# sailab-code/GNN_tf_2.x

Measured on AMD Instinct MI355X. Metric: node-state-updates/sec (nodes x iters / s), 1M-node synthetic graph, higher is better.
Workload: dtype f32; 1 GPU; synthetic randomGraph-recipe graph, N=1000000 nodes, E=9999690 arcs, state_dim=64, net_state 135->128->128->64 selu+BN, net_output 67->2 softmax+BN, max_iter=30, threshold=0 (all iterations run); the loop-invariant label aggregates (GNN.py:259, :263; 0.2 ms) are kept between Loops until the labels change, see cold_aggregates_ms_per_step; parallelism=single GPU, tile_form=one wave per 32-node tile (k_fused)

## Files before the change

gnn_tf_2.x_amd/GNN/_engine.py:

```python
from __future__ import annotations

import ctypes as C
import os

import numpy as np

_HERE = os.path.dirname(os.path.abspath(__file__))
LIB_PATH = os.environ.get('GNN_HIP_LIBRARY') or os.path.join(_HERE, 'libgnn_hip.so')

ACT_CODES = {'linear': 0, None: 0, 'relu': 1, 'selu': 2, 'elu': 3, 'tanh': 4, 'sigmoid': 5, 'softmax': 6}

EXPORTS = ['gnn_last_error', 'gnn_version', 'gnn_device_count', 'gnn_device_synchronize', 'gnn_graph_create', 'gnn_graph_create_from_arcs',
           'gnn_graph_derive', 'gnn_graph_derive_edge', 'gnn_graph_set_arc_order', 'gnn_graph_update_labels', 'gnn_graph_get_nodes', 'gnn_graph_dims', 'gnn_graph_destroy',
           'gnn_mlp_create', 'gnn_mlp_set_weights', 'gnn_mlp_get_weights', 'gnn_mlp_reset_optimizer', 'gnn_mlp_forward', 'gnn_mlp_destroy', 'gnn_loop_create',
           'gnn_loop_set_state0', 'gnn_loop_run', 'gnn_loop_get_state', 'gnn_loop_get_output', 'gnn_loop_readout', 'gnn_loop_set_edge_readout', 'gnn_loop_train_step',
           'gnn_loop_train_forward', 'gnn_loop_train_backward', 'gnn_loop_arm_optimizer', 'gnn_loop_optimizer_step', 'gnn_loop_update_moving_statistics', 'gnn_loss_grad',
           'gnn_loss_grad_ex', 'gnn_loop_set_loss_params',
           'gnn_mlp_set_regularizers', 'gnn_loop_set_clipping', 'gnn_loop_grad_sqnorm', 'gnn_loop_optimizer_step_scaled',
           'gnn_counters_get', 'gnn_lgnn_run', 'gnn_loop_run_many', 'gnn_loop_set_impl', 'gnn_loop_gate_info', 'gnn_loop_set_pieces', 'gnn_loop_range_info', 'gnn_split_f16_exponent', 'gnn_split_f16', 'gnn_loop_set_persistent', 'gnn_loop_set_tile_form', 'gnn_loop_drop_cached_aggregates', 'gnn_loop_set_profiling', 'gnn_loop_get_timing', 'gnn_loop_get_exchange_timing', 'gnn_loop_destroy', 'gnn_shard_range',
           'gnn_comm_unique_id', 'gnn_comm_create', 'gnn_comm_allreduce_max', 'gnn_comm_destroy', 'gnn_halo_plan', 'gnn_graph_create_halo',
           'gnn_comm_create_loopback', 'gnn_graph_set_full_adjacency', 'gnn_loop_set_slice_exchange', 'gnn_loop_run_group', 'gnn_loop_readout_group', 'gnn_graph_update_labels_group']

_lib = None


class EngineError(RuntimeError):
    pass


def lib():
    global _lib
    if _lib is None:
        if not os.path.exists(LIB_PATH):
            raise EngineError(f'{LIB_PATH} is missing: build it with `python -c "import __graft_entry__ as g; g.build()"` '
                              f'or `make -C gnn_tf_2.x_amd/csrc`')
        _lib = C.CDLL(LIB_PATH)
        _lib.gnn_last_error.restype = C.c_char_p
        for name in EXPORTS:
            if name != 'gnn_last_error':
                getattr(_lib, name).restype = C.c_int
    return _lib


def loss_grad(loss_kind: int, targets, out, sample_weights, label_smoothing: float = 0.0, huber_delta: float = 1.0):
    t, o, w = _f32(targets), _f32(out), _f32(sample_weights)
    if t.shape != o.shape or w.shape != (o.shape[0],): raise ValueError(f'targets {t.shape}, outputs {o.shape}, weights {w.shape} do not match')
    d = np.zeros_like(o)
    loss = C.c_double()
    _check(lib().gnn_loss_grad_ex(C.c_int(loss_kind), C.c_int64(o.shape[0]), C.c_int(o.shape[1]), _fp(t), _fp(o), _fp(w), C.c_double(label_smoothing),
                                  C.c_double(huber_delta), C.byref(loss), _fp(d)))
    return float(loss.value), d


def split_f16(values, exponent=None):
    v = np.ascontiguousarray(values, np.float32).ravel()
    if exponent is None:
        exponent = int(lib().gnn_split_f16_exponent(C.c_float(float(np.max(np.abs(v))) if v.size else 0.0)))
    p0, p1 = np.empty(v.size, np.uint16), np.empty(v.size, np.uint16)
    lib().gnn_split_f16(v.ctypes.data_as(C.c_void_p), C.c_int(v.size), C.c_int(int(exponent)), p0.ctypes.data_as(C.c_void_p), p1.ctypes.data_as(C.c_void_p))
    return p0.view(np.float16), p1.view(np.float16), int(exponent)


def _check(rc: int):
    if rc == 0:
        return
    msg = lib().gnn_last_error().decode(errors='replace')
    if rc == -1:
        raise ValueError(msg)
    if rc == -5:
        raise NotImplementedError(msg)
    raise EngineError(f'[gnn_status {rc}] {msg}')


def _f32(a, shape=None):
    a = np.ascontiguousarray(a, dtype=np.float32)
    if shape is not None and a.shape != tuple(shape):
        raise ValueError(f'expected shape {tuple(shape)}, got {a.shape}')
    return a


def _fp(a):
    return a.ctypes.data_as(C.POINTER(C.c_float)) if a is not None else None


def _ip(a):
    return a.ctypes.data_as(C.POINTER(C.c_int32)) if a is not None else None


def device_count() -> int:
    n = C.c_int(0)
    _check(lib().gnn_device_count(C.byref(n)))
    return n.value


def require_device(device: int = 0) -> None:
    n = device_count()
    if n <= device:
        raise EngineError(f'no HIP device {device} visible ({n} found): this engine only runs on MI355X (gfx950)')


def shard_range(n_nodes: int, rank: int, world: int) -> tuple[int, int]:
    b, n = C.c_int64(0), C.c_int64(0)
    _check(lib().gnn_shard_range(C.c_int64(n_nodes), C.c_int(rank), C.c_int(world), C.byref(b), C.byref(n)))
    return b.value, n.value


def halo_plan(n_nodes: int, world: int, indptr, adj_src):
    indptr = np.ascontiguousarray(indptr, dtype=np.int32)
    adj_src = np.ascontiguousarray(adj_src, dtype=np.int32)
    slot = np.empty(n_nodes, np.int32)
    counts = np.zeros(world, np.int64)
    block = C.c_int64(0)
    _check(lib().gnn_halo_plan(C.c_int64(n_nodes), C.c_int(world), _ip(indptr), _ip(adj_src), _ip(slot),
                               counts.ctypes.data_as(C.POINTER(C.c_int64)), C.byref(block)))
    return slot, counts, int(block.value)


def shard_halo(n_nodes: int, rank: int, world: int, indptr, adj_src, nodes, plan=None):
    slot, counts, block = plan if plan is not None else halo_plan(n_nodes, world, indptr, adj_src)
    rb, nr = shard_range(n_nodes, rank, world)
    shard = ((n_nodes + world - 1) // world + 31) // 32 * 32
    indptr = np.asarray(indptr)
    e0, e1 = int(indptr[rb]), int(indptr[rb + nr])
    src = np.asarray(adj_src)[e0:e1].astype(np.int64)
    owner = src // shard
    mine = owner == rank
    if np.any(~mine & (slot[src] < 0)):
        raise ValueError('halo plan does not cover a remote source')
    remapped = np.where(mine, src - rb, shard + owner * block + slot[src]).astype(np.int32)
    nodes = np.asarray(nodes, np.float32)
    rep = np.zeros((shard + world * block, nodes.shape[1]), np.float32)
    rep[:nr] = nodes[rb:rb + nr]
    for q in range(world):
        qb, qn = shard_range(n_nodes, q, world)
        ids = qb + np.nonzero(slot[qb:qb + qn] >= 0)[0]
        rep[shard + q * block: shard + q * block + len(ids)] = nodes[ids]
    send = np.nonzero(slot[rb:rb + nr] >= 0)[0].astype(np.int32)
    return dict(block=block, send_rows=send, adj_src=remapped, nodes=rep, row_begin=rb, n_rows=nr, e0=e0, e1=e1)


def shard_csr(n_nodes: int, rank: int, world: int, indptr, *per_entry_arrays):
    rb, nr = shard_range(n_nodes, rank, world)
    indptr = np.asarray(indptr)
    e0, e1 = int(indptr[rb]), int(indptr[rb + nr])
    return (rb, nr, (indptr[rb:rb + nr + 1] - e0).astype(np.int32)) + tuple(np.asarray(a)[e0:e1] for a in per_entry_arrays)


class Graph:

    def __init__(self, n_nodes, indptr, adj_src, adj_w, arc_w, arc_labels, nodes, mask, row_begin=0, device=0, _handle=None):
        self._h = C.c_void_p()
        if _handle is not None:
            self._h = _handle
            return
        require_device(device)
        indptr = np.ascontiguousarray(indptr, dtype=np.int32)
        adj_src = np.ascontiguousarray(adj_src, dtype=np.int32)
        adj_w, arc_w = _f32(adj_w), _f32(arc_w)
        arc_labels, nodes = _f32(arc_labels), _f32(nodes)
        mask = np.ascontiguousarray(mask, dtype=np.uint8)
        n_rows, n_arcs = len(indptr) - 1, len(adj_src)
        if arc_labels.ndim != 2 or arc_labels.shape[0] != n_arcs or nodes.ndim != 2 or nodes.shape[0] != n_nodes:
            raise ValueError('arc_labels must be [n_arcs, AL] and nodes [n_nodes, NL]')
        if len(adj_w) != n_arcs or len(arc_w) != n_arcs or len(mask) != n_rows:
            raise ValueError('inconsistent array lengths')
        _check(lib().gnn_graph_create(C.c_int64(n_nodes), C.c_int64(row_begin), C.c_int64(n_rows), C.c_int64(n_arcs),
                                      _ip(indptr), _ip(adj_src), _fp(adj_w), _fp(arc_w), _fp(arc_labels),
                                      C.c_int(arc_labels.shape[1]), _fp(nodes), C.c_int(nodes.shape[1]),
                                      mask.ctypes.data_as(C.POINTER(C.c_uint8)), C.c_int(device), C.byref(self._h)))

    @classmethod
    def halo(cls, n_nodes_global, rank, world, block, send_rows, indptr, adj_src_replica, adj_w, arc_w, arc_labels, nodes_replica, mask, device=0):
        require_device(device)
        indptr = np.ascontiguousarray(indptr, dtype=np.int32)
        adj = np.ascontiguousarray(adj_src_replica, dtype=np.int32)
        send = np.ascontiguousarray(send_rows, dtype=np.int32)
        adj_w, arc_w, arc_labels, nodes_replica = _f32(adj_w), _f32(arc_w), _f32(arc_labels), _f32(nodes_replica)
        mask = np.ascontiguousarray(mask, dtype=np.uint8)
        if len(adj_w) != len(adj) or len(arc_w) != len(adj) or arc_labels.shape[0] != len(adj) or len(mask) != len(indptr) - 1:
            raise ValueError('inconsistent array lengths')
        h = C.c_void_p()
        _check(lib().gnn_graph_create_halo(C.c_int64(n_nodes_global), C.c_int(rank), C.c_int(world), C.c_int64(block), C.c_int64(len(send)), _ip(send),
                                           C.c_int64(len(adj)), _ip(indptr), _ip(adj), _fp(adj_w), _fp(arc_w), _fp(arc_labels), C.c_int(arc_labels.shape[1]),
                                           _fp(nodes_replica), C.c_int(nodes_replica.shape[1]), mask.ctypes.data_as(C.POINTER(C.c_uint8)), C.c_int(device), C.byref(h)))
        return cls(None, None, None, None, None, None, None, None, _handle=h)

    @classmethod
    def from_arcs(cls, n_nodes, arc_src, arc_dst, arc_labels, aggregation_mode, nodes, mask, device=0):
        require_device(device)
        modes = {'sum': 0, 'normalized': 1, 'average': 2}
        if aggregation_mode not in modes: raise ValueError('ERROR: Unknown aggregation mode')
        arc_src = np.ascontiguousarray(arc_src, dtype=np.int32)
        arc_dst = np.ascontiguousarray(arc_dst, dtype=np.int32)
        arc_labels, nodes = _f32(arc_labels), _f32(nodes)
        mask = np.ascontiguousarray(mask, dtype=np.uint8)
        e = len(arc_src)
        if len(arc_dst) != e or arc_labels.shape[0] != e or nodes.shape[0] != n_nodes or len(mask) != n_nodes:
            raise ValueError('inconsistent array lengths')
        indptr, adj_src, arc_id = np.zeros(n_nodes + 1, np.int32), np.zeros(e, np.int32), np.zeros(e, np.int32)
        adj_w, arc_w = np.zeros(e, np.float32), np.zeros(e, np.float32)
        h = C.c_void_p()
        _check(lib().gnn_graph_create_from_arcs(C.c_int64(n_nodes), C.c_int64(e), _ip(arc_src), _ip(arc_dst), _fp(arc_labels),
                                                C.c_int(arc_labels.shape[1]), C.c_int(modes[aggregation_mode]), _fp(nodes), C.c_int(nodes.shape[1]),
                                                mask.ctypes.data_as(C.POINTER(C.c_uint8)), C.c_int(device), C.byref(h), _ip(indptr), _ip(adj_src),
                                                _fp(adj_w), _ip(arc_id), _fp(arc_w)))
        return cls(None, None, None, None, None, None, None, None, _handle=h), indptr, adj_src, adj_w, arc_id, arc_w

    def dims(self):
        n, r, e, m = C.c_int64(), C.c_int64(), C.c_int64(), C.c_int64()
        nl, al = C.c_int(), C.c_int()
        _check(lib().gnn_graph_dims(self._h, C.byref(n), C.byref(r), C.byref(e), C.byref(nl), C.byref(al), C.byref(m)))
        return dict(n_nodes=n.value, n_rows=r.value, n_arcs=e.value, NL=nl.value, AL=al.value, n_masked=m.value)

    def derive(self, extra: int) -> 'Graph':
        h = C.c_void_p()
        _check(lib().gnn_graph_derive(self._h, C.c_int(extra), C.byref(h)))
        d = Graph(None, None, None, None, None, None, None, None, _handle=h)
        d._base = self
        return d

    def derive_edge(self, extra_nodes: int, extra_arcs: int) -> 'Graph':
        h = C.c_void_p()
        _check(lib().gnn_graph_derive_edge(self._h, C.c_int(extra_nodes), C.c_int(extra_arcs), C.byref(h)))
        d = Graph(None, None, None, None, None, None, None, None, _handle=h)
        d._base = self
        return d

    def set_arc_order(self, arc_id, arc_labels_orig) -> None:
        arc_id = np.ascontiguousarray(arc_id, dtype=np.int32)
        _check(lib().gnn_graph_set_arc_order(self._h, _ip(arc_id), _fp(_f32(arc_labels_orig))))

    def update_labels(self, base: 'Graph', loop: 'Loop', get_state: bool, get_output: bool) -> None:
        _check(lib().gnn_graph_update_labels(self._h, base._h, loop._h, C.c_int(bool(get_state)), C.c_int(bool(get_output))))

    def set_full_adjacency(self, n_global: int, indptr, adj_src, adj_w):
        ip, src, w = np.ascontiguousarray(indptr, np.int32), np.ascontiguousarray(adj_src, np.int32), _f32(adj_w)
        _check(lib().gnn_graph_set_full_adjacency(self._h, C.c_int64(n_global), _ip(ip), _ip(src), _fp(w)))

    @staticmethod
    def update_labels_group(dsts, bases, loops, get_state: bool, get_output: bool) -> None:
        n = len(loops)
        arr = lambda xs: (C.c_void_p * n)(*[x._h for x in xs])
        _check(lib().gnn_graph_update_labels_group(arr(dsts), arr(bases), arr(loops), C.c_int(n), C.c_int(bool(get_state)), C.c_int(bool(get_output))))

    def nodes(self) -> np.ndarray:
        d = self.dims()
        out = np.empty((d['n_nodes'], d['NL']), dtype=np.float32)
        _check(lib().gnn_graph_get_nodes(self._h, _fp(out)))
        return out

    def close(self):
        if self._h:
            lib().gnn_graph_destroy(self._h)
            self._h = C.c_void_p()

    def __del__(self):
        try:
            self.close()
        except Exception:
            pass


class Mlp:

    def __init__(self, weights, activations, batch_normalization, bn_eps=1e-3, device=0):
        require_device(device)
        self._h = C.c_void_p()
        self.n = len(activations)
        self.activations = list(activations)
        self.batch_normalization = bool(batch_normalization)
        for a in activations:
            if a not in ACT_CODES:
                raise ValueError(f'unsupported activation {a!r}')
        w, b, bn = self._pack(weights)
        self.dims = np.array([w[0].shape[0]] + [x.shape[1] for x in w], dtype=np.int32)
        acts = np.array([ACT_CODES[a] for a in activations], dtype=np.int32)
        wp = (C.POINTER(C.c_float) * self.n)(*[_fp(x) for x in w])
        bp = (C.POINTER(C.c_float) * self.n)(*[_fp(x) for x in b])
        _check(lib().gnn_mlp_create(C.c_int(self.n), _ip(self.dims), _ip(acts), wp, bp, _fp(bn), C.c_float(bn_eps),
                                    C.c_int(device), C.byref(self._h)))

    def _pack(self, weights):
        n = self.n
        if len(weights) != 2 * n + (4 if self.batch_normalization else 0):
            raise ValueError(f'expected {2 * n + (4 if self.batch_normalization else 0)} weight arrays, got {len(weights)}')
        w = [_f32(weights[2 * l]) for l in range(n)]
        b = [_f32(weights[2 * l + 1]) for l in range(n)]
        for l in range(n):
            if w[l].ndim != 2 or b[l].shape != (w[l].shape[1],) or (l and w[l].shape[0] != w[l - 1].shape[1]):
                raise ValueError(f'layer {l}: inconsistent weight shapes')
        bn = None
        if self.batch_normalization:
            bn = np.ascontiguousarray(np.concatenate([_f32(a).ravel() for a in weights[2 * n:]]))
            if bn.size != 4 * w[-1].shape[1]:
                raise ValueError('BatchNormalization arrays must each have the output width')
        return w, b, bn

    def set_weights(self, weights):
        w, b, bn = self._pack(weights)
        if [x.shape for x in w] != [(int(self.dims[l]), int(self.dims[l + 1])) for l in range(self.n)]:
            raise ValueError('weight shapes differ from the ones this MLP was created with')
        wp = (C.POINTER(C.c_float) * self.n)(*[_fp(x) for x in w])
        bp = (C.POINTER(C.c_float) * self.n)(*[_fp(x) for x in b])
        _check(lib().gnn_mlp_set_weights(self._h, wp, bp, _fp(bn)))

    def get_weights(self):
        w = [np.empty((int(self.dims[l]), int(self.dims[l + 1])), np.float32) for l in range(self.n)]
        b = [np.empty((int(self.dims[l + 1]),), np.float32) for l in range(self.n)]
        f = int(self.dims[-1])
        bn = np.empty(4 * f, np.float32) if self.batch_normalization else None
        wp = (C.POINTER(C.c_float) * self.n)(*[_fp(x) for x in w])
        bp = (C.POINTER(C.c_float) * self.n)(*[_fp(x) for x in b])
        _check(lib().gnn_mlp_get_weights(self._h, wp, bp, _fp(bn)))
        out = []
        for l in range(self.n):
            out += [w[l], b[l]]
        if bn is not None:
            out += [bn[i * f:(i + 1) * f].copy() for i in range(4)]
        return out

    def reset_optimizer(self):
        _check(lib().gnn_mlp_reset_optimizer(self._h))

    def set_regularizers(self, coefficients):
        key = None if coefficients is None else (tuple(coefficients[0]), tuple(coefficients[1]))
        if key is not None and not any(key[0]) and not any(key[1]): key = None
        if key == getattr(self, '_reg_set', None):
            return
        if key is None:
            _check(lib().gnn_mlp_set_regularizers(self._h, None, None))
        else:
            if len(key[0]) != 2 * self.n or len(key[1]) != 2 * self.n: raise ValueError(f'expected {2 * self.n} coefficients per list')
            _check(lib().gnn_mlp_set_regularizers(self._h, (C.c_double * (2 * self.n))(*key[0]), (C.c_double * (2 * self.n))(*key[1])))
        self._reg_set = key

    def forward(self, x):
        x = _f32(x)
        if x.ndim != 2 or x.shape[1] != self.dims[0]:
            raise ValueError(f'expected [n, {self.dims[0]}] input')
        y = np.empty((x.shape[0], int(self.dims[-1])), dtype=np.float32)
        _check(lib().gnn_mlp_forward(self._h, C.c_int64(x.shape[0]), _fp(x), _fp(y)))
        return y

    def close(self):
        if self._h:
            lib().gnn_mlp_destroy(self._h)
            self._h = C.c_void_p()

    def __del__(self):
        try:
            self.close()
        except Exception:
            pass


class Comm:

    def __init__(self, unique_id: bytes, rank: int, world: int, device: int, _handle=None):
        self._h = C.c_void_p()
        self.rank, self.world = rank, world
        if _handle is not None:
            self._h = _handle
            return
        buf = (C.c_uint8 * 128).from_buffer_copy(unique_id)
        _check(lib().gnn_comm_create(buf, C.c_int(rank), C.c_int(world), C.c_int(device), C.byref(self._h)))

    @classmethod
    def loopback(cls, world: int, device: int = 0) -> list:
        require_device(device)
        hs = (C.c_void_p * world)()
        _check(lib().gnn_comm_create_loopback(C.c_int(world), C.c_int(device), hs))
        return [cls(None, r, world, device, _handle=C.c_void_p(hs[r])) for r in range(world)]

    @staticmethod
    def unique_id() -> bytes:
        buf = (C.c_uint8 * 128)()
        _check(lib().gnn_comm_unique_id(buf))
        return bytes(buf)

# ... 67 lines not shown
        u8 = lambda a: a.ctypes.data_as(C.POINTER(C.c_uint8)) if a is not None else None
        if ng_csr is not None:
            ngi, ngn, ngw = np.ascontiguousarray(ng_csr[0], np.int32), np.ascontiguousarray(ng_csr[1], np.int32), _f32(ng_csr[2])
            n_graphs = len(ngi) - 1
        else:
            ngi = ngn = ngw = None
            n_graphs = 0
        bs = _f32(bn_state) if bn_state is not None else None
        bo = _f32(bn_output) if bn_output is not None else None
        loss, k = C.c_float(), C.c_float()
        _check(lib().gnn_loop_train_step(self._h, _ip(sip), _ip(sdst), _fp(sw), _fp(targets), _fp(sample_weights),
                                         C.c_int64(targets.shape[0]), C.c_int(loss_kind), C.c_int(n_graphs), _ip(ngi), _ip(ngn), _fp(ngw),
                                         _fp(ds_), _fp(do_), u8(ms), u8(mo), C.c_uint64(seed), _fp(bs), _fp(bo), C.byref(loss), C.byref(k),
                                         _fp(gs), _fp(go), _fp(bns), _fp(bno)))

        def split(flat, shp):
            out, off = [], 0
            for x in shp:
                cnt = int(np.prod(x))
                out.append(flat[off:off + cnt].reshape(x).copy())
                off += cnt
            return out

        kk = int(k.value)
        return dict(loss=float(loss.value), k=float(k.value), grads_state=split(gs, shp_s), grads_output=split(go, shp_o),
                    bn_batch_state=bns[:kk], bn_batch_output=bno)

    def set_slice_exchange(self, on=True, form=None):
        if form not in (None, 'oneshot', 'pipelined'):
            raise ValueError("form must be 'oneshot' or 'pipelined'")
        code = 0 if not on else (1 if form == 'pipelined' else 2)
        _check(lib().gnn_loop_set_slice_exchange(self._h, C.c_int(code)))

    def update_moving_statistics(self, bn_momentum_state: float = 0.99, bn_momentum_output: float = 0.99):
        _check(lib().gnn_loop_update_moving_statistics(self._h, C.c_float(bn_momentum_state), C.c_float(bn_momentum_output)))

    def arm_optimizer(self, kind: int, hyper, mean: bool, bn_momentum_state: float = 0.99, bn_momentum_output: float = 0.99):
        h = _f32(np.asarray(list(hyper) + [0.0] * (4 - len(hyper)), np.float32))
        _check(lib().gnn_loop_arm_optimizer(self._h, C.c_int(kind), _fp(h), C.c_int(1 if mean else 0), C.c_float(bn_momentum_state),
                                            C.c_float(bn_momentum_output)))

    def optimizer_step(self, kind: int, hyper, state_grad_scale: float = 1.0, bn_momentum_state: float = 0.99, bn_momentum_output: float = 0.99):
        h = _f32(np.asarray(list(hyper) + [0.0] * (4 - len(hyper)), np.float32))
        _check(lib().gnn_loop_optimizer_step(self._h, C.c_int(kind), _fp(h), C.c_float(state_grad_scale), C.c_float(bn_momentum_state),
                                             C.c_float(bn_momentum_output)))

    def set_clipping(self, clipvalue: float = 0.0, clipnorm: float = 0.0, global_clipnorm: float = 0.0):
        key = (float(clipvalue), float(clipnorm), float(global_clipnorm))
        if key != getattr(self, '_clip_set', (0.0, 0.0, 0.0)):
            _check(lib().gnn_loop_set_clipping(self._h, C.c_double(key[0]), C.c_double(key[1]), C.c_double(key[2])))
            self._clip_set = key

    def set_loss_params(self, label_smoothing: float = 0.0, huber_delta: float = 1.0):
        key = (float(label_smoothing), float(huber_delta))
        if key != getattr(self, '_loss_params_set', (0.0, 1.0)):
            _check(lib().gnn_loop_set_loss_params(self._h, C.c_double(key[0]), C.c_double(key[1])))
            self._loss_params_set = key

    def grad_sqnorm(self, state_grad_scale: float = 1.0):
        sq, pen = C.c_double(), C.c_double()
        _check(lib().gnn_loop_grad_sqnorm(self._h, C.c_float(state_grad_scale), C.byref(sq), C.byref(pen)))
        return sq.value, pen.value

    def optimizer_step_scaled(self, kind: int, hyper, state_grad_scale: float, grad_scale: float, bn_momentum_state: float = 0.99,
                              bn_momentum_output: float = 0.99):
        h = _f32(np.asarray(list(hyper) + [0.0] * (4 - len(hyper)), np.float32))
        _check(lib().gnn_loop_optimizer_step_scaled(self._h, C.c_int(kind), _fp(h), C.c_float(state_grad_scale), C.c_double(grad_scale),
                                                    C.c_float(bn_momentum_state), C.c_float(bn_momentum_output)))

    @staticmethod
    def _grad_shapes(net: 'Mlp'):
        out = []
        for l in range(net.n):
            out += [(int(net.dims[l]), int(net.dims[l + 1])), (int(net.dims[l + 1]),)]
        if net.batch_normalization:
            out += [(int(net.dims[-1]),), (int(net.dims[-1]),)]
        return out

    def train_forward(self, net_state: 'Mlp', net_output: 'Mlp', src_csr, dropout_state=None, dropout_output=None,
                      masks_state=None, masks_output=None, seed: int = 0, bn_state=None, bn_output=None):
        sip, sdst, sw = (np.ascontiguousarray(src_csr[0], np.int32), np.ascontiguousarray(src_csr[1], np.int32), _f32(src_csr[2])) if src_csr is not None else (None, None, None)
        ds_ = _f32(dropout_state if dropout_state is not None else np.zeros(net_state.n + 1))
        do_ = _f32(dropout_output if dropout_output is not None else np.zeros(net_output.n + 1))
        ms = np.ascontiguousarray(masks_state, np.uint8) if masks_state is not None else None
        mo = np.ascontiguousarray(masks_output, np.uint8) if masks_output is not None else None
        u8 = lambda a: a.ctypes.data_as(C.POINTER(C.c_uint8)) if a is not None else None
        bs = _f32(bn_state) if bn_state is not None else None
        bo = _f32(bn_output) if bn_output is not None else None
        k = C.c_float()
        out = np.zeros((self.n_masked, self.T), np.float32)
        _check(lib().gnn_loop_train_forward(self._h, _ip(sip), _ip(sdst), _fp(sw), _fp(ds_), _fp(do_), u8(ms), u8(mo), C.c_uint64(seed),
                                            _fp(bs), _fp(bo), C.byref(k), _fp(out)))
        self._train_nets = (net_state, net_output, int(k.value))
        return float(k.value), out

    def train_backward(self, d_out_nodes, d_state_extra=None, want_d_nodes: bool = False, want_d_arcs: bool = False):
        net_state, net_output, kk = self._train_nets
        shp_s, shp_o = self._grad_shapes(net_state), self._grad_shapes(net_output)
        gs = np.zeros(sum(int(np.prod(x)) for x in shp_s), np.float32)
        go = np.zeros(sum(int(np.prod(x)) for x in shp_o), np.float32)
        bns = np.zeros((max(1, kk), 2, int(net_state.dims[-1])), np.float32)
        bno = np.zeros((2, int(net_output.dims[-1])), np.float32)
        d_out = _f32(d_out_nodes)
        if d_out.shape != (self.n_masked, self.T): raise ValueError(f'd_out_nodes shape {d_out.shape} != {(self.n_masked, self.T)}')
        dse = None
        if d_state_extra is not None:
            dse = _f32(d_state_extra)
            if dse.shape != (self.n_rows, self.Ds): raise ValueError(f'd_state_extra shape {dse.shape} != {(self.n_rows, self.Ds)}')
        dims = self.graph.dims()
        dn = np.zeros((self.n_rows, dims['NL']), np.float32) if want_d_nodes else None
        da = np.zeros((dims['n_arcs'], dims['AL']), np.float32) if want_d_arcs else None
        _check(lib().gnn_loop_train_backward(self._h, _fp(d_out), _fp(dse), _fp(gs), _fp(go), _fp(bns), _fp(bno), _fp(dn), _fp(da)))

        def split(flat, shp):
            out, off = [], 0
            for x in shp:
                cnt = int(np.prod(x))
                out.append(flat[off:off + cnt].reshape(x).copy())
                off += cnt
            return out

        return dict(grads_state=split(gs, shp_s), grads_output=split(go, shp_o), bn_batch_state=bns[:kk], bn_batch_output=bno, d_nodes=dn, d_arcs=da)

    def set_impl(self, impl: int) -> int:
        used = C.c_int(0)
        _check(lib().gnn_loop_set_impl(self._h, C.c_int(impl), C.byref(used)))
        return used.value

    def gate_info(self) -> tuple:
        a, b = C.c_int(0), C.c_int(0)
        _check(lib().gnn_loop_gate_info(self._h, C.byref(a), C.byref(b)))
        return bool(a.value), int(b.value)

    def set_pieces(self, pieces: int) -> int:
        used = C.c_int(0)
        _check(lib().gnn_loop_set_pieces(self._h, C.c_int(int(pieces)), C.byref(used)))
        return used.value

    def range_info(self) -> tuple:
        a, b = C.c_int(0), C.c_int(0)
        _check(lib().gnn_loop_range_info(self._h, C.byref(a), C.byref(b)))
        return bool(a.value), int(b.value)

    def set_persistent(self, enable: bool) -> bool:
        used = C.c_int(0)
        _check(lib().gnn_loop_set_persistent(self._h, C.c_int(bool(enable)), C.byref(used)))
        return bool(used.value)

    def set_tile_form(self, form: int) -> int:
        used = C.c_int(0)
        _check(lib().gnn_loop_set_tile_form(self._h, C.c_int(int(form)), C.byref(used)))
        return used.value

    def counters(self) -> dict:
        b, f, it, tot, avg = C.c_double(), C.c_double(), C.c_int(), C.c_float(), C.c_float()
        _check(lib().gnn_counters_get(self._h, C.byref(b), C.byref(f), C.byref(it), C.byref(tot), C.byref(avg)))
        return dict(bytes_per_iteration=b.value, flops_per_iteration=f.value, iterations=it.value, total_ms=tot.value, avg_iteration_ms=avg.value)

    @staticmethod
    def lgnn_run(loops, graphs, get_state: bool, get_output: bool) -> list:
        n = len(loops)
        ks = (C.c_float * n)()
        _check(lib().gnn_lgnn_run((C.c_void_p * n)(*[x._h for x in loops]), (C.c_void_p * n)(*[x._h for x in graphs]), C.c_int(n),
                                  C.c_int(bool(get_state)), C.c_int(bool(get_output)), ks))
        return [float(k) for k in ks]

    def drop_cached_aggregates(self):
        _check(lib().gnn_loop_drop_cached_aggregates(self._h))

    def set_profiling(self, on: bool):
        _check(lib().gnn_loop_set_profiling(self._h, C.c_int(bool(on))))

    def run(self, training: bool = False) -> float:
        k = C.c_float(0)
        _check(lib().gnn_loop_run(self._h, C.c_int(bool(training)), C.byref(k)))
        return float(k.value)

    @staticmethod
    def run_many(loops) -> list:
        n = len(loops)
        hs = (C.c_void_p * n)(*[l._h for l in loops])
        ks = (C.c_float * n)()
        _check(lib().gnn_loop_run_many(hs, C.c_int(n), ks))
        return [float(x) for x in ks]

    @staticmethod
    def run_group(loops) -> float:
        n = len(loops)
        hs = (C.c_void_p * n)(*[l._h for l in loops])
        k = C.c_float(0)
        _check(lib().gnn_loop_run_group(hs, C.c_int(n), C.byref(k)))
        return float(k.value)

    @staticmethod
    def readout_group(loops, ng_indptr, ng_node, ng_w) -> np.ndarray:
        n = len(loops)
        hs = (C.c_void_p * n)(*[l._h for l in loops])
        ng_indptr = np.ascontiguousarray(ng_indptr, dtype=np.int32)
        ng_node = np.ascontiguousarray(ng_node, dtype=np.int32)
        ng_w = _f32(ng_w)
        g = len(ng_indptr) - 1
        out = np.empty((g, loops[0].T), dtype=np.float32)
        _check(lib().gnn_loop_readout_group(hs, C.c_int(n), C.c_int(g), _ip(ng_indptr), _ip(ng_node), _fp(ng_w), _fp(out)))
        return out

    def timing(self):
        tot, avg, n = C.c_float(), C.c_float(), C.c_int()
        _check(lib().gnn_loop_get_timing(self._h, C.byref(tot), C.byref(avg), C.byref(n)))
        gap = C.c_float()
        _check(lib().gnn_loop_get_exchange_timing(self._h, C.byref(gap)))
        return dict(total_ms=tot.value, avg_iter_ms=avg.value, n_iter_timed=n.value, avg_between_bodies_ms=gap.value)

    def state(self) -> np.ndarray:
        out = np.empty((self.n_rows, self.Ds), dtype=np.float32)
        _check(lib().gnn_loop_get_state(self._h, _fp(out)))
        return out

    def output(self) -> np.ndarray:
        out = np.empty((self.n_masked, self.T), dtype=np.float32)
        m = C.c_int64(0)
        _check(lib().gnn_loop_get_output(self._h, _fp(out), C.byref(m)))
        return out

    def readout(self, ng_indptr, ng_node, ng_w) -> np.ndarray:
        ng_indptr = np.ascontiguousarray(ng_indptr, dtype=np.int32)
        ng_node = np.ascontiguousarray(ng_node, dtype=np.int32)
        ng_w = _f32(ng_w)
        g = len(ng_indptr) - 1
        out = np.empty((g, self.T), dtype=np.float32)
        _check(lib().gnn_loop_readout(self._h, C.c_int(g), _ip(ng_indptr), _ip(ng_node), _fp(ng_w), _fp(out)))
        return out

    def close(self):
        if self._h:
            lib().gnn_loop_destroy(self._h)
            self._h = C.c_void_p()

    def __del__(self):
        try:
            self.close()
        except Exception:
            pass
```

gnn_tf_2.x_amd/csrc/gnn_build.hip:

```cpp
#include <hipcub/hipcub.hpp>
#include <string.h>

#include <algorithm>
#include <vector>

#include "gnn_common.h"

namespace {

inline unsigned cdiv(int64_t a, int64_t b) { return (unsigned)((a + b - 1) / b); }

__global__ void k_keys(int64_t e, const int32_t *src, const int32_t *dst, unsigned long long *key, int32_t *id, int32_t *indeg)
{
    const int64_t a = (int64_t)blockIdx.x * blockDim.x + threadIdx.x;
    if (a >= e) return;
    key[a] = ((unsigned long long)(uint32_t)dst[a] << 32) | (uint32_t)src[a];
    id[a] = (int32_t)a;
    atomicAdd(indeg + dst[a], 1);
}

__global__ void k_values(int64_t e, const int32_t *dst, const int32_t *indeg, int mode, float *w)
{
    const int64_t a = (int64_t)blockIdx.x * blockDim.x + threadIdx.x;
    if (a >= e) return;
    float v = 1.0f;
    if (mode == 1) v = (float)(1.0 / (double)e);
    else if (mode == 2) v = (float)(1.0 / (double)indeg[dst[a]]);
    w[a] = v;
}

__global__ void k_permute_adj(int64_t e, const int32_t *perm, const int32_t *src, const float *w, int32_t *adj_src, float *adj_w)
{
    const int64_t q = (int64_t)blockIdx.x * blockDim.x + threadIdx.x;
    if (q >= e) return;
    const int32_t a = perm[q];
    adj_src[q] = src[a];
    adj_w[q] = w[a];
}

__global__ void k_permute_arc(int64_t e, int AL, const int32_t *perm, const float *w, const float *labels, float *arc_w, float *arc_labels)
{
    const int64_t t = (int64_t)blockIdx.x * blockDim.x + threadIdx.x;
    const int width = AL > 0 ? AL : 1;
    if (t >= e * width) return;
    const int64_t q = t / width;
    const int c = (int)(t - q * width);
    const int32_t a = perm[q];
    if (c == 0) arc_w[q] = w[a];
    if (AL > 0) arc_labels[q * AL + c] = labels[(int64_t)a * AL + c];
}

struct Scratch {
    std::vector<void *> p;
    template <typename T>
    int get(T **out, size_t count)
    {
        *out = nullptr;
        if (gnn_dev_malloc((void **)out, std::max<size_t>(1, count) * sizeof(T)) != hipSuccess) return gnn_fail(GNN_ERR_HIP, "hipMalloc of %zu bytes failed", count * sizeof(T));
        p.push_back(*out);
        return GNN_OK;
    }
    ~Scratch() { for (void *q : p) (void)hipFree(q); }
};

template <typename T>
int keep(T **dst, size_t count)
{
    *dst = nullptr;
    if (gnn_dev_malloc((void **)dst, std::max<size_t>(1, count) * sizeof(T)) != hipSuccess) return gnn_fail(GNN_ERR_HIP, "hipMalloc of %zu bytes failed", count * sizeof(T));
    return GNN_OK;
}

}

extern "C" int gnn_graph_create_from_arcs(int64_t n_nodes, int64_t n_arcs, const int32_t *arc_src, const int32_t *arc_dst,
                                          const float *arc_labels, int dim_arc_label, int aggregation_mode, const float *nodes,
                                          int dim_node_label, const uint8_t *mask, int device, gnn_graph **out,
                                          int32_t *indptr_out, int32_t *adj_src_out, float *adj_w_out, int32_t *arc_id_out,
                                          float *arc_w_out)
{
    ARGCHK(out, "out is NULL");
    *out = nullptr;
    ARGCHK(n_nodes > 0 && n_nodes < (int64_t)1 << 31, "n_nodes=%lld out of range", (long long)n_nodes);
    ARGCHK(n_arcs >= 0 && n_arcs < (int64_t)1 << 31, "n_arcs=%lld out of range", (long long)n_arcs);
    ARGCHK(dim_node_label > 0 && dim_arc_label >= 0, "label dims must be NL>0, AL>=0");
    ARGCHK(aggregation_mode >= 0 && aggregation_mode <= 2, "aggregation_mode: 0 sum, 1 normalized, 2 average");
    ARGCHK(nodes && mask, "nodes/mask are required");
    ARGCHK(n_arcs == 0 || (arc_src && arc_dst && (arc_labels || dim_arc_label == 0)), "arc arrays are required");
    for (int64_t a = 0; a < n_arcs; ++a)
        ARGCHK(arc_src[a] >= 0 && arc_src[a] < n_nodes && arc_dst[a] >= 0 && arc_dst[a] < n_nodes, "arc %lld = (%d, %d) outside [0,%lld)",
               (long long)a, arc_src[a], arc_dst[a], (long long)n_nodes);
    HIPCHK(hipSetDevice(device));
    const int64_t N = n_nodes, E = n_arcs;
    const int AL = dim_arc_label;
    Scratch tmp;
    int32_t *d_src = nullptr, *d_dst = nullptr, *d_id = nullptr, *d_perm1 = nullptr, *d_perm2 = nullptr, *d_indeg = nullptr, *d_dst_sorted = nullptr;
    unsigned long long *d_key = nullptr, *d_key_sorted = nullptr;
    float *d_lab = nullptr, *d_w = nullptr;
    int rc;
    if ((rc = tmp.get(&d_src, E)) || (rc = tmp.get(&d_dst, E)) || (rc = tmp.get(&d_id, E)) || (rc = tmp.get(&d_perm1, E)) ||
        (rc = tmp.get(&d_perm2, E)) || (rc = tmp.get(&d_indeg, N + 1)) || (rc = tmp.get(&d_dst_sorted, E)) || (rc = tmp.get(&d_key, E)) ||
        (rc = tmp.get(&d_key_sorted, E)) || (rc = tmp.get(&d_lab, (size_t)E * AL)) || (rc = tmp.get(&d_w, E)))
        return rc;
    if (E) {
        HIPCHK(hipMemcpy(d_src, arc_src, sizeof(int32_t) * E, hipMemcpyHostToDevice));
        HIPCHK(hipMemcpy(d_dst, arc_dst, sizeof(int32_t) * E, hipMemcpyHostToDevice));
        if (AL) HIPCHK(hipMemcpy(d_lab, arc_labels, sizeof(float) * E * AL, hipMemcpyHostToDevice));
    }
    HIPCHK(hipMemset(d_indeg, 0, sizeof(int32_t) * (N + 1)));

    gnn_graph *g = new gnn_graph();
    g->device = device; g->N = N; g->N_global = N; g->nodes_rows = N; g->row_begin = 0; g->own_off = 0; g->n_rows = N; g->E = E;
    g->NL = dim_node_label; g->AL = AL; g->base_NL = dim_node_label; g->base_AL = AL;
    g->sh = new gnn_graph_shared();
    gnn_graph_shared *sh = g->sh;
    auto fail = [&](int code) { gnn_graph_destroy(g); return code; };
#define HIPCHK_G(expr)                                                                                         \
    do {                                                                                                       \
        hipError_t e_ = (expr);                                                                                \
        if (e_ != hipSuccess) return fail(gnn_fail(GNN_ERR_HIP, "%s -> %s", #expr, hipGetErrorString(e_)));    \
    } while (0)
    if ((rc = keep(&sh->indptr, N + 1)) || (rc = keep(&sh->adj_src, E)) || (rc = keep(&sh->adj_w, E)) || (rc = keep(&sh->arc_w, E)) ||
        (rc = keep(&sh->arc_labels, (size_t)E * AL)))
        return fail(rc);

    if (E) {
        hipLaunchKernelGGL(k_keys, cdiv(E, 256), 256, 0, 0, E, d_src, d_dst, d_key, d_id, d_indeg);
        hipLaunchKernelGGL(k_values, cdiv(E, 256), 256, 0, 0, E, d_dst, d_indeg, aggregation_mode, d_w);
    }
    {
        size_t bytes = 0;
        if (hipcub::DeviceScan::ExclusiveSum(nullptr, bytes, d_indeg, sh->indptr, (int)(N + 1)) != hipSuccess) return fail(gnn_fail(GNN_ERR_HIP, "hipcub scan sizing failed"));
        void *ws = nullptr;
        if ((rc = tmp.get((char **)&ws, bytes))) return fail(rc);
        if (hipcub::DeviceScan::ExclusiveSum(ws, bytes, d_indeg, sh->indptr, (int)(N + 1)) != hipSuccess) return fail(gnn_fail(GNN_ERR_HIP, "hipcub scan failed"));
    }
    if (E) {
        int node_bits = 1;
        while (((int64_t)1 << node_bits) < N) ++node_bits;
        size_t b1 = 0, b2 = 0;
        if (hipcub::DeviceRadixSort::SortPairs(nullptr, b1, d_key, d_key_sorted, d_id, d_perm1, (int)E, 0, 32 + node_bits) != hipSuccess ||
            hipcub::DeviceRadixSort::SortPairs(nullptr, b2, d_dst, d_dst_sorted, d_id, d_perm2, (int)E, 0, node_bits) != hipSuccess)
            return fail(gnn_fail(GNN_ERR_HIP, "hipcub sort sizing failed"));
        void *ws = nullptr;
        if ((rc = tmp.get((char **)&ws, std::max(b1, b2)))) return fail(rc);
        if (hipcub::DeviceRadixSort::SortPairs(ws, b1, d_key, d_key_sorted, d_id, d_perm1, (int)E, 0, 32 + node_bits) != hipSuccess ||
            hipcub::DeviceRadixSort::SortPairs(ws, b2, d_dst, d_dst_sorted, d_id, d_perm2, (int)E, 0, node_bits) != hipSuccess)
            return fail(gnn_fail(GNN_ERR_HIP, "hipcub sort failed"));
        hipLaunchKernelGGL(k_permute_adj, cdiv(E, 256), 256, 0, 0, E, d_perm1, d_src, d_w, sh->adj_src, sh->adj_w);
        hipLaunchKernelGGL(k_permute_arc, cdiv(E * (AL > 0 ? AL : 1), 256), 256, 0, 0, E, AL, d_perm2, d_w, d_lab, sh->arc_w, sh->arc_labels);
        HIPCHK_G(hipGetLastError());
    }
    HIPCHK_G(hipStreamSynchronize(nullptr));

    std::vector<int32_t> indptr((size_t)N + 1);
    HIPCHK_G(hipMemcpy(indptr.data(), sh->indptr, sizeof(int32_t) * (N + 1), hipMemcpyDeviceToHost));
    if (indptr[N] != E) return fail(gnn_fail(GNN_ERR_HIP, "device build: indptr[N]=%d but %lld arcs", indptr[N], (long long)E));
    int maxdeg = 0;
    for (int64_t r = 0; r < N; ++r) maxdeg = std::max(maxdeg, indptr[r + 1] - indptr[r]);
    sh->max_degree = maxdeg;
    std::vector<int32_t> rows, pos((size_t)N);
    for (int64_t r = 0; r < N; ++r) { pos[r] = (int32_t)rows.size(); if (mask[r]) rows.push_back((int32_t)r); }
    g->n_masked = (int64_t)rows.size();
    std::vector<int32_t> both(rows);
    both.insert(both.end(), pos.begin(), pos.end());
    if ((rc = keep(&sh->mask, N)) || (rc = keep(&sh->masked_rows, both.size())) || (rc = keep(&g->nodes, (size_t)N * dim_node_label))) return fail(rc);
    HIPCHK_G(hipMemcpy(sh->mask, mask, (size_t)N, hipMemcpyHostToDevice));
    HIPCHK_G(hipMemcpy(sh->masked_rows, both.data(), sizeof(int32_t) * both.size(), hipMemcpyHostToDevice));
    HIPCHK_G(hipMemcpy(g->nodes, nodes, sizeof(float) * (size_t)N * dim_node_label, hipMemcpyHostToDevice));

    if (indptr_out) memcpy(indptr_out, indptr.data(), sizeof(int32_t) * (N + 1));
    if (E) {
        if (adj_src_out) HIPCHK_G(hipMemcpy(adj_src_out, sh->adj_src, sizeof(int32_t) * E, hipMemcpyDeviceToHost));
        if (adj_w_out) HIPCHK_G(hipMemcpy(adj_w_out, sh->adj_w, sizeof(float) * E, hipMemcpyDeviceToHost));
        if (arc_id_out) HIPCHK_G(hipMemcpy(arc_id_out, d_perm2, sizeof(int32_t) * E, hipMemcpyDeviceToHost));
        if (arc_w_out) HIPCHK_G(hipMemcpy(arc_w_out, sh->arc_w, sizeof(float) * E, hipMemcpyDeviceToHost));
    }
    *out = g;
    return GNN_OK;
#undef HIPCHK_G
}
```

gnn_tf_2.x_amd/csrc/gnn_common.h:

```cpp
#pragma once
#include <hip/hip_runtime.h>
#include <stdint.h>
#include <string>
#include <vector>

#include "gnn_hip.h"

int gnn_fail(int code, const char *fmt, ...);

hipError_t gnn_dev_malloc(void **p, size_t bytes);
bool gnn_poison_enabled();

#define HIPCHK(expr)                                                                             \
    do {                                                                                         \
        hipError_t e_ = (expr);                                                                  \
        if (e_ != hipSuccess) return gnn_fail(GNN_ERR_HIP, "%s -> %s", #expr, hipGetErrorString(e_)); \
    } while (0)

#define ARGCHK(cond, ...)                                     \
    do {                                                      \
        if (!(cond)) return gnn_fail(GNN_ERR_ARG, __VA_ARGS__); \
    } while (0)

__device__ __forceinline__ float gnn_expf(float x)
{
    const float xc = __builtin_fminf(__builtin_fmaxf(x, -87.33654022216797f), 88.72283935546875f);
    const float u = xc * 1.44269504088896341f;
    const float n = __builtin_rintf(u);
    const float f = u - n;
    float p = 0.0013218672247603536f;
    p = __builtin_fmaf(p, f, 0.009671698324382305f);
    p = __builtin_fmaf(p, f, 0.05550893023610115f);
    p = __builtin_fmaf(p, f, 0.24022237956523895f);
    p = __builtin_fmaf(p, f, 0.6931468844413757f);
    p = __builtin_fmaf(p, f, 1.0f);
    float e = __builtin_ldexpf(p, (int)n);
    e = x > 88.72283935546875f ? __builtin_inff() : e;
    e = x < -87.33654022216797f ? 0.0f : e;
    return x != x ? x : e;
}

__device__ __forceinline__ float gnn_act(float v, int act)
{
    switch (act) {
    case GNN_ACT_RELU: return v > 0.0f ? v : 0.0f;
    case GNN_ACT_SELU: {
        float neg = 1.6732632423543772f * (gnn_expf(v) - 1.0f);
        return 1.0507009873554805f * (v > 0.0f ? v : neg);
    }
    case GNN_ACT_ELU: return v > 0.0f ? v : (gnn_expf(v) - 1.0f);
    case GNN_ACT_TANH: {
        float a = __builtin_fabsf(v);
        float t = gnn_expf(-2.0f * a);
        float q = __fdiv_rn(1.0f - t, 1.0f + t);
        return v < 0.0f ? -q : q;
    }
    case GNN_ACT_SIGMOID: return __fdiv_rn(1.0f, 1.0f + gnn_expf(-v));
    default: return v;
    }
}

#define GNN_FLAG_SLOTS 16
#define GNN_FLAG_STRIDE 32
#define GNN_FLAG_WORDS (GNN_FLAG_SLOTS * GNN_FLAG_STRIDE)
#define GNN_BODY_CHUNK 16

__device__ __forceinline__ bool gnn_gate_open(const int *gate, int world)
{
    if (!gate) return true;
    int any = 0;
    for (int p = 0; p < world * GNN_FLAG_SLOTS; ++p) any |= gate[p * GNN_FLAG_STRIDE];
    return any != 0;
}

__device__ __forceinline__ bool gnn_gate_open_block(const int *gate, int world)
{
    if (!gate) return true;
    __shared__ int gate_any;
    if (threadIdx.x == 0) gate_any = 0;
    __syncthreads();
    int any = 0;
    for (int p = threadIdx.x; p < world * GNN_FLAG_SLOTS; p += blockDim.x) any |= gate[p * GNN_FLAG_STRIDE];
    if (any) gate_any = 1;
    __syncthreads();
    return gate_any != 0;
}

__device__ __forceinline__ void gnn_flag_raise(int *flag_rank_base)
{
    int *w = flag_rank_base + (blockIdx.x & (GNN_FLAG_SLOTS - 1)) * GNN_FLAG_STRIDE;
    if (__hip_atomic_load(w, __ATOMIC_RELAXED, __HIP_MEMORY_SCOPE_AGENT) == 0) atomicOr(w, 1);
}

#define GNN_BAND_ABS 1e-5f
#define GNN_BAND_REL 1e-3f
__device__ __forceinline__ bool gnn_gate_borderline(float root, float rhs, float band) { return band > 0.0f && __builtin_fabsf(root - rhs) <= band; }
struct GnnFlagPeek { int c0, c1, c2; };
__device__ __forceinline__ GnnFlagPeek gnn_flag_peek(int *flag_rank_base)
{
    int *w = flag_rank_base + (blockIdx.x & (GNN_FLAG_SLOTS - 1)) * GNN_FLAG_STRIDE;
    GnnFlagPeek p;
    p.c0 = __hip_atomic_load(w, __ATOMIC_RELAXED, __HIP_MEMORY_SCOPE_AGENT);
    p.c1 = __hip_atomic_load(w + 1, __ATOMIC_RELAXED, __HIP_MEMORY_SCOPE_AGENT);
    p.c2 = __hip_atomic_load(w + 2, __ATOMIC_RELAXED, __HIP_MEMORY_SCOPE_AGENT);
    return p;
}
__device__ __forceinline__ void gnn_flag_raise_peeked(int *flag_rank_base, const GnnFlagPeek &p, bool moved, bool robust, bool border)
{
    int *w = flag_rank_base + (blockIdx.x & (GNN_FLAG_SLOTS - 1)) * GNN_FLAG_STRIDE;
    if (moved && p.c0 == 0) atomicOr(w, 1);
    if (robust && p.c1 == 0) atomicOr(w + 1, 1);
    if (border && p.c2 == 0) atomicOr(w + 2, 1);
}

__device__ __forceinline__ void gnn_flag_raise_certified(int *flag_rank_base, bool moved, bool robust, bool border)
{
    int *w = flag_rank_base + (blockIdx.x & (GNN_FLAG_SLOTS - 1)) * GNN_FLAG_STRIDE;
    if (!(moved || border)) return;
    const int c0 = __hip_atomic_load(w, __ATOMIC_RELAXED, __HIP_MEMORY_SCOPE_AGENT);
    const int c1 = __hip_atomic_load(w + 1, __ATOMIC_RELAXED, __HIP_MEMORY_SCOPE_AGENT);
    const int c2 = __hip_atomic_load(w + 2, __ATOMIC_RELAXED, __HIP_MEMORY_SCOPE_AGENT);
    if (moved && c0 == 0) atomicOr(w, 1);
    if (robust && c1 == 0) atomicOr(w + 1, 1);
    if (border && c2 == 0) atomicOr(w + 2, 1);
}

struct gnn_graph_shared {
    int refs = 1;
    int32_t *indptr = nullptr, *adj_src = nullptr, *masked_rows = nullptr;
    float *adj_w = nullptr, *arc_w = nullptr, *arc_labels = nullptr;
    uint8_t *mask = nullptr;
    int max_degree = 0;
    int32_t *src_indptr = nullptr, *src_dst = nullptr;
    float *src_w = nullptr;
    int32_t *arc_id = nullptr;
    float *arc_labels_orig = nullptr;
    int32_t *full_indptr = nullptr, *full_src = nullptr;
    float *full_w = nullptr;
    int64_t full_rows = 0;
};

struct gnn_graph {
    int device = 0;
    int64_t N = 0, N_global = 0, row_begin = 0, own_off = 0, n_rows = 0, E = 0, n_masked = 0;
    int NL = 0, AL = 0;
    int halo_world = 0, halo_rank = 0;
    int64_t halo_block = 0, halo_count = 0;
    int32_t *halo_send = nullptr;
    bool halo_send_owned = true;
    int64_t nodes_rows = 0;
    gnn_graph_shared *sh = nullptr;
    float *nodes = nullptr;
    int base_NL = 0;
    float *arc_labels_own = nullptr, *arc_labels_orig_own = nullptr;
    int base_AL = 0;
    uint64_t label_version = 1;
    hipEvent_t ready = nullptr;
};

inline const float *gnn_graph_arc_labels(const gnn_graph *g) { return g->arc_labels_own ? g->arc_labels_own : g->sh->arc_labels; }

struct gnn_mlp {
    int device = 0;
    int n_layers = 0;
    std::vector<int> dims, acts;
    std::vector<float *> W, b;
    float *slab = nullptr;
    size_t slab_floats = 0;
    float *bn_scale = nullptr, *bn_shift = nullptr;
    float *bn_raw = nullptr;
    float *opt_a = nullptr, *opt_b = nullptr;
    float *opt_c = nullptr;
    int opt_kind = -1;
    std::vector<double> reg_l1, reg_l2;
    bool has_bn = false;
    float eps = 1e-3f;
    float *packed = nullptr;
    size_t packed_floats = 0;
    int *packed_split = nullptr;
    size_t packed_split_dwords = 0;
    int split_exp[3] = {0, 0, 0};
    int pack_nlc = -1;
    bool pack_dirty = true;
    uint64_t version = 0;
};

struct gnn_loop;
struct gnn_comm_group {
    int world = 1, refs = 0;
    hipStream_t stream = nullptr;
    std::vector<gnn_loop *> member;
};

struct gnn_comm {
    int rank = 0, world = 1, device = 0;
    void *nccl = nullptr;
    gnn_comm_group *grp = nullptr;
    hipStream_t stream = nullptr;
    hipStream_t xstream = nullptr;
    double *scratch = nullptr;
    int loops = 0;
    bool closed = false;
};

struct gnn_train_settings {
    struct { bool armed = false; int kind = 0; float h[4] = {0, 0, 0, 0}; bool mean = false; float mom_s = 0.99f, mom_o = 0.99f; } opt;
    struct { float value = 0.0f; double norm = 0.0, global = 0.0; } clip;
    struct { double smoothing = 0.0, delta = 1.0; } loss;
    int k_hint = 0;
};
#define GNN_INTERNAL __attribute__((visibility("hidden")))
struct GNN_INTERNAL gnn_train_ctx;
struct GNN_INTERNAL gnn_train_arena;

struct gnn_loop {
    gnn_graph *g = nullptr;
    gnn_mlp *st = nullptr, *ou = nullptr;
    gnn_comm *comm = nullptr;
    int device = 0, rank = 0, world = 1;
    int D = 0, Ds = 0, NLc = 0, in_s = 0, wf = 0, T = 0, max_iter = 0;
    float thr = 0.f;
    int64_t shard_rows = 0, N_pad = 0, own_off = 0;
    hipStream_t stream = nullptr;
    float *state[2] = {nullptr, nullptr};
    float *state_init = nullptr;
    float *inp = nullptr;
    float *inv = nullptr;
    uint64_t inv_version = 0;
    float *tmp[2] = {nullptr, nullptr};
    float *feats = nullptr, *out = nullptr, *otmp[2] = {nullptr, nullptr};
    int *flags = nullptr;
    int *tile_ctr = nullptr;
    int *kfinal_dev = nullptr, *kfinal_host = nullptr;
    int certified_reruns = 0;
    bool last_run_rerun = false;
    int pieces = 2;
    int range_reruns = 0;
    bool last_run_range_rerun = false;
    bool small_words_clean = false;
    unsigned small_runs = 0;
    float *small_xs = nullptr;
    size_t small_xs_floats = 0;
    bool small_disabled = false;
    int kfinal = -1;
    bool have_state0 = false, ran = false;
    bool graph_ready_seen = false;
    int impl_req = 1, impl_used = 0;
    int tile_form = 0;
    int32_t *ng_ip = nullptr, *ng_node = nullptr;
    float *ng_w = nullptr, *ng_out = nullptr, *ng_part = nullptr;
    std::vector<int32_t> ng_key;
    std::vector<float> ng_w_host;
    float *ng_host = nullptr;
    int ng_G = 0, ng_host_floats = 0;
    bool ng_inlaunch = false;
    uint64_t out_runs = 0, ng_inlaunch_run = 0;
    bool edge_mode = false, edge_expected = false;
    int32_t *edge_dst = nullptr, *edge_rows = nullptr;
    float *edge_labels = nullptr;
    int64_t n_edge_masked = 0;
    int32_t *edge_inc_ptr = nullptr, *edge_inc = nullptr;
    int *gate_host = nullptr;
    bool profiling = false;
    std::vector<hipEvent_t> ev;
    hipEvent_t ev_total[2] = {nullptr, nullptr};
    float total_ms = 0.f, avg_iter_ms = 0.f;
    float avg_gap_ms = 0.f;
    int n_iter_timed = 0;
    bool slice_mode = false;
    int Cs = 0;
    float *sl_send = nullptr;
    float *sl_state = nullptr;
    float *sl_agg = nullptr;
    float *sl_recv = nullptr;
    bool sl_pipeline = true;
    std::vector<hipEvent_t> sl_ev;
    hipEvent_t sl_done = nullptr;
    float *agg_own = nullptr;
    gnn_train_ctx *train_ctx = nullptr;
    gnn_train_arena *train_arena = nullptr;
    gnn_train_settings train;
};

inline bool gnn_loop_ng_folded(const gnn_loop *l) { return l->ng_inlaunch && l->ng_inlaunch_run == l->out_runs; }

int gnn_graph_wait_ready(const gnn_graph *g, hipStream_t st);
int gnn_launch_spmm(hipStream_t st, int64_t n_rows, const int32_t *indptr, const int32_t *idx, const float *w, const float *X,
                    int width, int64_t ldx, float *out, int64_t ldo, const int *gate, int world);

int gnn_launch_dense(hipStream_t st, int64_t n, int n_in, int n_out, const float *X, int64_t ldx, const float *W, const float *b,
                     int act, float *Y, int64_t ldy);
int gnn_launch_check(hipStream_t st, int64_t n_rows, int d, const float *s, const float *so, float thr, int *flag_rank_base);
int gnn_comm_allgather32(gnn_comm *c, const void *send, void *recv, size_t count, hipStream_t st);
int gnn_launch_feats_edge(hipStream_t st, const gnn_loop *l, const float *state, float *feats);

int gnn_launch_copy_cols(hipStream_t st, int64_t n_rows, int w, const float *src, int64_t lds_, float *dst, int64_t ldd, const int *gate, int world);

int gnn_mlp_refresh_bn(gnn_mlp *m, hipStream_t st);
void gnn_train_ctx_free(gnn_loop *l);
void gnn_train_arena_free(gnn_loop *l);

bool gnn_fused_supported(const gnn_loop *l);
bool gnn_fused_pair_selected(const gnn_loop *l);
int gnn_fused_prepare(gnn_loop *l);
int gnn_fused_pack(gnn_mlp *m, int nlc);
int gnn_fused_iteration(gnn_loop *l, int k);
bool gnn_small_supported(const gnn_loop *l);
int gnn_small_run(gnn_loop *l, bool *output_done);
void gnn_fused_release(gnn_mlp *m);
```

gnn_tf_2.x_amd/csrc/gnn_engine.hip:

```cpp
#include <dlfcn.h>
#include <math.h>
#include <stdarg.h>
#include <stdio.h>
#include <stdlib.h>
#include <string.h>

#include <algorithm>

#include "gnn_common.h"

static thread_local char g_err[1024] = "";

int gnn_fail(int code, const char *fmt, ...)
{
    va_list ap;
    va_start(ap, fmt);
    vsnprintf(g_err, sizeof(g_err), fmt, ap);
    va_end(ap);
    return code;
}

extern "C" const char *gnn_last_error(void) { return g_err; }
extern "C" int gnn_version(void) { return 1; }

// ... 491 lines not shown
}

__global__ void k_arc_base(int64_t E, int ALb, const float *__restrict__ base, int ALd, float *__restrict__ dst)
{
    const int64_t t = (int64_t)blockIdx.x * blockDim.x + threadIdx.x;
    if (t >= E * ALd) return;
    const int64_t p = t / ALd;
    const int c = (int)(t - p * ALd);
    dst[t] = c < ALb ? base[p * ALb + c] : 0.0f;
}

__global__ void k_arc_scatter(int64_t M, int T, const int32_t *__restrict__ rows, const float *__restrict__ out, int ALb, int ALd, float *__restrict__ dst)
{
    const int64_t t = (int64_t)blockIdx.x * blockDim.x + threadIdx.x;
    if (t >= M * T) return;
    const int64_t m = t / T;
    const int c = (int)(t - m * T);
    dst[(int64_t)rows[m] * ALd + ALb + c] = out[t];
}

__global__ void k_arc_permute(int64_t E, int AL, const int32_t *__restrict__ arc_id, const float *__restrict__ orig, float *__restrict__ csr)
{
    const int64_t t = (int64_t)blockIdx.x * blockDim.x + threadIdx.x;
    if (t >= E * AL) return;
    const int64_t q = t / AL;
    const int c = (int)(t - q * AL);
    csr[t] = orig[(int64_t)arc_id[q] * AL + c];
}

__global__ void k_randn(int64_t count, int64_t offset, uint64_t seed, float stddev, float *out)
{
    const int64_t t = (int64_t)blockIdx.x * blockDim.x + threadIdx.x;
    if (t >= count) return;
    const uint64_t h = splitmix64(seed ^ splitmix64((uint64_t)(t + offset)));
    const float u1 = ((float)(uint32_t)(h >> 40) + 1.0f) * (1.0f / 16777217.0f);
    const float u2 = (float)(uint32_t)((h >> 8) & 0xFFFFFF) * (1.0f / 16777216.0f);
    out[t] = stddev * sqrtf(-2.0f * logf(u1)) * cosf(6.28318530717958647692f * u2);
}

__global__ void k_fill(int64_t count, float v, float *out)
{
    const int64_t t = (int64_t)blockIdx.x * blockDim.x + threadIdx.x;
    if (t < count) out[t] = v;
}

static inline unsigned cdiv(int64_t a, int64_t b) { return (unsigned)((a + b - 1) / b); }

int gnn_launch_spmm(hipStream_t st, int64_t n_rows, const int32_t *indptr, const int32_t *idx, const float *w,
                       const float *X, int width, int64_t ldx, float *out, int64_t ldo, const int *gate, int world)
{
    if (n_rows == 0 || width == 0) return GNN_OK;
    const bool vec4 = (width % 4 == 0) && (ldx % 4 == 0) && (((uintptr_t)X & 15) == 0);
    const int vec = vec4 ? 4 : 1;
    int lpr = 1;
    while (lpr * vec < width && lpr < 64) lpr <<= 1;
    const int64_t threads = n_rows * lpr;
    const unsigned grid = (unsigned)std::min<int64_t>(cdiv(threads, 256), 256 * 32);
    const bool indexed = idx != nullptr;
    if (vec4 && indexed && width <= 16) hipLaunchKernelGGL((k_spmm<4, true, 8>), grid, 256, 0, st, n_rows, indptr, idx, w, X, width, ldx, out, ldo, lpr, gate, world);
    else if (vec4 && indexed) hipLaunchKernelGGL((k_spmm<4, true>), grid, 256, 0, st, n_rows, indptr, idx, w, X, width, ldx, out, ldo, lpr, gate, world);
    else if (vec4) hipLaunchKernelGGL((k_spmm<4, false>), grid, 256, 0, st, n_rows, indptr, idx, w, X, width, ldx, out, ldo, lpr, gate, world);
    else if (indexed) hipLaunchKernelGGL((k_spmm<1, true>), grid, 256, 0, st, n_rows, indptr, idx, w, X, width, ldx, out, ldo, lpr, gate, world);
    else hipLaunchKernelGGL((k_spmm<1, false>), grid, 256, 0, st, n_rows, indptr, idx, w, X, width, ldx, out, ldo, lpr, gate, world);
    HIPCHK(hipGetLastError());
    return GNN_OK;
}

int gnn_launch_dense(hipStream_t st, int64_t n, int n_in, int n_out, const float *X, int64_t ldx, const float *W, const float *b,
                     int act, float *Y, int64_t ldy)
{
    if (n == 0) return GNN_OK;
    constexpr int R = 8;
    const int n_in_pad = (n_in + 3) & ~3;
    const size_t lds = sizeof(float) * R * n_in_pad;
    if (lds > 64 * 1024) return gnn_fail(GNN_ERR_UNSUPPORTED, "layer input width %d too large", n_in);
    if (act == GNN_ACT_SOFTMAX) return gnn_fail(GNN_ERR_ARG, "gnn_launch_dense: softmax is applied by the caller");
    const int threads = std::min(256, ((n_out + 63) / 64) * 64);
    hipLaunchKernelGGL((k_dense<R>), cdiv(n, R), threads, lds, st, n, n_in, n_in_pad, n_out, X, ldx, W, b, act, (const float *)nullptr,
                       (const float *)nullptr, Y, ldy, (const int *)nullptr, 1);
    HIPCHK(hipGetLastError());
    return GNN_OK;
}

static int launch_check(hipStream_t st, int64_t n_rows, int d, const float *s, const float *so, float thr, int *flag_out,
                        const int *gate, int world)
{
    if (n_rows == 0) return GNN_OK;
    static bool big_lds[64] = {false};
    int dev = 0;
    HIPCHK(hipGetDevice(&dev));
    if (dev < 0 || dev >= 64 || !big_lds[dev]) {
        HIPCHK(hipFuncSetAttribute(reinterpret_cast<const void *>(k_check), hipFuncAttributeMaxDynamicSharedMemorySize, 2 * 256 * 33 * 4));
        if (dev >= 0 && dev < 64) big_lds[dev] = true;
    }
    hipLaunchKernelGGL(k_check, cdiv(n_rows, 256), 256, sizeof(float) * 256 * 33 * (so ? 2 : 1), st, n_rows, d, s, so, thr, flag_out, gate, world);
    HIPCHK(hipGetLastError());
    return GNN_OK;
}

int gnn_launch_feats_edge(hipStream_t st, const gnn_loop *l, const float *state, float *feats)
{
    if (!l->n_edge_masked) return GNN_OK;
    const gnn_graph *g = l->g;
    const int64_t tot = l->n_edge_masked * l->ou->dims[0];
    hipLaunchKernelGGL(k_feats_edge, cdiv(tot, 256), 256, 0, st, l->n_edge_masked, l->edge_rows, l->edge_dst, g->sh->adj_src, state, state,
                       l->kfinal_dev, l->Ds, g->nodes, g->NL, l->NLc, g->arc_labels_orig_own ? g->arc_labels_orig_own : l->edge_labels, g->AL, feats, l->own_off);
    HIPCHK(hipGetLastError());
    return GNN_OK;
}

int gnn_launch_check(hipStream_t st, int64_t n_rows, int d, const float *s, const float *so, float thr, int *flag_rank_base)
{
    return launch_check(st, n_rows, d, s, so, thr, flag_rank_base, nullptr, 1);
}

static int launch_mlp(hipStream_t st, const gnn_mlp *m, int64_t n, const float *X, int64_t ldx, float *Y, int64_t ldy,
                      float *t0, float *t1, const int *gate, int world)
{
    if (n == 0) return GNN_OK;
    const float *in = X;
    int64_t ldin = ldx;
    constexpr int R = 8;
    for (int l = 0; l < m->n_layers; ++l) {
        const bool last = l == m->n_layers - 1;
        float *out = last ? Y : ((l & 1) ? t1 : t0);
        const int64_t ldo = last ? ldy : m->dims[l + 1];
        const int n_in = m->dims[l], n_out = m->dims[l + 1], act = m->acts[l];
        const int n_in_pad = (n_in + 3) & ~3;
        const size_t lds = sizeof(float) * R * n_in_pad;
        if (lds > 64 * 1024) return gnn_fail(GNN_ERR_UNSUPPORTED, "layer input width %d too large", n_in);
        const int threads = std::min(256, ((n_out + 63) / 64) * 64);
        const float *sc = (last && m->has_bn) ? m->bn_scale : nullptr, *sh = (last && m->has_bn) ? m->bn_shift : nullptr;
        hipLaunchKernelGGL((k_dense<R>), cdiv(n, R), threads, lds, st, n, n_in, n_in_pad, n_out, in, ldin, m->W[l], m->b[l],
                           act, sc, sh, out, ldo, gate, world);
        HIPCHK(hipGetLastError());
        if (act == GNN_ACT_SOFTMAX) {
            hipLaunchKernelGGL(k_softmax_bn, cdiv(n, 256), 256, 0, st, n, n_out, out, ldo, sc, sh, gate, world);
            HIPCHK(hipGetLastError());
        }
        in = out;
        ldin = ldo;
    }
    return GNN_OK;
}

static void graph_release_shared(gnn_graph_shared *sh)
{
    if (!sh || --sh->refs > 0) return;
    (void)hipFree(sh->indptr); (void)hipFree(sh->adj_src); (void)hipFree(sh->masked_rows);
    (void)hipFree(sh->adj_w); (void)hipFree(sh->arc_w); (void)hipFree(sh->arc_labels); (void)hipFree(sh->mask);
    (void)hipFree(sh->src_indptr); (void)hipFree(sh->src_dst); (void)hipFree(sh->src_w);
    (void)hipFree(sh->arc_id); (void)hipFree(sh->arc_labels_orig);
    (void)hipFree(sh->full_indptr); (void)hipFree(sh->full_src); (void)hipFree(sh->full_w);
    delete sh;
}

static int graph_create_impl(int64_t n_index, int64_t n_global, int64_t row_begin, int64_t own_off, int64_t n_rows, int64_t n_arcs,
                             const int32_t *indptr, const int32_t *adj_src, const float *adj_w, const float *arc_w,
                             const float *arc_labels, int dim_arc_label, const float *nodes, int dim_node_label,
                             const uint8_t *mask, int device, gnn_graph **out)
{
    ARGCHK(out, "out is NULL");
    *out = nullptr;
    ARGCHK(n_index > 0 && n_index < (int64_t)1 << 31 && n_global > 0 && n_global < (int64_t)1 << 31, "n_nodes=%lld out of range", (long long)n_global);
    ARGCHK(row_begin >= 0 && n_rows >= 0 && row_begin + n_rows <= n_global && own_off >= 0 && own_off + n_rows <= n_index,
           "owned rows [%lld,+%lld) outside [0,%lld)", (long long)row_begin, (long long)n_rows, (long long)n_global);
    ARGCHK(n_arcs >= 0 && n_arcs < (int64_t)1 << 31, "n_arcs=%lld out of range", (long long)n_arcs);
    ARGCHK(dim_node_label > 0 && dim_arc_label >= 0, "label dims must be NL>0, AL>=0");
    ARGCHK(indptr && nodes && mask, "indptr/nodes/mask are required");
    ARGCHK(n_arcs == 0 || (adj_src && adj_w && arc_w && (arc_labels || dim_arc_label == 0)), "arc arrays are required");
    ARGCHK(indptr[0] == 0 && indptr[n_rows] == n_arcs, "indptr[0]=%d, indptr[n_rows]=%d, n_arcs=%lld", indptr[0],
           indptr[n_rows], (long long)n_arcs);
    int maxdeg = 0;
    for (int64_t r = 0; r < n_rows; ++r) {
        const int d = indptr[r + 1] - indptr[r];
        ARGCHK(d >= 0, "indptr not monotone at row %lld", (long long)r);
        maxdeg = std::max(maxdeg, d);
    }
    for (int64_t e = 0; e < n_arcs; ++e)
        ARGCHK(adj_src[e] >= 0 && adj_src[e] < n_index, "adj_src[%lld]=%d outside [0,%lld)", (long long)e, adj_src[e], (long long)n_index);

    HIPCHK(hipSetDevice(device));
    gnn_graph *g = new gnn_graph();
    g->device = device; g->N = n_index; g->N_global = n_global; g->row_begin = row_begin; g->own_off = own_off; g->n_rows = n_rows; g->E = n_arcs;
    g->NL = dim_node_label; g->AL = dim_arc_label; g->base_NL = dim_node_label; g->base_AL = dim_arc_label;
    g->nodes_rows = n_index;
    g->sh = new gnn_graph_shared();
    g->sh->max_degree = maxdeg;
    std::vector<int32_t> rows, pos((size_t)n_rows);
    for (int64_t r = 0; r < n_rows; ++r) { pos[r] = (int32_t)rows.size(); if (mask[r]) rows.push_back((int32_t)r); }
    g->n_masked = (int64_t)rows.size();
    std::vector<int32_t> both(rows);
    both.insert(both.end(), pos.begin(), pos.end());
    int rc = 0;
    if ((rc = dev_upload(&g->sh->indptr, indptr, (size_t)n_rows + 1)) || (rc = dev_upload(&g->sh->adj_src, adj_src, (size_t)n_arcs)) ||
        (rc = dev_upload(&g->sh->adj_w, adj_w, (size_t)n_arcs)) || (rc = dev_upload(&g->sh->arc_w, arc_w, (size_t)n_arcs)) ||
        (rc = dev_upload(&g->sh->arc_labels, arc_labels, (size_t)n_arcs * dim_arc_label)) ||
        (rc = dev_upload(&g->sh->mask, mask, (size_t)n_rows)) || (rc = dev_upload(&g->sh->masked_rows, both.data(), both.size())) ||
        (rc = dev_upload(&g->nodes, nodes, (size_t)n_index * dim_node_label))) {
        gnn_graph_destroy(g);
        return rc;
    }
    *out = g;
    return GNN_OK;
}

extern "C" int gnn_graph_create(int64_t n_nodes, int64_t row_begin, int64_t n_rows, int64_t n_arcs,
                                const int32_t *indptr, const int32_t *adj_src, const float *adj_w, const float *arc_w,
                                const float *arc_labels, int dim_arc_label, const float *nodes, int dim_node_label,
                                const uint8_t *mask, int device, gnn_graph **out)
{
    return graph_create_impl(n_nodes, n_nodes, row_begin, row_begin, n_rows, n_arcs, indptr, adj_src, adj_w, arc_w, arc_labels, dim_arc_label,
                             nodes, dim_node_label, mask, device, out);
}

extern "C" int gnn_graph_create_halo(int64_t n_nodes_global, int rank, int world, int64_t halo_block, int64_t n_send, const int32_t *send_rows,
                                     int64_t n_arcs, const int32_t *indptr, const int32_t *adj_src_replica, const float *adj_w,
                                     const float *arc_w, const float *arc_labels, int dim_arc_label, const float *nodes_replica,
                                     int dim_node_label, const uint8_t *mask, int device, gnn_graph **out)
{
    ARGCHK(out, "out is NULL");
    *out = nullptr;
    ARGCHK(world >= 2 && rank >= 0 && rank < world && halo_block >= 0 && n_send >= 0 && n_send <= halo_block && (n_send == 0 || send_rows), "bad halo description");
    int64_t rb = 0, nr = 0;
    int rc = gnn_shard_range(n_nodes_global, rank, world, &rb, &nr);
    if (rc) return rc;
    const int64_t shard = ((n_nodes_global + world - 1) / world + 31) / 32 * 32;
    for (int64_t j = 0; j < n_send; ++j)
        ARGCHK(send_rows[j] >= 0 && send_rows[j] < nr && (j == 0 || send_rows[j] > send_rows[j - 1]), "send_rows must be ascending owned-row indices");
    const int64_t n_index = shard + (int64_t)world * halo_block;
    rc = graph_create_impl(n_index, n_nodes_global, rb, 0, nr, n_arcs, indptr, adj_src_replica, adj_w, arc_w, arc_labels, dim_arc_label, nodes_replica,
                           dim_node_label, mask, device, out);
    if (rc) return rc;
    gnn_graph *g = *out;
    g->halo_world = world; g->halo_rank = rank; g->halo_block = halo_block; g->halo_count = n_send;
    rc = dev_upload(&g->halo_send, send_rows, (size_t)n_send);
    if (rc) { gnn_graph_destroy(g); *out = nullptr; return rc; }
    return GNN_OK;
}

extern "C" int gnn_halo_plan(int64_t n_nodes, int world, const int32_t *indptr, const int32_t *adj_src, int32_t *slot, int64_t *counts, int64_t *block)
{
    ARGCHK(n_nodes > 0 && world >= 1 && indptr && slot && counts && block, "bad arguments");
    const int64_t shard = ((n_nodes + world - 1) / world + 31) / 32 * 32;
    std::vector<uint8_t> bnd((size_t)n_nodes, 0);
    for (int64_t d = 0; d < n_nodes; ++d) {
        const int64_t od = d / shard;
        for (int32_t e = indptr[d]; e < indptr[d + 1]; ++e) {
            const int32_t v = adj_src[e];
            ARGCHK(v >= 0 && v < n_nodes, "adj_src[%d]=%d outside [0,%lld)", e, v, (long long)n_nodes);
            if (v / shard != od) bnd[v] = 1;
        }
    }
    int64_t mx = 0;
    for (int q = 0; q < world; ++q) {
        int64_t c = 0;
        const int64_t b = std::min<int64_t>(n_nodes, shard * q), e = std::min<int64_t>(n_nodes, shard * (q + 1));
        for (int64_t v = b; v < e; ++v) slot[v] = bnd[v] ? (int32_t)c++ : -1;
        counts[q] = c;
        mx = std::max(mx, c);
    }
    *block = mx;
    return GNN_OK;
}

static inline const int32_t *graph_mask_pos(const gnn_graph *g) { return g->sh->masked_rows + g->n_masked; }

static inline int64_t derived_node_rows(int64_t n) { return n + 33 * 64; }

extern "C" int gnn_graph_derive(const gnn_graph *base, int extra, gnn_graph **out)
{
    ARGCHK(base && out && extra >= 0, "bad arguments");
    *out = nullptr;
    HIPCHK(hipSetDevice(base->device));
    gnn_graph *g = new gnn_graph(*base);
    g->sh->refs++;
    g->NL = base->base_NL + extra;
    g->nodes = nullptr;
    g->arc_labels_own = g->arc_labels_orig_own = nullptr;
    g->halo_send_owned = false;
    g->AL = base->base_AL;
    g->nodes_rows = derived_node_rows(g->N);
    g->ready = nullptr;
    int rc = dev_alloc(&g->nodes, (size_t)g->nodes_rows * g->NL);
    if (!rc) rc = graph_zero_fill(g, g->nodes, (size_t)g->nodes_rows * g->NL * sizeof(float));
    if (rc) { gnn_graph_destroy(g); return rc; }
    *out = g;
    return GNN_OK;
}

extern "C" int gnn_graph_set_arc_order(gnn_graph *g, const int32_t *arc_id, const float *arc_labels_orig)
{
    ARGCHK(g && (g->E == 0 || (arc_id && (arc_labels_orig || g->AL == 0))), "bad arguments");
    ARGCHK(g->NL == g->base_NL && !g->arc_labels_own, "set the arc order on the original (underived) graph");
    HIPCHK(hipSetDevice(g->device));
    std::vector<uint8_t> seen((size_t)g->E, 0);
    for (int64_t q = 0; q < g->E; ++q) {
        ARGCHK(arc_id[q] >= 0 && arc_id[q] < g->E && !seen[arc_id[q]], "arc_id is not a permutation of the arcs at entry %lld", (long long)q);
        seen[arc_id[q]] = 1;
    }
    (void)hipFree(g->sh->arc_id); (void)hipFree(g->sh->arc_labels_orig);
    g->sh->arc_id = nullptr; g->sh->arc_labels_orig = nullptr;
    int rc = dev_upload(&g->sh->arc_id, arc_id, (size_t)g->E);
    if (!rc) rc = dev_upload(&g->sh->arc_labels_orig, arc_labels_orig, (size_t)g->E * g->AL);
    return rc;
}
// ... 366 lines not shown
        return GNN_OK;
    }
    if (c->nccl && g_rccl.CommDestroy) g_rccl.CommDestroy(c->nccl);
    if (c->stream) (void)hipStreamDestroy(c->stream);
    if (c->xstream) (void)hipStreamDestroy(c->xstream);
    (void)hipFree(c->scratch);
    delete c;
    return GNN_OK;
}

extern "C" int gnn_shard_range(int64_t n_nodes, int rank, int world, int64_t *row_begin, int64_t *n_rows)
{
    ARGCHK(n_nodes > 0 && world >= 1 && rank >= 0 && rank < world && row_begin && n_rows, "bad arguments");
    const int64_t shard = ((n_nodes + world - 1) / world + 31) / 32 * 32;
    const int64_t b = std::min<int64_t>(n_nodes, shard * rank), e = std::min<int64_t>(n_nodes, shard * (rank + 1));
    *row_begin = b;
    *n_rows = e - b;
    return GNN_OK;
}

extern "C" int gnn_loop_create(gnn_graph *g, gnn_mlp *net_state, gnn_mlp *net_output, int state_dim, int max_iter,
                               float threshold, gnn_comm *comm, gnn_loop **out)
{
    ARGCHK(out, "out is NULL");
    *out = nullptr;
    ARGCHK(g && net_state && net_output, "graph and both MLPs are required");
    ARGCHK(state_dim >= 0, "param <state_vect_dim> must be int>=0");
    ARGCHK(max_iter >= 0 && max_iter <= 100000, "max_iteration=%d out of range", max_iter);
    ARGCHK(g->device == net_state->device && g->device == net_output->device, "handles live on different devices");
    const int Ds = state_dim ? state_dim : g->NL;
    const int NLc = state_dim ? g->NL : 0;
    const int in_s = Ds + NLc + Ds + NLc + g->AL;
    ARGCHK(net_state->dims[0] == in_s, "net_state input width %d != AL + 2*(NL + D) = %d", net_state->dims[0], in_s);
    ARGCHK(net_state->dims.back() == Ds, "net_state output width %d != state width %d", net_state->dims.back(), Ds);
    const bool edge_width = net_output->dims[0] == 2 * (Ds + NLc) + g->AL && net_output->dims[0] != Ds + NLc;
    ARGCHK(net_output->dims[0] == Ds + NLc || edge_width, "net_output input width %d is neither NL + D = %d (node/graph based) nor 2 (NL + D) + AL = %d (edge based)",
           net_output->dims[0], Ds + NLc, 2 * (Ds + NLc) + g->AL);
    const int world = comm ? comm->world : 1, rank = comm ? comm->rank : 0;
    ARGCHK(!g->halo_world || (g->halo_world == world && g->halo_rank == rank), "boundary-exchange shard of rank %d/%d used with rank %d/%d",
           g->halo_rank, g->halo_world, rank, world);
    ARGCHK(!comm || !comm->grp || !comm->grp->member[rank], "loopback rank %d already has a loop (one loop per rank and group)", rank);
    int64_t rb = 0, nr = 0;
    gnn_shard_range(g->N_global, rank, world, &rb, &nr);
    ARGCHK(rb == g->row_begin && nr == g->n_rows, "graph owns rows [%lld,+%lld) but rank %d/%d must own [%lld,+%lld)",
           (long long)g->row_begin, (long long)g->n_rows, rank, world, (long long)rb, (long long)nr);
    ARGCHK(!comm || comm->device == g->device, "communicator and graph live on different devices");

    HIPCHK(hipSetDevice(g->device));
    gnn_loop *l = new gnn_loop();
    if (comm) comm->loops++;
    l->g = g; l->st = net_state; l->ou = net_output; l->comm = comm; l->device = g->device; l->rank = rank; l->world = world;
    l->D = state_dim; l->Ds = Ds; l->NLc = NLc; l->in_s = in_s; l->wf = Ds + NLc; l->T = net_output->dims.back();
    l->max_iter = max_iter; l->thr = threshold;
    l->edge_expected = edge_width;
    l->shard_rows = ((g->N_global + world - 1) / world + 31) / 32 * 32;
    l->N_pad = g->halo_world ? g->N : l->shard_rows * world;
    l->own_off = g->halo_world ? 0 : l->shard_rows * rank;
    int rc = 0;
    if (comm) l->stream = comm->stream;
    else {
        hipError_t e = hipStreamCreateWithFlags(&l->stream, hipStreamNonBlocking);
        if (e != hipSuccess) { gnn_loop_destroy(l); return gnn_fail(GNN_ERR_HIP, "hipStreamCreate: %s", hipGetErrorString(e)); }
    }
    int maxw_s = 1, maxw_o = 1;
    for (int i = 1; i <= net_state->n_layers; ++i) maxw_s = std::max(maxw_s, net_state->dims[i]);
    for (int i = 1; i <= net_output->n_layers; ++i) maxw_o = std::max(maxw_o, net_output->dims[i]);
    for (int b = 0; b < 2 && !rc; ++b) {
        rc = dev_alloc(&l->state[b], (size_t)l->N_pad * Ds);
        if (!rc) rc = zero_on_stream(l->state[b], sizeof(float) * (size_t)l->N_pad * Ds, l->stream);
    }
    if (!rc) rc = dev_alloc(&l->flags, (size_t)(max_iter + 2) * world * GNN_FLAG_WORDS + 4);
    if (!rc) rc = dev_alloc(&l->kfinal_dev, 4);
    if (!rc) rc = dev_alloc(&l->tile_ctr, (2 * ((size_t)max_iter + 1) + 3) & ~(size_t)3);
    if (!rc && hipHostMalloc((void **)&l->kfinal_host, 4 * sizeof(int)) != hipSuccess) rc = gnn_fail(GNN_ERR_HIP, "hipHostMalloc");
    if (!rc) l->kfinal_host[1] = l->kfinal_host[2] = l->kfinal_host[3] = 0;
    if (!rc && hipHostMalloc((void **)&l->gate_host, sizeof(int) * (size_t)world * GNN_FLAG_WORDS) != hipSuccess) rc = gnn_fail(GNN_ERR_HIP, "hipHostMalloc");
    if (!edge_width) {
        if (!rc) rc = dev_alloc(&l->feats, (size_t)g->n_masked * l->wf);
        if (!rc) rc = dev_alloc(&l->out, (size_t)g->n_masked * l->T);
        for (int b = 0; b < 2 && !rc; ++b) rc = dev_alloc(&l->otmp[b], (size_t)g->n_masked * maxw_o);
    }
    if (!rc && hipEventCreate(&l->ev_total[0]) != hipSuccess) rc = gnn_fail(GNN_ERR_HIP, "hipEventCreate");
    if (!rc && hipEventCreate(&l->ev_total[1]) != hipSuccess) rc = gnn_fail(GNN_ERR_HIP, "hipEventCreate");
    if (rc) { gnn_loop_destroy(l); return rc; }
    l->impl_req = 2;
    (void)maxw_s;
    if (comm && comm->grp) comm->grp->member[rank] = l;
    *out = l;
    return GNN_OK;
}

static int loop_ensure_unfused(gnn_loop *l)
{
    if (l->inp) return GNN_OK;
    int maxw = 1;
    for (int i = 1; i <= l->st->n_layers; ++i) maxw = std::max(maxw, l->st->dims[i]);
    int rc = dev_alloc(&l->inp, (size_t)l->g->n_rows * l->in_s);
    for (int b = 0; b < 2 && !rc; ++b) rc = dev_alloc(&l->tmp[b], (size_t)l->g->n_rows * maxw);
    return rc;
}

extern "C" int gnn_loop_set_impl(gnn_loop *l, int impl, int *used)
{
    ARGCHK(l && impl >= 0 && impl <= 2, "impl must be 0 (unfused), 1 (fused, exact f32 MFMA) or 2 (fused, split bf16 MFMA)");
    l->impl_req = impl;
    if (used) *used = (impl >= 1 && gnn_fused_supported(l)) ? impl : 0;
    return GNN_OK;
}

extern "C" int gnn_loop_set_pieces(gnn_loop *l, int pieces, int *used)
{
    ARGCHK(l && (pieces == 2 || pieces == 3), "pieces must be 2 (fp16 x 2) or 3 (bf16 x 3)");
    l->pieces = pieces;
    if (used) *used = pieces;
    return GNN_OK;
}

extern "C" int gnn_loop_range_info(const gnn_loop *l, int *last_run_repeated, int *repeats_total)
{
    ARGCHK(l, "loop is NULL");
    if (last_run_repeated) *last_run_repeated = l->last_run_range_rerun ? 1 : 0;
    if (repeats_total) *repeats_total = l->range_reruns;
    return GNN_OK;
}

extern "C" int gnn_loop_gate_info(const gnn_loop *l, int *last_run_repeated, int *repeats_total)
{
    ARGCHK(l, "loop is NULL");
    if (last_run_repeated) *last_run_repeated = l->last_run_rerun ? 1 : 0;
    if (repeats_total) *repeats_total = l->certified_reruns;
    return GNN_OK;
}

extern "C" int gnn_loop_drop_cached_aggregates(gnn_loop *l)
{
    ARGCHK(l, "loop is NULL");
    l->inv_version = 0;
    return GNN_OK;
}

extern "C" int gnn_loop_set_persistent(gnn_loop *l, int enable, int *used)
{
    ARGCHK(l, "loop is NULL");
    l->small_disabled = enable == 0;
    if (used) *used = gnn_small_supported(l) ? 1 : 0;
    return GNN_OK;
}

extern "C" int gnn_loop_set_tile_form(gnn_loop *l, int form, int *used)
{
    ARGCHK(l && form >= 0 && form <= 2, "form must be 0 (library's choice), 1 (one wave per tile) or 2 (wave pair per tile)");
    l->tile_form = form;
    if (used) *used = (l->impl_req >= 1 && gnn_fused_supported(l)) ? (gnn_fused_pair_selected(l) ? 2 : 1) : 0;
    return GNN_OK;
}

extern "C" int gnn_loop_set_profiling(gnn_loop *l, int enable)
{
    ARGCHK(l, "loop is NULL");
    l->profiling = enable != 0;
    return GNN_OK;
}

extern "C" int gnn_loop_get_timing(const gnn_loop *l, float *total_ms, float *avg_iter_ms, int *n_iter_timed)
{
    ARGCHK(l, "loop is NULL");
    if (!l->ran) return gnn_fail(GNN_ERR_STATE, "gnn_loop_run has not been called");
    if (total_ms) *total_ms = l->total_ms;
    if (avg_iter_ms) *avg_iter_ms = l->avg_iter_ms;
    if (n_iter_timed) *n_iter_timed = l->n_iter_timed;
    return GNN_OK;
}

extern "C" int gnn_loop_get_exchange_timing(const gnn_loop *l, float *avg_between_bodies_ms)
{
    ARGCHK(l && avg_between_bodies_ms, "bad arguments");
    if (!l->ran) return gnn_fail(GNN_ERR_STATE, "gnn_loop_run has not been called");
    *avg_between_bodies_ms = l->avg_gap_ms;
    return GNN_OK;
}

extern "C" int gnn_counters_get(const gnn_loop *l, double *bytes_per_iteration, double *flops_per_iteration, int *iterations, float *total_ms,
                                float *avg_iteration_ms)
{
    ARGCHK(l, "loop is NULL");
    const gnn_graph *g = l->g;
    const double n = (double)g->n_rows, e = (double)g->E, ds = (double)l->Ds;
    if (bytes_per_iteration) *bytes_per_iteration = e * (4.0 * ds + 8.0) + 4.0 * (n + 1.0) + n * (8.0 * ds + 4.0 * (2.0 * l->NLc + g->AL));
    if (flops_per_iteration) {
        double f = 0.0;
        for (int i = 0; i < l->st->n_layers; ++i) f += 2.0 * (double)l->st->dims[i] * (double)l->st->dims[i + 1];
        *flops_per_iteration = n * f + 2.0 * e * ds;
    }
    if (iterations) *iterations = l->ran ? l->kfinal : 0;
    if (total_ms) *total_ms = l->ran ? l->total_ms : 0.f;
    if (avg_iteration_ms) *avg_iteration_ms = l->ran ? l->avg_iter_ms : 0.f;
    return GNN_OK;
}

extern "C" int gnn_loop_set_state0(gnn_loop *l, const float *state0, uint64_t seed)
{
    ARGCHK(l, "loop is NULL");
    HIPCHK(hipSetDevice(l->device));
    const gnn_graph *g = l->g;
    const size_t cnt = (size_t)g->n_rows * l->Ds;
    if (!l->state_init && l->D) { int rc = dev_alloc(&l->state_init, cnt); if (rc) return rc; }
    float *own = l->state_init;
    if (l->D == 0) {
        l->have_state0 = true;
        return GNN_OK;
    }
    if (state0) {
        HIPCHK(hipMemcpyAsync(own, state0, cnt * sizeof(float), hipMemcpyHostToDevice, l->stream));
        HIPCHK(hipStreamSynchronize(l->stream));
    } else if (cnt) {
        hipLaunchKernelGGL(k_randn, cdiv((int64_t)cnt, 256), 256, 0, l->stream, (int64_t)cnt, (int64_t)g->row_begin * l->Ds, seed, 0.1f, own);
        HIPCHK(hipGetLastError());
        HIPCHK(hipStreamSynchronize(l->stream));
    }
    l->have_state0 = true;
    return GNN_OK;
}

static const size_t NO_FLAGS = ~(size_t)0;

__global__ void k_pack_rows(int64_t count, int Ds, const int32_t *__restrict__ rows, const float *__restrict__ own, float *__restrict__ dst)
{
    const int64_t t = (int64_t)blockIdx.x * blockDim.x + threadIdx.x;
    if (t >= count * Ds) return;
    const int64_t r = t / Ds;
    const int c = (int)(t - r * Ds);
    dst[t] = own[(int64_t)rows[r] * Ds + c];
}

static inline void loop_segment(const gnn_loop *l, int rank, size_t *off_rows, size_t *rows)
{
    const gnn_graph *g = l->g;
    if (g->halo_world) { *off_rows = (size_t)l->shard_rows + (size_t)rank * g->halo_block; *rows = (size_t)g->halo_block; }
    else { *off_rows = (size_t)l->shard_rows * rank; *rows = (size_t)l->shard_rows; }
}

static int loop_exchange(gnn_loop *l, int b, size_t flag_off)
{
    if (l->world == 1) return GNN_OK;
    const gnn_graph *g = l->g;
    size_t off = 0, rows = 0;
    loop_segment(l, l->rank, &off, &rows);
    if (b >= 0 && g->halo_world && g->halo_count) {
        const int64_t tot = g->halo_count * l->Ds;
        hipLaunchKernelGGL(k_pack_rows, cdiv(tot, 256), 256, 0, l->stream, g->halo_count, l->Ds, g->halo_send, l->state[b] + (size_t)l->own_off * l->Ds,
                           l->state[b] + off * l->Ds);
        HIPCHK(hipGetLastError());
    }
    if (l->comm->grp) {
        gnn_comm_group *grp = l->comm->grp;
        for (int p = 0; p < l->world; ++p) {
            gnn_loop *peer = grp->member[p];
            if (p == l->rank) continue;
            if (!peer) return gnn_fail(GNN_ERR_STATE, "loopback rank %d has no loop: create one loop per rank and run them with gnn_loop_run_group", p);
            if (b >= 0 && rows)
                HIPCHK(hipMemcpyAsync(peer->state[b] + off * l->Ds, l->state[b] + off * l->Ds, sizeof(float) * rows * l->Ds, hipMemcpyDeviceToDevice, l->stream));
            if (flag_off != NO_FLAGS)
                HIPCHK(hipMemcpyAsync(peer->flags + flag_off + (size_t)l->rank * GNN_FLAG_WORDS, l->flags + flag_off + (size_t)l->rank * GNN_FLAG_WORDS,
                                      sizeof(int) * GNN_FLAG_WORDS, hipMemcpyDeviceToDevice, l->stream));
        }
        return GNN_OK;
    }
    size_t base = 0, unused = 0;
    loop_segment(l, 0, &base, &unused);
    NCCLCHK(g_rccl.GroupStart());
    if (b >= 0 && rows)
        NCCLCHK(g_rccl.AllGather(l->state[b] + off * l->Ds, l->state[b] + base * l->Ds, rows * l->Ds, NCCL_FLOAT32, l->comm->nccl, l->stream));
    if (flag_off != NO_FLAGS)
        NCCLCHK(g_rccl.AllGather(l->flags + flag_off + (size_t)l->rank * GNN_FLAG_WORDS, l->flags + flag_off, GNN_FLAG_WORDS, NCCL_INT32, l->comm->nccl, l->stream));
    NCCLCHK(g_rccl.GroupEnd());
    return GNN_OK;
}

__global__ void k_copy_cols(int64_t n_rows, int w, const float *__restrict__ src, int64_t lds_, float *__restrict__ dst, int64_t ldd,
                            const int *gate, int world)
{
    if (!gnn_gate_open_block(gate, world)) return;
    const int64_t t = (int64_t)blockIdx.x * blockDim.x + threadIdx.x;
    if (t >= n_rows * w) return;
    const int64_t r = t / w;
    const int c = (int)(t - r * w);
    dst[r * ldd + c] = src[r * lds_ + c];
}

int gnn_launch_copy_cols(hipStream_t st, int64_t n_rows, int w, const float *src, int64_t lds_, float *dst, int64_t ldd, const int *gate, int world)
{
    if (n_rows == 0 || w == 0) return GNN_OK;
    hipLaunchKernelGGL(k_copy_cols, cdiv(n_rows * w, 256), 256, 0, st, n_rows, w, src, lds_, dst, ldd, gate, world);
    HIPCHK(hipGetLastError());
    return GNN_OK;
}

template <int VEC>
__global__ void k_slice_pack(int64_t n_rows, int64_t shard_rows, int Ds, int Cs, const float *__restrict__ own, float *__restrict__ send,
                             const int *gate, int world)
{
    if (!gnn_gate_open_block(gate, world)) return;
    const int64_t t = (int64_t)blockIdx.x * blockDim.x + threadIdx.x;
    const int pr = Ds / VEC;
    if (t >= shard_rows * pr) return;
    const int64_t r = t / pr;
// ... 811 lines not shown
```

gnn_tf_2.x_amd/csrc/gnn_fused.h:

```cpp
#pragma once
#include <hip/hip_runtime.h>
#include <stdint.h>

constexpr int GNN_FUSED_MAXL = 3;
constexpr int GNN_FUSED_WAVES = 8;
constexpr int GNN_FUSED_THREADS = 64 * GNN_FUSED_WAVES;
#define GNN_F16_EX 4
#define GNN_F16_LIMIT 65504.0f

struct GnnFusedArgs {
    int64_t n_rows, row_begin;
    const int32_t *indptr, *adj_src;
    const float *adj_w;
    const float *inv;
    const float *state_cur;
    float *state_nxt;
    int64_t state_bytes;
    int Ds, NLc, AL, IW, in_s, c_aggs, KP, lpr, lpr_log2, vec, kk0;
    const float *Wp[GNN_FUSED_MAXL];
    const float *bias[GNN_FUSED_MAXL];
    const float *bn_scale, *bn_shift;
    float thr;
    const int *gate;
    int *flag_out;
    int world;
    int certify;
    int *tile_ctr;
    int wstride;
    int stagger;
    const int *Ws[GNN_FUSED_MAXL];
    int chunks0;
    int pieces;
    float bsc[GNN_FUSED_MAXL], usc[GNN_FUSED_MAXL];
    const int *Ws_base;
    int ws_bytes, ws_off[GNN_FUSED_MAXL];
    int tile_base;
    int full_tiles;
    int variant;
    const float *agg_in;
    int threads;
    int single_ticket;
    unsigned long long *stamps;
    int lds_floats;
};

struct GnnSmallCtl {
    float *state0, *state1;
    const float *init;
    int *kfinal;
    int *flags;
    int *host_result;
    float *xs;
    int DP;
    int rnd;
    const float *Wraw[GNN_FUSED_MAXL];
    int din[GNN_FUSED_MAXL], dout[GNN_FUSED_MAXL];
    int KP16;
    int *zero_words;
    int n_words;
    int max_iter;
    float *out;
    const uint8_t *mask;
    const int32_t *mask_pos;
    const float *nodes_own;
    const float *ow, *ob, *obn_scale, *obn_shift;
    int NL, NLc, T, oact;
    const int32_t *ng_ip, *ng_node;
    const float *ng_w;
    float *ng_host;
    int G, ro_word;
    int ecache;
};

constexpr int GNN_SMALL_ECACHE = 1024;
constexpr int GNN_SMALL16_HP = 36;
template <int ROWS>
struct GnnSmallLds {
    static_assert(ROWS == 16 || ROWS == 32, "16- or 32-node tiles");
    static constexpr int H = 0;
    static constexpr int IPT = ROWS == 16 ? 16 * GNN_SMALL16_HP : 32;
    static constexpr int EP = IPT + ROWS + 4;
    static constexpr int HB = EP + 96;
    static constexpr int HW = HB + 64;
    static constexpr int SCR = HW + 544;
    static constexpr int LABELS = 32 * ROWS;
    static constexpr int EC_SRC = SCR + 2 * LABELS;
    static constexpr int EC_W = EC_SRC + GNN_SMALL_ECACHE;
    static constexpr int END = EC_W + GNN_SMALL_ECACHE + 4;
    static constexpr size_t bytes(int KP) { return sizeof(float) * ((size_t)ROWS * KP + END); }
};

template <int... V> struct GnnSteps { static constexpr int values[] = {V...}; };
using GnnSmallKK0 = GnnSteps<8, 12, 16, 24, 32, 36, 40, 48>;
using GnnSmall16S0 = GnnSteps<4, 8, 12, 16, 20, 24>;

bool gnn_small_launch(int layers, int act, int kk0, const GnnFusedArgs &a, const GnnSmallCtl &c, unsigned grid, size_t lds_bytes,
                      hipStream_t st);
bool gnn_small16_launch(int layers, int act, int s0, const GnnFusedArgs &a, const GnnSmallCtl &c, unsigned grid, size_t lds_bytes, hipStream_t st);

bool gnn_fused_launch_l1(int act, int nt, int ntl, const GnnFusedArgs &a, unsigned grid, size_t lds_bytes, hipStream_t st);
bool gnn_fused_launch_s1(int act, int nt, int ntl, const GnnFusedArgs &a, unsigned grid, size_t lds_bytes, hipStream_t st);
bool gnn_fused_launch_s2(int act, int nt, int ntl, const GnnFusedArgs &a, unsigned grid, size_t lds_bytes, hipStream_t st);
bool gnn_fused_launch_s3(int act, int nt, int ntl, const GnnFusedArgs &a, unsigned grid, size_t lds_bytes, hipStream_t st);
bool gnn_fused_launch_p2(int act, const GnnFusedArgs &a, unsigned grid, size_t lds_bytes, hipStream_t st);
bool gnn_fused_launch_p3(int act, const GnnFusedArgs &a, unsigned grid, size_t lds_bytes, hipStream_t st);
bool gnn_fused_launch_l2(int act, int nt, int ntl, const GnnFusedArgs &a, unsigned grid, size_t lds_bytes, hipStream_t st);
bool gnn_fused_launch_l3(int act, int nt, int ntl, const GnnFusedArgs &a, unsigned grid, size_t lds_bytes, hipStream_t st);
```

gnn_tf_2.x_amd/csrc/gnn_fused.hip:

```cpp
#include <stdio.h>
#include <stdlib.h>
#include <string.h>

#include <algorithm>
#include <cmath>
#include <vector>

#include "gnn_common.h"
#include "gnn_fused.h"

namespace {

constexpr int MAXL = GNN_FUSED_MAXL;
constexpr int K_GROUP = 12;
constexpr int K_SLACK = 8;

struct FusedPlan {
    int layers = 0, NT = 0, NTL = 0, KP = 0, kk0 = 0, act = 0;
    int pad = 0, KPs = 0;
    int nt[MAXL] = {0, 0, 0};
    int kk[MAXL] = {0, 0, 0};
    size_t w_off[MAXL] = {0, 0, 0}, b_off[MAXL] = {0, 0, 0}, bn_off = 0, total = 0;
    int chunks[MAXL] = {0, 0, 0};
    size_t s_off[MAXL] = {0, 0, 0}, h_off[MAXL] = {0, 0, 0}, s_total = 0;
};

constexpr int GNN_FUSED_VARIANT_DEFAULT = 1;
constexpr int GNN_FUSED_SPREAD_DEFAULT = 8;
constexpr int GNN_FUSED_SPREAD_SMALL_DEFAULT = 6;
constexpr int S_SLACK = 2;

int round_tiles(int width) { return width <= 32 ? 1 : (width <= 64 ? 2 : 4); }

bool make_plan(const gnn_mlp *m, int nlc, FusedPlan &p)
{
    if (m->n_layers < 1 || m->n_layers > MAXL) return false;
    p.layers = m->n_layers;
    p.act = m->acts[0];
    int hid = 0;
    for (int l = 0; l < m->n_layers; ++l) {
        if (m->acts[l] != p.act || m->acts[l] == GNN_ACT_SOFTMAX) return false;
        if (m->dims[l + 1] > 128) return false;
        if (l < m->n_layers - 1) hid = std::max(hid, m->dims[l + 1]);
    }
    p.NTL = round_tiles(m->dims.back());
    if (p.layers == 1) {
        p.NT = p.NTL;
    } else {
        p.NT = std::max(round_tiles(hid), p.NTL);
        if (p.NT > 1 && p.NTL == 1) p.NTL = 2;
    }
    p.kk0 = ((m->dims[0] + 1) / 2 + K_GROUP - 1) / K_GROUP * K_GROUP;
    p.KP = std::max(2 * p.kk0, (m->dims[0] + 15) / 16 * 16) + 1;
    size_t off = 0;
    for (int l = 0; l < p.layers; ++l) {
        p.nt[l] = l == p.layers - 1 ? p.NTL : p.NT;
        p.kk[l] = l == 0 ? p.kk0 : 16 * p.NT;
        p.w_off[l] = off;
        off += (size_t)(p.kk[l] + (l == 0 ? K_SLACK : 0)) * 64 * p.nt[l];
    }
    for (int l = 0; l < p.layers; ++l) { p.b_off[l] = off; off += 32 * (size_t)p.nt[l]; }
    p.bn_off = off;
    off += 2 * 32 * (size_t)p.NTL;
    p.total = off;
    const int ds = m->dims.back();
    p.pad = ds == 64 ? (4 - (ds + nlc) % 4) % 4 : 0;
    p.KPs = p.KP;
    if (ds == 64) {
        p.KPs = (std::max(2 * p.kk0, (m->dims[0] + p.pad + 15) / 16 * 16) + 3) / 4 * 4;
        if ((p.KPs / 4) % 2 == 0) p.KPs += 4;
    }
    size_t soff = 0;
    for (int l = 0; l < p.layers; ++l) {
        p.chunks[l] = l == 0 ? (m->dims[0] + p.pad + 15) / 16 : 2 * p.NT;
        p.s_off[l] = soff;
        soff += (size_t)(p.chunks[l] + (l == 0 ? S_SLACK : 0)) * p.nt[l] * 3 * 256;
    }
    for (int l = 0; l < p.layers; ++l) {
        p.h_off[l] = soff;
        soff += (size_t)(p.chunks[l] + (l == 0 ? S_SLACK : 0)) * p.nt[l] * 2 * 256;
    }
    p.s_total = soff;
    return true;
}

size_t lds_bytes(const FusedPlan &p)
{
    return (size_t)GNN_FUSED_WAVES * 32 * std::max(p.KP, p.KPs) * sizeof(float) + 128 + GNN_FUSED_WAVES * 36 * sizeof(int) + (3 + 2) * 32 * 4 * sizeof(float) + 16;
}

constexpr int PAIR_CH0 = 9;
bool pair_covers(const FusedPlan &p, int ds) { return ds == 64 && p.NTL == 2 && p.NT == 4 && (p.layers == 2 || p.layers == 3) && p.chunks[0] == PAIR_CH0; }
int pair_xs(const FusedPlan &p)
{
    int xs = 16 * p.chunks[0] - 64 + 4;
    if ((xs / 4) % 2 == 0) xs += 4;
    return xs;
}
size_t pair_lds_bytes(const FusedPlan &p)
{
    return sizeof(float) * ((size_t)4 * (32 * pair_xs(p) + p.chunks[0] * 768) + 16 + GNN_FUSED_WAVES * 20 + 3 * 32 * 2 + 2 * 32 * 4) + 128;
}
int device_cus(int device)
{
    static int n_cu_dev[64] = {0};
    if (device < 0 || device >= 64) return 256;
    if (!n_cu_dev[device]) {
        hipDeviceProp_t prop;
        n_cu_dev[device] = hipGetDeviceProperties(&prop, device) == hipSuccess ? std::max(1, prop.multiProcessorCount) : 256;
    }
    return n_cu_dev[device];
}

}

bool gnn_fused_pair_selected(const gnn_loop *l)
{
    FusedPlan p;
    if (l->impl_req != 2 || l->slice_mode || !make_plan(l->st, l->NLc, p)) return false;
    if (!pair_covers(p, l->Ds) || pair_lds_bytes(p) > 160 * 1024) return false;
    if (l->tile_form) return l->tile_form == 2;
    return (l->g->n_rows + 31) / 32 <= (int64_t)4 * device_cus(l->device);
}

extern "C" int gnn_split_f16_exponent(float max_abs)
{
    if (!(max_abs > 0.0f) || !std::isfinite(max_abs)) return 0;
    int e2 = 0;
    (void)std::frexp(max_abs, &e2);
    return std::min(60, std::max(-60, 15 - e2));
}
extern "C" void gnn_split_f16(const float *v, int n, int e, uint16_t *p0, uint16_t *p1)
{
    for (int i = 0; i < n; ++i) {
        const float s = std::ldexp(v[i], e);
        const _Float16 h0 = (_Float16)s;
        const _Float16 h1 = (_Float16)(s - (float)h0);
        memcpy(p0 + i, &h0, 2);
        memcpy(p1 + i, &h1, 2);
    }
}

int gnn_fused_pack(gnn_mlp *m, int nlc)
{
    FusedPlan p;
    if (!make_plan(m, nlc, p)) { gnn_fused_release(m); return GNN_OK; }
    m->pack_nlc = nlc;
    const int lab = m->dims.back() + nlc;
    std::vector<float> img(p.total, 0.0f);
    std::vector<uint32_t> simg(p.s_total, 0u);
    std::vector<float> W, b;
    for (int l = 0; l < m->n_layers; ++l) {
        const int n_in = m->dims[l], n_out = m->dims[l + 1];
        W.resize((size_t)n_in * n_out);
        b.resize(n_out);
        HIPCHK(hipMemcpy(W.data(), m->W[l], W.size() * sizeof(float), hipMemcpyDeviceToHost));
        HIPCHK(hipMemcpy(b.data(), m->b[l], b.size() * sizeof(float), hipMemcpyDeviceToHost));
        float *wp = img.data() + p.w_off[l];
        const int nt = p.nt[l];
        for (int kk = 0; kk < p.kk[l]; ++kk)
            for (int lane = 0; lane < 64; ++lane)
                for (int jt = 0; jt < nt; ++jt) {
                    const int k = 2 * kk + (lane >> 5), j = 32 * jt + (lane & 31);
                    wp[((size_t)kk * 64 + lane) * nt + jt] = (k < n_in && j < n_out) ? W[(size_t)k * n_out + j] : 0.0f;
                }
        for (int j = 0; j < n_out; ++j) img[p.b_off[l] + j] = b[j];
        float fold = 1.0f;
        if (p.act == GNN_ACT_SELU && m->n_layers > 1) {
            const double LOG2E = 1.44269504088896341, SCALE = 1.0507009873554805;
            const bool in_folded = l > 0, out_folded = l < m->n_layers - 1;
            fold = (float)((in_folded ? SCALE / LOG2E : 1.0) * (out_folded ? LOG2E : 1.0));
        }
        uint32_t *sp = simg.data() + p.s_off[l];
        std::vector<float> wf((size_t)p.chunks[l] * nt * 64 * 8);
        for (int c = 0; c < p.chunks[l]; ++c)
            for (int jt = 0; jt < nt; ++jt)
                for (int lane = 0; lane < 64; ++lane)
                    for (int i = 0; i < 8; ++i) {
                        const int h = lane >> 5, r = 8 * (c & 1) + i;
                        int k = l == 0 ? 16 * c + 8 * h + i : 32 * (c >> 1) + (r & 3) + 8 * (r >> 2) + 4 * h;
                        if (l == 0 && p.pad) k = k < lab ? k : (k < lab + p.pad ? n_in : k - p.pad);
                        const int j = 32 * jt + (lane & 31);
                        float v = (k < n_in && j < n_out) ? W[(size_t)k * n_out + j] : 0.0f;
                        v *= fold;
                        wf[(((size_t)c * nt + jt) * 64 + lane) * 8 + i] = v;
                        for (int pc = 0; pc < 3; ++pc) {
                            uint32_t bits;
                            memcpy(&bits, &v, 4);
                            const uint32_t hi = bits & 0xffff0000u;
                            float piece;
                            memcpy(&piece, &hi, 4);
                            v = v - piece;
                            uint32_t &d = sp[((((size_t)c * nt + jt) * 3 + pc) * 64 + lane) * 4 + i / 2];
                            d |= (i & 1) ? hi : (hi >> 16);
                        }
                    }
        float mw = 0.0f;
        for (float v : wf) mw = std::max(mw, std::fabs(v));
        const int e = gnn_split_f16_exponent(mw);
        m->split_exp[l] = e;
        std::vector<uint16_t> h0(wf.size()), h1(wf.size());
        gnn_split_f16(wf.data(), (int)wf.size(), e, h0.data(), h1.data());
        uint16_t *hp = reinterpret_cast<uint16_t *>(simg.data() + p.h_off[l]);
        for (int c = 0; c < p.chunks[l]; ++c)
            for (int jt = 0; jt < nt; ++jt)
                for (int lane = 0; lane < 64; ++lane)
                    for (int i = 0; i < 8; ++i) {
                        const size_t src = (((size_t)c * nt + jt) * 64 + lane) * 8 + i;
                        hp[((((size_t)c * nt + jt) * 2 + 0) * 64 + lane) * 8 + i] = h0[src];
                        hp[((((size_t)c * nt + jt) * 2 + 1) * 64 + lane) * 8 + i] = h1[src];
                    }
    }
    if (m->has_bn) {
        const int f = m->dims.back();
        HIPCHK(hipMemcpy(img.data() + p.bn_off, m->bn_scale, f * sizeof(float), hipMemcpyDeviceToHost));
        HIPCHK(hipMemcpy(img.data() + p.bn_off + 32 * p.NTL, m->bn_shift, f * sizeof(float), hipMemcpyDeviceToHost));
    }
    if (m->packed_floats != p.total) {
        gnn_fused_release(m);
        HIPCHK(gnn_dev_malloc((void **)&m->packed, p.total * sizeof(float)));
        m->packed_floats = p.total;
    }
    HIPCHK(hipMemcpy(m->packed, img.data(), p.total * sizeof(float), hipMemcpyHostToDevice));
    if (m->packed_split_dwords != p.s_total) {
        if (m->packed_split) (void)hipFree(m->packed_split);
        m->packed_split = nullptr;
        HIPCHK(gnn_dev_malloc((void **)&m->packed_split, p.s_total * sizeof(uint32_t)));
        m->packed_split_dwords = p.s_total;
    }
    HIPCHK(hipMemcpy(m->packed_split, simg.data(), p.s_total * sizeof(uint32_t), hipMemcpyHostToDevice));
    return GNN_OK;
}

void gnn_fused_release(gnn_mlp *m)
{
    if (m->packed) (void)hipFree(m->packed);
    if (m->packed_split) (void)hipFree(m->packed_split);
    m->packed = nullptr;
    m->packed_split = nullptr;
    m->packed_floats = 0;
    m->packed_split_dwords = 0;
}

bool gnn_fused_supported(const gnn_loop *l)
{
    FusedPlan p;
    if (!make_plan(l->st, l->NLc, p)) return false;
    if (l->st->pack_dirty || l->st->pack_nlc != l->NLc) {
        if (gnn_fused_pack(l->st, l->NLc) != GNN_OK) return false;
        l->st->pack_dirty = false;
    }
    if (!l->st->packed) return false;
    if (lds_bytes(p) > 160 * 1024) return false;
    const int Ds = l->Ds;
    if (!((Ds % 4 == 0 && Ds <= 256) || Ds <= 64)) return false;
    if ((int64_t)l->N_pad * Ds * (int64_t)sizeof(float) >= ((int64_t)1 << 31)) return false;
    return l->g->n_rows > 0;
}

int gnn_fused_prepare(gnn_loop *l)
{
    const gnn_graph *g = l->g;
    const int IW = 2 * l->NLc + g->AL;
    if (!l->inv) {
        const size_t inv_floats = std::max<size_t>(1, (size_t)((g->n_rows + 31) / 32 * 32) * IW);
        HIPCHK(gnn_dev_malloc((void **)&l->inv, inv_floats * sizeof(float)));
        HIPCHK(hipMemsetAsync(l->inv, 0, inv_floats * sizeof(float), l->stream));
    }
    if (IW == 0) return GNN_OK;
    if (l->inv_version == g->label_version) return GNN_OK;
    l->inv_version = g->label_version;
    int rc = gnn_launch_spmm(l->stream, g->n_rows, g->sh->indptr, nullptr, g->sh->arc_w, gnn_graph_arc_labels(g), g->AL, g->AL,
                             l->inv + 2 * l->NLc, IW, nullptr, 1);
    if (rc) return rc;
    if (l->NLc) {
        rc = gnn_launch_spmm(l->stream, g->n_rows, g->sh->indptr, g->sh->adj_src, g->sh->adj_w, g->nodes, g->NL, g->NL,
                             l->inv + l->NLc, IW, nullptr, 1);
        if (rc) return rc;
        rc = gnn_launch_copy_cols(l->stream, g->n_rows, g->NL, g->nodes + (size_t)g->own_off * g->NL, g->NL, l->inv, IW, nullptr, 1);
        if (rc) return rc;
    }
    return GNN_OK;
}

static int fused_args(gnn_loop *l, int k, bool split, FusedPlan &p, GnnFusedArgs &a)
{
    const gnn_graph *g = l->g;
    const gnn_mlp *m = l->st;
    if (!make_plan(m, l->NLc, p)) return gnn_fail(GNN_ERR_UNSUPPORTED, "fused path does not cover this net_state");
    if (m->pack_nlc != l->NLc) return gnn_fail(GNN_ERR_STATE, "weight image laid out for another label width");
    const int cur = k & 1, nxt = cur ^ 1, P = l->world;
    a = GnnFusedArgs{};
    a.n_rows = g->n_rows; a.row_begin = l->own_off;
    a.indptr = g->sh->indptr; a.adj_src = g->sh->adj_src; a.adj_w = g->sh->adj_w;
    a.inv = l->inv;
    a.state_cur = l->state[cur];
    a.state_bytes = (int64_t)l->N_pad * l->Ds * (int64_t)sizeof(float);
    a.state_nxt = l->state[nxt] + (size_t)l->own_off * l->Ds;
    const int pad = split ? p.pad : 0;
    a.Ds = l->Ds; a.NLc = l->NLc; a.AL = g->AL; a.IW = 2 * l->NLc + g->AL; a.in_s = l->in_s + pad; a.c_aggs = l->Ds + l->NLc + pad;
    a.KP = split ? p.KPs : p.KP; a.kk0 = p.kk0;
    a.vec = (l->Ds % 4 == 0) ? 4 : 1;
    int lpr = 1, lg = 0;
    while ((lpr * a.vec < l->Ds || lpr < 2) && lpr < 64) { lpr <<= 1; ++lg; }
    a.lpr = lpr; a.lpr_log2 = lg;
    for (int i = 0; i < p.layers; ++i) {
        a.Wp[i] = m->packed + p.w_off[i];
        a.bias[i] = m->packed + p.b_off[i];
    }
    for (int i = 0; i < p.layers; ++i) a.Ws[i] = m->packed_split + p.s_off[i];
    a.chunks0 = p.chunks[0];
    a.Ws_base = m->packed_split;
    a.ws_bytes = (int)(p.s_total * sizeof(uint32_t));
    a.pieces = l->pieces == 2 ? 2 : 3;
    for (int i = 0; i < p.layers; ++i) {
        a.ws_off[i] = (int)((a.pieces == 2 ? p.h_off[i] : p.s_off[i]) * sizeof(uint32_t));
        const int e = a.pieces == 2 ? m->split_exp[i] + GNN_F16_EX : 0;
        a.bsc[i] = std::ldexp(1.0f, e);
        a.usc[i] = std::ldexp(1.0f, -e);
    }
    a.variant = GNN_FUSED_VARIANT_DEFAULT;
    a.bn_scale = m->has_bn ? m->packed + p.bn_off : nullptr;
    a.bn_shift = m->has_bn ? m->packed + p.bn_off + 32 * p.NTL : nullptr;
    a.thr = l->thr;
    a.gate = l->flags + (size_t)k * P * GNN_FLAG_WORDS;
    a.flag_out = l->flags + ((size_t)(k + 1) * P + l->rank) * GNN_FLAG_WORDS;
    a.world = P;
    a.certify = split ? 1 : 0;
    a.stamps = nullptr;
    a.agg_in = l->slice_mode ? l->agg_own : nullptr;
    a.threads = 0;
    a.wstride = 1;
    a.tile_base = 0;
    a.full_tiles = 0;
    return GNN_OK;
}

int gnn_fused_iteration(gnn_loop *l, int k)
{
    const gnn_graph *g = l->g;
    FusedPlan p;
    GnnFusedArgs a;
    const bool split = l->impl_req == 2;
    int rc = fused_args(l, k, split, p, a);
    if (rc) return rc;
    const size_t n_tiles = (size_t)((g->n_rows + 31) / 32);
#ifdef GNN_DIAG
    static const int variant_env = getenv("GNN_FUSED_VARIANT") ? atoi(getenv("GNN_FUSED_VARIANT")) : GNN_FUSED_VARIANT_DEFAULT;
    a.variant = variant_env;
#endif
#ifdef GNN_DIAG
    static const int debug = getenv("GNN_FUSED_DEBUG") ? atoi(getenv("GNN_FUSED_DEBUG")) : 0;
    a.wstride = (debug & 1) ? 0 : 1;
    static const char *stamp_file = getenv("GNN_FUSED_STAMPS");
    static unsigned long long *stamp_buf = nullptr;
    const size_t n_waves = n_tiles;
    if (stamp_file && k == 1) {
        if (!stamp_buf) HIPCHK(gnn_dev_malloc((void **)&stamp_buf, n_waves * 16 * sizeof(unsigned long long)));
        HIPCHK(hipMemsetAsync(stamp_buf, 0, n_waves * 16 * sizeof(unsigned long long), l->stream));
        a.stamps = stamp_buf;
    }
#endif
    if (l->device < 0 || l->device >= 64) return gnn_fail(GNN_ERR_ARG, "device %d out of range", l->device);
    const int n_cu = device_cus(l->device);
    const unsigned grid = (unsigned)std::min<size_t>((size_t)n_cu, n_tiles);
    a.tile_ctr = l->tile_ctr + k;
    int stagger_rounds = GNN_FUSED_SPREAD_DEFAULT;
#ifdef GNN_DIAG
    static const int stagger_env = getenv("GNN_FUSED_STAGGER") ? atoi(getenv("GNN_FUSED_STAGGER")) : GNN_FUSED_SPREAD_DEFAULT;
    stagger_rounds = stagger_env;
#endif
    a.stagger = n_tiles >= (size_t)4 * GNN_FUSED_WAVES * grid ? stagger_rounds : (n_tiles > (size_t)GNN_FUSED_WAVES * grid ? GNN_FUSED_SPREAD_SMALL_DEFAULT : 0);
#ifdef GNN_DIAG
    static const int stagger_small = getenv("GNN_FUSED_STAGGER_SMALL") ? atoi(getenv("GNN_FUSED_STAGGER_SMALL")) : 0;
    const bool small_grid = n_tiles > (size_t)GNN_FUSED_WAVES * grid && n_tiles < (size_t)4 * GNN_FUSED_WAVES * grid;
    if (small_grid && stagger_small > 0) { a.stagger = stagger_small; a.variant |= 4; }
    static const int spread_small = getenv("GNN_FUSED_SPREAD_SMALL") ? atoi(getenv("GNN_FUSED_SPREAD_SMALL")) : -1;
    if (small_grid && spread_small >= 0) a.stagger = spread_small;
#endif
    a.single_ticket = n_tiles <= (size_t)GNN_FUSED_WAVES * grid ? 1 : 0;
    const size_t lds = lds_bytes(p);
    a.lds_floats = gnn_poison_enabled() ? (int)(lds / sizeof(float)) : 0;
    auto go = [&](const GnnFusedArgs &aa, unsigned gr) -> bool {
        if (split) {
            if (p.layers == 1) return gnn_fused_launch_s1(p.act, p.NT, p.NTL, aa, gr, lds, l->stream);
            if (p.layers == 2) return gnn_fused_launch_s2(p.act, p.NT, p.NTL, aa, gr, lds, l->stream);
            return gnn_fused_launch_s3(p.act, p.NT, p.NTL, aa, gr, lds, l->stream);
        }
        if (p.layers == 1) return gnn_fused_launch_l1(p.act, p.NT, p.NTL, aa, gr, lds, l->stream);
        if (p.layers == 2) return gnn_fused_launch_l2(p.act, p.NT, p.NTL, aa, gr, lds, l->stream);
        return gnn_fused_launch_l3(p.act, p.NT, p.NTL, aa, gr, lds, l->stream);
    };
    bool ok = false;
    const int64_t n_tiles64 = (g->n_rows + 31) / 32;
    bool pair = false;
    if (split && gnn_fused_pair_selected(l)) {
        GnnFusedArgs ap = a;
        ap.KP = pair_xs(p);
        ap.full_tiles = 1; ap.tile_base = 0;
        const unsigned grid_p = (unsigned)std::min<int64_t>((int64_t)n_cu, (n_tiles64 + 3) / 4);
        ap.stagger = n_tiles64 >= (int64_t)4 * 4 * grid_p ? stagger_rounds : (n_tiles64 > (int64_t)4 * grid_p ? GNN_FUSED_SPREAD_SMALL_DEFAULT : 0);
        const size_t lds_p = pair_lds_bytes(p);
        ap.lds_floats = gnn_poison_enabled() ? (int)(lds_p / sizeof(float)) : 0;
        pair = p.layers == 2 ? gnn_fused_launch_p2(p.act, ap, grid_p, lds_p, l->stream) : gnn_fused_launch_p3(p.act, ap, grid_p, lds_p, l->stream);
    }
    if (pair) ok = true;
    else if (l->Ds == 64 && p.NTL == 2 && n_tiles64 >= 1) {
        GnnFusedArgs af = a;
        af.full_tiles = 1; af.tile_base = 0;
        ok = go(af, (unsigned)std::min<size_t>((size_t)n_cu, (size_t)n_tiles64));
    } else
        ok = go(a, grid);
    if (!ok) return gnn_fail(GNN_ERR_UNSUPPORTED, "no fused instantiation for %d layers, tiles (%d,%d), activation %d", p.layers, p.NT, p.NTL, p.act);
#ifdef GNN_DIAG
    if (a.stamps) {
        std::vector<unsigned long long> host(n_waves * (pair ? 16 : 8));
        HIPCHK(hipStreamSynchronize(l->stream));
        HIPCHK(hipMemcpy(host.data(), stamp_buf, host.size() * sizeof(unsigned long long), hipMemcpyDeviceToHost));
        if (FILE *f = fopen(stamp_file, "wb")) { fwrite(host.data(), sizeof(unsigned long long), host.size(), f); fclose(f); }
    }
#endif
    HIPCHK(hipGetLastError());
    return GNN_OK;
}

bool gnn_small_supported(const gnn_loop *l)
{
    if (l->world != 1 || l->impl_req < 1 || l->small_disabled || l->profiling) return false;
    if (!gnn_fused_supported(l)) return false;
    FusedPlan p;
    if (!make_plan(l->st, l->NLc, p)) return false;
    if (p.NT != 1 || p.NTL != 1) return false;
    const int64_t n_tiles = (l->g->n_rows + 31) / 32;
    if (p.kk0 > 48) return false;
    return n_tiles >= 1 && n_tiles <= 256;
}

int gnn_small_run(gnn_loop *l, bool *output_done)
{
    FusedPlan p;
    GnnFusedArgs a;
    int rc = fused_args(l, 0, false, p, a);
    if (rc) return rc;
    const gnn_graph *g = l->g;
    a.gate = nullptr; a.flag_out = nullptr; a.tile_ctr = nullptr; a.stagger = 0;
    GnnSmallCtl c{};
    c.state0 = l->state[0]; c.state1 = l->state[1];
    c.init = l->D ? l->state_init : g->nodes + (size_t)g->own_off * g->NL;
    c.kfinal = l->kfinal_dev;
    c.host_result = l->kfinal_host;
    int kk_small = p.kk0, s0 = 0;
    for (int cand : GnnSmallKK0::values)
        if (2 * cand >= a.in_s && cand <= p.kk0) { kk_small = cand; break; }
    for (int cand : GnnSmall16S0::values)
        if (4 * cand >= a.in_s) { s0 = cand; break; }
    bool tile16 = g->n_rows <= 16 * 256 && s0 > 0;
#ifdef GNN_DIAG
    static const int tile_env = getenv("GNN_SMALL_TILE") ? atoi(getenv("GNN_SMALL_TILE")) : 0;
    if (tile_env == 32) tile16 = false;
#endif
    const int rows_per_tile = tile16 ? 16 : 32;
    const unsigned grid = (unsigned)((g->n_rows + rows_per_tile - 1) / rows_per_tile);
    c.DP = l->Ds <= 16 ? 16 : 32;
    {
        const size_t need = (size_t)2 * grid * rows_per_tile * c.DP;
        if (l->small_xs_floats < need) {
            if (l->small_xs) (void)hipFree(l->small_xs);
            l->small_xs = nullptr; l->small_xs_floats = 0;
            HIPCHK(gnn_dev_malloc((void **)&l->small_xs, need * sizeof(float)));
            l->small_xs_floats = need;
        }
        c.xs = l->small_xs;
    }
    c.max_iter = l->max_iter;
    c.ecache = GNN_SMALL_ECACHE;
#ifdef GNN_DIAG
    static const int ecache_env = getenv("GNN_SMALL_ECACHE") ? atoi(getenv("GNN_SMALL_ECACHE")) : GNN_SMALL_ECACHE;
    c.ecache = std::min(GNN_SMALL_ECACHE, ecache_env);
#endif
    const size_t n_words = ((size_t)l->max_iter + 3 + 3) & ~(size_t)3;
    l->kfinal_host[1] = 0;
    if (!l->small_words_clean) {
        HIPCHK(hipMemsetAsync(l->flags, 0, sizeof(int) * 2 * n_words, l->stream));
        l->small_words_clean = true;
        l->small_runs = 0;
    }
    c.flags = l->flags + (l->small_runs & 1) * n_words;
    c.zero_words = l->flags + ((l->small_runs & 1) ^ 1) * n_words;
    c.n_words = (int)n_words;
    ++l->small_runs;
    *output_done = false;
    const gnn_mlp *ou = l->ou;
    if (!l->edge_mode && g->n_masked && ou->n_layers == 1 && l->T <= 8 && l->Ds + l->NLc <= 64 && l->Ds <= 32 && g->NL <= 32) {
        c.out = l->out; c.mask = g->sh->mask; c.mask_pos = g->sh->masked_rows + g->n_masked;
        c.nodes_own = g->nodes + (size_t)g->own_off * g->NL;
        c.ow = ou->W[0]; c.ob = ou->b[0];
        c.obn_scale = ou->has_bn ? ou->bn_scale : nullptr; c.obn_shift = ou->has_bn ? ou->bn_shift : nullptr;
        c.NL = g->NL; c.NLc = l->NLc; c.T = l->T; c.oact = ou->acts[0];
        *output_done = true;
        l->ng_inlaunch = false;
        if (l->ng_ip && l->ng_G > 0 && g->n_masked == g->n_rows) {
            if (l->ng_host_floats < l->ng_G * l->T) {
                if (l->ng_host) (void)hipHostFree(l->ng_host);
                l->ng_host = nullptr; l->ng_host_floats = 0;
                if (hipHostMalloc((void **)&l->ng_host, sizeof(float) * (size_t)l->ng_G * l->T) == hipSuccess) l->ng_host_floats = l->ng_G * l->T;
            }
            if (l->ng_host) {
                c.ng_ip = l->ng_ip; c.ng_node = l->ng_node; c.ng_w = l->ng_w; c.ng_host = l->ng_host; c.G = l->ng_G; c.ro_word = l->max_iter + 1;
                l->ng_inlaunch = true;
                l->ng_inlaunch_run = l->out_runs;
            }
        }
    }
    c.rnd = g->sh->max_degree > 8 ? 8 : 4;
#ifdef GNN_DIAG
    static const char *small_stamp_file = getenv("GNN_SMALL_STAMPS");
    static unsigned long long *small_stamp_buf = nullptr;
    if (small_stamp_file) {
        if (!small_stamp_buf) HIPCHK(gnn_dev_malloc((void **)&small_stamp_buf, 256 * sizeof(unsigned long long)));
        HIPCHK(hipMemsetAsync(small_stamp_buf, 0, 256 * sizeof(unsigned long long), l->stream));
        a.stamps = small_stamp_buf;
    }
#endif
    bool launched;
    if (tile16) {
        const gnn_mlp *m = l->st;
        for (int q = 0; q < p.layers; ++q) { c.Wraw[q] = m->W[q]; c.din[q] = m->dims[q]; c.dout[q] = m->dims[q + 1]; }
        c.KP16 = std::max((a.in_s + 3) / 4 * 4, 4 * s0);
        if (c.KP16 % 8 == 0) c.KP16 += 4;
        const size_t lds = GnnSmallLds<16>::bytes(c.KP16);
        a.lds_floats = gnn_poison_enabled() ? (int)(lds / sizeof(float)) : 0;
        launched = gnn_small16_launch(p.layers, p.act, s0, a, c, grid, lds, l->stream);
    } else {
        const size_t lds = GnnSmallLds<32>::bytes(p.KP);
        a.lds_floats = gnn_poison_enabled() ? (int)(lds / sizeof(float)) : 0;
        launched = gnn_small_launch(p.layers, p.act, kk_small, a, c, grid, lds, l->stream);
    }
    if (!launched)
        return gnn_fail(GNN_ERR_UNSUPPORTED, "no persistent-loop instantiation for %d layers, activation %d", p.layers, p.act);
    HIPCHK(hipGetLastError());
#ifdef GNN_DIAG
    if (small_stamp_file) {
        unsigned long long host[256];
        HIPCHK(hipStreamSynchronize(l->stream));
        HIPCHK(hipMemcpy(host, small_stamp_buf, sizeof(host), hipMemcpyDeviceToHost));
        if (FILE *f = fopen(small_stamp_file, "wb")) { fwrite(host, sizeof(unsigned long long), 256, f); fclose(f); }
    }
#endif
    return GNN_OK;
}
```

gnn_tf_2.x_amd/csrc/gnn_fused_kernel.h:

```cpp
#pragma once
#include <utility>

#include "gnn_common.h"
#include "gnn_fused.h"

typedef float f32x16 __attribute__((ext_vector_type(16)));

namespace gnn_fused_dev {

#define GNN_GLOBAL __attribute__((address_space(1)))
template <class T>
__device__ __forceinline__ const GNN_GLOBAL T *gptr(const T *p) { return (const GNN_GLOBAL T *)p; }
template <class T>
__device__ __forceinline__ GNN_GLOBAL T *gptr_w(T *p) { return (GNN_GLOBAL T *)p; }
typedef float v4f __attribute__((ext_vector_type(4)));
typedef float v2f __attribute__((ext_vector_type(2)));
typedef int v4i_ __attribute__((ext_vector_type(4)));
__device__ __forceinline__ v4f gload4(const float *p) { return *(const GNN_GLOBAL v4f *)p; }
#ifndef GNN_STORE_AUX
#define GNN_STORE_AUX 2
#endif
__device__ __forceinline__ void gstore_row4(float *base, int64_t off, v4f v)
{
#if GNN_STORE_AUX == 0
// ... 588 lines not shown
    {
        i = lane / width; c = lane - i * width;
        qi = 64 / width; qc = 64 - qi * width;
    }
    __device__ __forceinline__ void next()
    {
        i += qi; c += qc;
        if (c >= width) { c -= width; ++i; }
    }
};

__device__ __forceinline__ void zero_pad_columns(const GnnFusedArgs &a, float *X, int lane, int KP)
{
    const int padw = KP - a.in_s;
    RowCol rc(lane, padw);
    for (int t = lane; t < 32 * padw; t += 64, rc.next()) X[rc.i * KP + a.in_s + rc.c] = 0.0f;
    const int hole0 = a.Ds + a.NLc, holew = a.c_aggs - hole0;
    if (holew > 0 && lane < 32)
        for (int c = 0; c < holew; ++c) X[lane * KP + hole0 + c] = 0.0f;
}

template <bool COH = false, int RND = 4>
__device__ __forceinline__ void load_tile_generic(const GnnFusedArgs &a, float *X, const int *ipt, int64_t i0, int lane,
                                               int nvalid, int KP, int c_aggs, bool own_from_lds = false, const int *ecache_src = nullptr,
                                               const float *ecache_w = nullptr, int ecache_base = 0, bool skip_gather = false)
{
    const int Ds = a.Ds, NLc = a.NLc;
    if (!own_from_lds) {
        zero_pad_columns(a, X, lane, KP);
        if (nvalid < 32) {
            RowCol rc(lane, a.in_s);
            for (int t = lane; t < (32 - nvalid) * a.in_s; t += 64, rc.next()) X[(nvalid + rc.i) * KP + rc.c] = 0.0f;
        }
    }
    if (own_from_lds) {
        const int total = nvalid * Ds;
        RowCol rc(lane, Ds);
        for (int t = lane; t < total; t += 64, rc.next()) X[rc.i * KP + rc.c] = X[rc.i * KP + c_aggs + rc.c];
        __builtin_amdgcn_fence(__ATOMIC_ACQ_REL, "wavefront");
    } else {
        const float *src = a.state_cur + (a.row_begin + i0) * Ds;
        const int total = nvalid * Ds;
        RowCol rc(lane, Ds);
        for (int t = lane; t < total; t += 64, rc.next()) X[rc.i * KP + rc.c] = sload1<COH>(src + t);
    }
    if (a.IW > 0 && !own_from_lds) {
        const float *src = a.inv + i0 * a.IW;
        const int total = nvalid * a.IW;
        RowCol rc(lane, a.IW);
        for (int t = lane; t < total; t += 64, rc.next()) X[rc.i * KP + label_col(rc.c, Ds, NLc, c_aggs)] = gload1(src + t);
    }
    __builtin_amdgcn_fence(__ATOMIC_ACQ_REL, "wavefront");
    if (skip_gather) return;
    if (a.agg_in) {
        const float *src = a.agg_in + i0 * Ds;
        const int total = nvalid * Ds;
        RowCol rc(lane, Ds);
        for (int t = lane; t < total; t += 64, rc.next()) X[rc.i * KP + c_aggs + rc.c] = gload1(src + t);
        return;
    }
    if (Ds <= 32) {
        const int node = lane & 31, hf = lane >> 5;
        const int cbeg = hf ? (Ds + 1) / 2 : 0, cend = hf ? Ds : (Ds + 1) / 2;
        const int beg = ipt[node], end = ipt[node + 1];
        float acc[16];
#pragma unroll
        for (int c = 0; c < 16; ++c) acc[c] = 0.0f;
        for (int e = beg; e < end; e += RND) {
            float w[RND];
            const float *xp[RND];
#pragma unroll
            for (int u = 0; u < RND; ++u) {
                const int ee = e + u < end ? e + u : e;
                w[u] = ecache_w ? ecache_w[ee - ecache_base] : gload1(a.adj_w + ee);
                xp[u] = a.state_cur + (int64_t)(ecache_src ? ecache_src[ee - ecache_base] : gload1(a.adj_src + ee)) * Ds + cbeg;
            }
            float x[RND][16];
#pragma unroll
            for (int u = 0; u < RND; ++u)
#pragma unroll
                for (int c = 0; c < 16; ++c) x[u][c] = (cbeg + c < cend) ? sload1<COH>(xp[u] + c) : 0.0f;
#pragma unroll
            for (int u = 0; u < RND; ++u)
                if (e + u < end) {
#pragma unroll
                    for (int c = 0; c < 16; ++c)
                        if (cbeg + c < cend) acc[c] = __builtin_fmaf(w[u], x[u][c], acc[c]);
                }
        }
        if (node < nvalid) {
#pragma unroll
            for (int c = 0; c < 16; ++c)
                if (cbeg + c < cend) X[node * KP + c_aggs + cbeg + c] = acc[c];
        }
        return;
    }
    const int lpr = a.lpr, gl = lane & (lpr - 1), grp = lane >> a.lpr_log2, groups = 64 >> a.lpr_log2;
    const bool colok = gl * a.vec < Ds;
    const int c0 = colok ? gl * a.vec : 0;
    for (int pass = 0; pass * groups < 32; ++pass) {
        const int i = pass * groups + grp;
        const int beg = ipt[i], end = ipt[i + 1];
        float acc[4] = {0.f, 0.f, 0.f, 0.f};
        for (int e = beg; e < end; e += 4) {
            float w[4];
            v4f x[4];
#pragma unroll
            for (int u = 0; u < 4; ++u) {
                const int ee = e + u < end ? e + u : e;
                w[u] = gload1(a.adj_w + ee);
                const float *xp = a.state_cur + (int64_t)gload1(a.adj_src + ee) * Ds + c0;
                if (a.vec == 4) {
                    if constexpr (COH) x[u] = v4f{sload1<true>(xp), sload1<true>(xp + 1), sload1<true>(xp + 2), sload1<true>(xp + 3)};
                    else x[u] = gload4(xp);
                } else x[u] = v4f{sload1<COH>(xp), 0.f, 0.f, 0.f};
            }
#pragma unroll
            for (int u = 0; u < 4; ++u) {
                if (e + u < end) {
                    acc[0] = __builtin_fmaf(w[u], x[u].x, acc[0]);
                    if (a.vec == 4) {
                        acc[1] = __builtin_fmaf(w[u], x[u].y, acc[1]); acc[2] = __builtin_fmaf(w[u], x[u].z, acc[2]);
                        acc[3] = __builtin_fmaf(w[u], x[u].w, acc[3]);
                    }
                }
            }
        }
        if (i < nvalid && colok) {
            float *x = X + i * KP + c_aggs + c0;
            x[0] = acc[0];
            if (a.vec == 4) { x[1] = acc[1]; x[2] = acc[2]; x[3] = acc[3]; }
        }
    }
}

__device__ __forceinline__ void gather_fma(v2f &acc01, v2f &acc23, float w, v4f x)
{
    float a0 = acc01.x, a1 = acc01.y, a2 = acc23.x, a3 = acc23.y;
    asm("v_fma_f32 %0, %1, %2, %0" : "+v"(a0) : "v"(w), "v"(x.x));
    asm("v_fma_f32 %0, %1, %2, %0" : "+v"(a1) : "v"(w), "v"(x.y));
    asm("v_fma_f32 %0, %1, %2, %0" : "+v"(a2) : "v"(w), "v"(x.z));
    asm("v_fma_f32 %0, %1, %2, %0" : "+v"(a3) : "v"(w), "v"(x.w));
    acc01 = v2f{a0, a1}; acc23 = v2f{a2, a3};
}

template <int GB, int... J>
__device__ __forceinline__ void gather_batch(int my_src, float my_w, __amdgpu_buffer_rsrc_t rsrc, int voff0, float (&w)[GB],
                                             v4f (&x)[GB], std::integer_sequence<int, J...>)
{
    ((w[J] = row_bcast_f<J>(my_w),
      x[J] = __builtin_bit_cast(v4f, __builtin_amdgcn_raw_buffer_load_b128(rsrc, (row_bcast_i<J>(my_src) << 8) + voff0, 0, 0))), ...);
}

template <bool AL16, bool PADDED = false>
__device__ __forceinline__ void load_tile_fast64(const GnnFusedArgs &a, float *X, const int *ipt, int64_t i0, int lane,
                                                 int KP, int c_aggs, int my_src, float my_w)
{
    constexpr int GB = 16, Ds = 64;
    const int gl = lane & 15, grp = lane >> 4;
    v4f own[8];
    {
        const float *src = a.state_cur + (a.row_begin + i0) * Ds + lane * 4;
#pragma unroll
        for (int u = 0; u < 8; ++u) own[u] = gload4(src + u * 256);
    }
    float lab[4];
    const int IW = a.IW, nlab = 32 * IW;
    {
        const float *src = a.inv + i0 * IW;
#pragma unroll
        for (int u = 0; u < 4; ++u) lab[u] = (lane + 64 * u < nlab) ? gload1(src + lane + 64 * u) : 0.0f;
    }
    if constexpr (!PADDED) zero_pad_columns(a, X, lane, KP);
    __builtin_amdgcn_fence(__ATOMIC_ACQ_REL, "wavefront");

    int node = grp * 8;
    const int node_end = node + 8;
    const int e_begin = ipt[node], e_end = ipt[node_end];
    int next_end = ipt[node + 1];
    v2f acc01 = {0.f, 0.f}, acc23 = {0.f, 0.f};
    const __amdgpu_buffer_rsrc_t rsrc = __builtin_amdgcn_make_buffer_rsrc(const_cast<float *>(a.state_cur), 0, (int)a.state_bytes, 0x00020000);
    const int voff0 = gl * 16;
    float *xo = X + c_aggs + gl * 4;
#define GNN_ROW_BOUNDARY(e)                                                                     \
    while ((e) >= next_end) {                                                                   \
        float *xr = xo + node * KP;                                                             \
        if constexpr (AL16) *reinterpret_cast<v4f *>(xr) = v4f{acc01.x, acc01.y, acc23.x, acc23.y};   \
        else { xr[0] = acc01.x; xr[1] = acc01.y; xr[2] = acc23.x; xr[3] = acc23.y; }            \
        acc01 = v2f{0.f, 0.f}; acc23 = v2f{0.f, 0.f};                                           \
        ++node;                                                                                 \
        next_end = ipt[node + 1];                                                               \
    }
    int base = e_begin;
    for (; base + GB <= e_end; base += GB) {
        float w[GB];
        v4f x[GB];
        gather_batch<GB>(my_src, my_w, rsrc, voff0, w, x, std::make_integer_sequence<int, GB>{});
        const int nb = base + GB + gl;
        my_src = 0; my_w = 0.0f;
        if (nb < e_end) { my_src = gstream1(a.adj_src + nb); my_w = gstream1(a.adj_w + nb); }
#pragma unroll
        for (int u = 0; u < GB; ++u) {
            GNN_ROW_BOUNDARY(base + u)
            gather_fma(acc01, acc23, w[u], x[u]);
        }
    }
    {
        const int cnt = e_end - base;
        float w[GB];
        v4f x[GB];
        gather_batch<GB>(my_src, my_w, rsrc, voff0, w, x, std::make_integer_sequence<int, GB>{});
#pragma unroll
        for (int u = 0; u < GB; ++u) {
            if (u < cnt) {
                GNN_ROW_BOUNDARY(base + u)
                gather_fma(acc01, acc23, w[u], x[u]);
            }
        }
    }
#undef GNN_ROW_BOUNDARY
    for (; node < node_end; ++node) {
        float *xr = xo + node * KP;
        if constexpr (AL16) *reinterpret_cast<v4f *>(xr) = v4f{acc01.x, acc01.y, acc23.x, acc23.y};
        else { xr[0] = acc01.x; xr[1] = acc01.y; xr[2] = acc23.x; xr[3] = acc23.y; }
        acc01 = v2f{0.f, 0.f}; acc23 = v2f{0.f, 0.f};
    }
#pragma unroll
    for (int u = 0; u < 8; ++u) {
        float *x = X + (4 * u + (lane >> 4)) * KP + (lane & 15) * 4;
        if constexpr (AL16) *reinterpret_cast<v4f *>(x) = own[u];
        else { x[0] = own[u].x; x[1] = own[u].y; x[2] = own[u].z; x[3] = own[u].w; }
    }
    const float inv_iw = 1.0f / (float)(IW > 0 ? IW : 1);
#pragma unroll
    for (int u = 0; u < 4; ++u) {
        const int t = lane + 64 * u;
        if (t < nlab) {
            const int i = (int)(((float)t + 0.5f) * inv_iw), c = t - i * IW;
            X[i * KP + label_col(c, Ds, a.NLc, c_aggs)] = lab[u];
        }
    }
    if (nlab > 256)
        for (int t = 256 + lane; t < nlab; t += 64) {
            const int i = t / IW, c = t - i * IW;
            X[i * KP + label_col(c, Ds, a.NLc, c_aggs)] = gload1(a.inv + i0 * IW + t);
        }
}

template <bool AL16>
__device__ __forceinline__ void load_tile_given64(const GnnFusedArgs &a, float *X, int64_t i0, int lane, int KP, int c_aggs)
{
    constexpr int Ds = 64;
    v4f own[8], agg[8];
    {
        const float *src = a.state_cur + (a.row_begin + i0) * Ds + lane * 4;
        const float *sag = a.agg_in + i0 * Ds + lane * 4;
#pragma unroll
        for (int u = 0; u < 8; ++u) {
            own[u] = gload4(src + u * 256);
            agg[u] = gload4(sag + u * 256);
        }
    }
    float lab[4];
    const int IW = a.IW, nlab = 32 * IW;
    {
        const float *src = a.inv + i0 * IW;
#pragma unroll
        for (int u = 0; u < 4; ++u) lab[u] = (lane + 64 * u < nlab) ? gload1(src + lane + 64 * u) : 0.0f;
    }
#pragma unroll
    for (int u = 0; u < 8; ++u) {
        float *x = X + (4 * u + (lane >> 4)) * KP + (lane & 15) * 4;
        if constexpr (AL16) { *reinterpret_cast<v4f *>(x) = own[u]; *reinterpret_cast<v4f *>(x + c_aggs) = agg[u]; }
        else {
            x[0] = own[u].x; x[1] = own[u].y; x[2] = own[u].z; x[3] = own[u].w;
            x[c_aggs] = agg[u].x; x[c_aggs + 1] = agg[u].y; x[c_aggs + 2] = agg[u].z; x[c_aggs + 3] = agg[u].w;
        }
    }
    const float inv_iw = 1.0f / (float)(IW > 0 ? IW : 1);
#pragma unroll
    for (int u = 0; u < 4; ++u) {
        const int t = lane + 64 * u;
        if (t < nlab) {
            const int i = (int)(((float)t + 0.5f) * inv_iw), c = t - i * IW;
            X[i * KP + label_col(c, Ds, a.NLc, c_aggs)] = lab[u];
        }
    }
    if (nlab > 256)
        for (int t = 256 + lane; t < nlab; t += 64) {
            const int i = t / IW, c = t - i * IW;
            X[i * KP + label_col(c, Ds, a.NLc, c_aggs)] = gload1(a.inv + i0 * IW + t);
        }
}

template <bool COH = false, bool STORE = true>
__device__ __forceinline__ void check_store_generic(const GnnFusedArgs &a, float *X, int64_t i0, int lane, int nvalid, int KP,
                                                 int c_aggs, int *moved_out = nullptr)
{
    const int Ds = a.Ds, half = lane >> 5;
    if constexpr (STORE) {
        float *dst = a.state_nxt + i0 * Ds;
        const int total = nvalid * Ds;
        RowCol rc(lane, Ds);
        for (int t = lane; t < total; t += 64, rc.next()) sstore1<COH>(dst + t, X[rc.i * KP + c_aggs + rc.c]);
    }
    const float *xo = X + (lane & 31) * KP, *xn = xo + c_aggs;
    float s_ = 0.0f;
    for (int f = 0; f < Ds; ++f) {
        const float o = xo[f];
        const float d = half ? o : (xn[f] - o);
        const float dd = d * d;
        s_ = s_ + dd;
    }
    const float root = sqrtf(s_);
    const float nrm = shfl_f(root, (lane & 31) + 32);
    const float rhs = a.thr * nrm;
    const bool voter = (half == 0) && ((lane & 31) < nvalid);
    const int moved = voter && (root > rhs);
    if (moved_out) *moved_out = __any(moved) ? 1 : 0;
    else if (a.certify) {
        const float band = GNN_BAND_ABS * nrm + GNN_BAND_REL * rhs;
        const int robust = voter && (root > rhs + band), border = voter && gnn_gate_borderline(root, rhs, band);
        const bool am = __any(moved), ar = __any(robust), ab = __any(border);
        if (lane == 0) gnn_flag_raise_certified(a.flag_out, am, ar, ab);
    }
    else if (__any(moved) && lane == 0) gnn_flag_raise(a.flag_out);
}

__device__ __forceinline__ void check_store_fast64(const GnnFusedArgs &a, float *X, int64_t i0, int lane, int KP, int c_aggs)
{
    constexpr int Ds = 64;
    const int half = lane >> 5;
    const float *xo = X + (lane & 31) * KP, *xn = xo + c_aggs;
    float s_ = 0.0f;
#pragma unroll
    for (int f = 0; f < Ds; f += 16) {
        float o[16], nw[16];
#pragma unroll
        for (int u = 0; u < 16; ++u) { o[u] = xo[f + u]; nw[u] = xn[f + u]; }
#pragma unroll
        for (int u = 0; u < 16; ++u) {
            const float d = half ? o[u] : (nw[u] - o[u]);
            const float dd = d * d;
            s_ = s_ + dd;
        }
    }
    const float root = sqrtf(s_);
    const float nrm = shfl_f(root, (lane & 31) + 32);
    const float rhs = a.thr * nrm;
    const int moved = (half == 0) && (root > rhs);
    if (__any(moved) && lane == 0) gnn_flag_raise(a.flag_out);
    float *dst = a.state_nxt + i0 * Ds + lane;
    const float *xs = X + c_aggs + lane;
#pragma unroll
    for (int i = 0; i < 32; i += 8) {
        float v[8];
#pragma unroll
        for (int u = 0; u < 8; ++u) v[u] = xs[(i + u) * KP];
#pragma unroll
        for (int u = 0; u < 8; ++u) gstore_row1(dst + (i + u) * Ds, v[u]);
    }
}

__device__ __forceinline__ void finish_fast64_aligned(const GnnFusedArgs &a, float *X, f32x16 (&out)[2], int64_t i0, int lane, int KP, int c_aggs,
                                                      const GnnFlagPeek &peek)
{
    const int half = lane >> 5;
    float *xrow = X + (lane & 31) * KP;
    float d2 = 0.0f, o2 = 0.0f;
#pragma unroll
    for (int jt = 0; jt < 2; ++jt)
#pragma unroll
        for (int q = 0; q < 4; ++q) {
            const int f0 = 32 * jt + 8 * q + 4 * half;
            const v4f o = *reinterpret_cast<const v4f *>(xrow + f0);
            const v4f nw = {out[jt][4 * q], out[jt][4 * q + 1], out[jt][4 * q + 2], out[jt][4 * q + 3]};
            *reinterpret_cast<v4f *>(xrow + c_aggs + f0) = nw;
            const v4f d = nw - o;
            d2 = __builtin_fmaf(d.x, d.x, d2); d2 = __builtin_fmaf(d.y, d.y, d2); d2 = __builtin_fmaf(d.z, d.z, d2); d2 = __builtin_fmaf(d.w, d.w, d2);
            o2 = __builtin_fmaf(o.x, o.x, o2); o2 = __builtin_fmaf(o.y, o.y, o2); o2 = __builtin_fmaf(o.z, o.z, o2); o2 = __builtin_fmaf(o.w, o.w, o2);
        }
    d2 = d2 + shfl_f(d2, lane ^ 32);
    o2 = o2 + shfl_f(o2, lane ^ 32);
    const float root = sqrtf(d2), nrm = sqrtf(o2);
    {
        const float rhs = a.thr * nrm, band = GNN_BAND_ABS * nrm + GNN_BAND_REL * rhs;
        const bool am = __any(root > rhs), ar = __any(root > rhs + band), ab = __any(gnn_gate_borderline(root, rhs, band));
        if (lane == 0) gnn_flag_raise_peeked(a.flag_out, peek, am, ar, ab);
    }
    __builtin_amdgcn_fence(__ATOMIC_ACQ_REL, "wavefront");
    const int64_t dst = i0 * 64 + lane * 4;
    const float *xs = X + (lane >> 4) * KP + c_aggs + (lane & 15) * 4;
    v4f v[8];
#pragma unroll
    for (int u = 0; u < 8; ++u) v[u] = *reinterpret_cast<const v4f *>(xs + 4 * u * KP);
#pragma unroll
    for (int u = 0; u < 8; ++u) gstore_row4(a.state_nxt, dst + 256 * u, v[u]);
}

__device__ __forceinline__ void check_store_fast64_partial(const GnnFusedArgs &a, float *X, int64_t i0, int lane, int KP, int c_aggs, int nvalid)
{
    constexpr int Ds = 64;
    const int half = lane >> 5;
    const float *xo = X + (lane & 31) * KP, *xn = xo + c_aggs;
    float s_ = 0.0f;
#pragma unroll
    for (int f = 0; f < Ds; f += 16) {
        float o[16], nw[16];
#pragma unroll
        for (int u = 0; u < 16; ++u) { o[u] = xo[f + u]; nw[u] = xn[f + u]; }
#pragma unroll
        for (int u = 0; u < 16; ++u) {
            const float d = half ? o[u] : (nw[u] - o[u]);
            const float dd = d * d;
            s_ = s_ + dd;
        }
    }
    const float root = sqrtf(s_);
    const float nrm = shfl_f(root, (lane & 31) + 32);
    const float rhs = a.thr * nrm;
    const int moved = (half == 0) && (lane < nvalid) && (root > rhs);
    if (__any(moved) && lane == 0) gnn_flag_raise(a.flag_out);
    float *dst = a.state_nxt + i0 * Ds + lane;
    const float *xs = X + c_aggs + lane;
    for (int i = 0; i < nvalid; ++i) gptr_w(dst)[i * Ds] = xs[i * KP];
}

__device__ __forceinline__ void finish_fast64_partial(const GnnFusedArgs &a, float *X, f32x16 (&out)[2], int64_t i0, int lane, int KP, int c_aggs,
                                                      int nvalid)
{
    const int half = lane >> 5;
    float *xrow = X + (lane & 31) * KP;
    float d2 = 0.0f, o2 = 0.0f;
#pragma unroll
    for (int jt = 0; jt < 2; ++jt)
#pragma unroll
        for (int q = 0; q < 4; ++q) {
            const int f0 = 32 * jt + 8 * q + 4 * half;
            const v4f o = *reinterpret_cast<const v4f *>(xrow + f0);
            const v4f nw = {out[jt][4 * q], out[jt][4 * q + 1], out[jt][4 * q + 2], out[jt][4 * q + 3]};
            *reinterpret_cast<v4f *>(xrow + c_aggs + f0) = nw;
            const v4f d = nw - o;
            d2 = __builtin_fmaf(d.x, d.x, d2); d2 = __builtin_fmaf(d.y, d.y, d2); d2 = __builtin_fmaf(d.z, d.z, d2); d2 = __builtin_fmaf(d.w, d.w, d2);
            o2 = __builtin_fmaf(o.x, o.x, o2); o2 = __builtin_fmaf(o.y, o.y, o2); o2 = __builtin_fmaf(o.z, o.z, o2); o2 = __builtin_fmaf(o.w, o.w, o2);
        }
    d2 = d2 + shfl_f(d2, lane ^ 32);
    o2 = o2 + shfl_f(o2, lane ^ 32);
    const float root = sqrtf(d2), nrm = sqrtf(o2);
    {
        const bool voter = (lane & 31) < nvalid;
        const float rhs = a.thr * nrm, band = GNN_BAND_ABS * nrm + GNN_BAND_REL * rhs;
        const bool am = __any(voter && root > rhs), ar = __any(voter && root > rhs + band), ab = __any(voter && gnn_gate_borderline(root, rhs, band));
        if (lane == 0) gnn_flag_raise_certified(a.flag_out, am, ar, ab);
    }
    __builtin_amdgcn_fence(__ATOMIC_ACQ_REL, "wavefront");
    float *dst = a.state_nxt + i0 * 64 + lane * 4;
    const float *xs = X + (lane >> 4) * KP + c_aggs + (lane & 15) * 4;
    for (int u = 0; u < 8; ++u)
        if (4 * u + (lane >> 4) < nvalid) *reinterpret_cast<GNN_GLOBAL v4f *>(gptr_w(dst) + 256 * u) = *reinterpret_cast<const v4f *>(xs + 4 * u * KP);
}

__device__ __forceinline__ int tile_rowptr_request(const GnnFusedArgs &a, int tile, int lane)
{
    const int64_t i0 = (int64_t)tile * 32;
    if (i0 >= a.n_rows) return 0;
    const int nvalid = (int)((a.n_rows - i0) < 32 ? (a.n_rows - i0) : 32);
    return (lane <= nvalid) ? gstream1(a.indptr + i0 + lane) : 0;
}
__device__ __forceinline__ int tile_rowptr_clamp(const GnnFusedArgs &a, int tile, int lane, int raw)
{
    const int64_t i0 = (int64_t)tile * 32;
    if (i0 >= a.n_rows) return 0;
    const int nvalid = (int)((a.n_rows - i0) < 32 ? (a.n_rows - i0) : 32);
    const int last_ip = shfl_i(raw, nvalid);
    return lane <= nvalid ? raw : last_ip;
}
__device__ __forceinline__ void tile_first_ids(const GnnFusedArgs &a, int ip, int lane, int &src, float &w)
{
    const int gl = lane & 15, grp = lane >> 4;
    const int e_begin = shfl_i(ip, grp * 8), e_end = shfl_i(ip, grp * 8 + 8);
    src = 0; w = 0.0f;
    if (e_begin + gl < e_end) { src = gstream1(a.adj_src + e_begin + gl); w = gstream1(a.adj_w + e_begin + gl); }
}

template <int N>
__device__ __forceinline__ void zero_acc(f32x16 (&acc)[N])
{
#pragma unroll
    for (int jt = 0; jt < N; ++jt)
#pragma unroll
        for (int r = 0; r < 16; ++r) acc[jt][r] = 0.0f;
}

template <int LAYERS, int NT, int NTL, int ACT, bool SPLIT, bool FULL = false, bool GIVEN = false, int PC = 3>
__global__ void __launch_bounds__(GNN_FUSED_THREADS, 2) k_fused(const GnnFusedArgs a0)
{
    const GnnFusedArgs &a = a0;
    extern __shared__ __attribute__((aligned(16))) float lds[];
    if (!gnn_gate_open(a.gate, a.world)) return;
#ifdef GNN_DIAG
    if (a.lds_floats) {
        for (int t = threadIdx.x; t < a.lds_floats; t += blockDim.x) lds[t] = __builtin_nanf("");
        __syncthreads();
    }
#endif
    const int lane = threadIdx.x & 63, wave = __builtin_amdgcn_readfirstlane(threadIdx.x >> 6);
    const int KP = a.KP, Ds = a.Ds;
    float *X = lds + (size_t)wave * 32 * KP;
    const int c_aggs = a.c_aggs;
    const int W_launch = (int)gridDim.x * (int)(blockDim.x >> 6);
    const int w_launch = wave * (int)gridDim.x + (int)blockIdx.x;
    const bool third_round = (int64_t)2 * W_launch * 32 < a.n_rows;
    int tile = w_launch + a.tile_base, next_tile = w_launch + W_launch + a.tile_base;
    const int ip_first_raw = tile_rowptr_request(a, tile, lane);
    float *ep = lds + (size_t)GNN_FUSED_WAVES * 32 * KP + 32 + GNN_FUSED_WAVES * 36;
    for (int t = threadIdx.x; t < 3 * 32 * NTL; t += blockDim.x) {
        const int which = t / (32 * NTL), f = t - which * 32 * NTL;
        ep[t] = which == 0 ? a.bias[LAYERS - 1][f] * (SPLIT ? a.bsc[LAYERS - 1] : 1.0f) : (a.bn_scale ? (which == 1 ? a.bn_scale[f] : a.bn_shift[f]) : 0.0f);
    }
    float *hb = ep + 3 * 32 * NTL;
    if constexpr (SPLIT && LAYERS > 1)
        for (int t = threadIdx.x; t < (LAYERS - 1) * 32 * NT; t += blockDim.x)
            hb[t] = a.bias[t / (32 * NT)][t % (32 * NT)] * (ACT == GNN_ACT_SELU ? 1.44269504088896341f : 1.0f) * a.bsc[t / (32 * NT)];
    __syncthreads();
    if (a.stagger > 0) {
        int rounds = 0;
        if (a.variant & 4) rounds = wave >= GNN_FUSED_WAVES / 2 ? a.stagger : 0;
        else rounds = (int)((((unsigned)blockIdx.x * GNN_FUSED_WAVES + (unsigned)wave) * 0x9E3779B1u) >> 16) % (unsigned)(a.stagger + 1);
        for (int i = 0; i < rounds; ++i) __builtin_amdgcn_s_sleep(127);
    }
    int ip_cur = tile_rowptr_clamp(a, tile, lane, ip_first_raw);
    int src_cur = 0;
    float w_cur = 0.0f;
    if (FULL || Ds == 64) tile_first_ids(a, ip_cur, lane, src_cur, w_cur);
    if constexpr (FULL) zero_pad_columns(a, X, lane, KP);
  for (;;) {
    const int64_t i0 = (int64_t)tile * 32;
    if (i0 >= a.n_rows) break;
    const int nvalid = (int)((a0.n_rows - i0) < 32 ? (a0.n_rows - i0) : 32);
    GnnFusedArgs a = a0;
    asm volatile("" : "+s"(a.Wp[0]), "+s"(a.Wp[1]), "+s"(a.Wp[2]), "+s"(a.bias[0]), "+s"(a.bias[1]), "+s"(a.bias[2]));
    asm volatile("" : "+s"(a.bn_scale), "+s"(a.bn_shift), "+s"(a.state_cur), "+s"(a.state_nxt), "+s"(a.inv), "+s"(a.adj_src), "+s"(a.adj_w));
#ifndef GNN_DIAG
#define GNN_STAMP(slot) do { } while (0)
#else
    unsigned long long *stamp = a.stamps ? a.stamps + ((size_t)tile << 3) : nullptr;
#define GNN_STAMP(slot)                                                                      \
    do {                                                                                     \
        if (stamp) {                                                                         \
            __builtin_amdgcn_sched_barrier(0);                                               \
            const unsigned long long t_ = __builtin_amdgcn_s_memtime();                      \
            if (lane == 0) stamp[slot] = t_;                                                 \
            __builtin_amdgcn_sched_barrier(0);                                               \
        }                                                                                    \
    } while (0)
#endif
    GNN_STAMP(0);

    int *ipt = reinterpret_cast<int *>(lds + (size_t)GNN_FUSED_WAVES * 32 * KP + 32) + wave * 36;
    if (lane <= 32) ipt[lane] = ip_cur;
    const int ip_next_raw = tile_rowptr_request(a, next_tile, lane);
    const bool fast64 = FULL || ((Ds == 64) && (nvalid == 32) && !a.agg_in);
    if (a.variant & 1) __builtin_amdgcn_s_setprio(3);
    if constexpr (FULL && GIVEN) load_tile_given64<SPLIT>(a, X, i0, lane, KP, c_aggs);
    else if constexpr (FULL) load_tile_fast64<SPLIT, true>(a, X, ipt, i0, lane, KP, c_aggs, src_cur, w_cur);
    else {
        if (fast64) load_tile_fast64<SPLIT>(a, X, ipt, i0, lane, KP, c_aggs, src_cur, w_cur);
        else load_tile_generic(a, X, ipt, i0, lane, nvalid, KP, c_aggs);
    }
    if (a.variant & 1) __builtin_amdgcn_s_setprio(0);
    __builtin_amdgcn_fence(__ATOMIC_ACQ_REL, "wavefront");
    GNN_STAMP(2);

    const int half = lane >> 5;
    const float *xb = X + (lane & 31) * KP + half;
    f32x16 out[NTL];
    float mx = 0.0f;
    if constexpr (SPLIT) {
        const __amdgpu_buffer_rsrc_t wrs = __builtin_amdgcn_make_buffer_rsrc(const_cast<int *>(a.Ws_base), 0, a.ws_bytes, 0x00020000);
        const int wv = lane * 16;
        const float *xr = X + (lane & 31) * KP + 8 * half;
        if constexpr (LAYERS == 1) {
            layer0_split<NTL, false, PC>(xr, wrs, wv, a.ws_off[0], a.chunks0, out, ep, half, mx);
        } else {
            f32x16 h1[NT];
            if constexpr (FULL) layer0_split<NT, true, PC>(xr, wrs, wv, a.ws_off[0], a.chunks0, h1, hb, half, mx);
            else {
                if (Ds == 64) layer0_split<NT, true, PC>(xr, wrs, wv, a.ws_off[0], a.chunks0, h1, hb, half, mx);
                else layer0_split<NT, false, PC>(xr, wrs, wv, a.ws_off[0], a.chunks0, h1, hb, half, mx);
            }
            GNN_STAMP(3);
            GNN_STAMP(4);
            if constexpr (PC == 2) { asm volatile("" : "+v"(mx)); mx = __builtin_fmaxf(mx, hidden_range<NT>(h1, a.usc[0])); asm volatile("" : "+v"(mx)); }
            if constexpr (LAYERS == 2) {
                layer_split_from_regs<NT, NTL, ACT, PC>(h1, ep, half, out, wrs, wv, a.ws_off[1], a.usc[0], mx);
            } else {
                f32x16 h2[NT];
                layer_split_from_regs<NT, NT, ACT, PC>(h1, hb + 32 * NT, half, h2, wrs, wv, a.ws_off[1], a.usc[0], mx);
                if constexpr (PC == 2) { asm volatile("" : "+v"(mx)); mx = __builtin_fmaxf(mx, hidden_range<NT>(h2, a.usc[1])); asm volatile("" : "+v"(mx)); }
                layer_split_from_regs<NT, NTL, ACT, PC>(h2, ep, half, out, wrs, wv, a.ws_off[2], a.usc[1], mx);
            }
        }
    } else if constexpr (LAYERS == 1) {
        zero_acc<NTL>(out);
        layer_from_lds<NTL>(xb, a.Wp[0] + (size_t)lane * NTL, a.kk0, out, a.wstride);
    } else {
        f32x16 h1[NT];
        zero_acc<NT>(h1);
        layer_from_lds<NT>(xb, a.Wp[0] + (size_t)lane * NT, a.kk0, h1, a.wstride);
        GNN_STAMP(3);
        GNN_STAMP(4);
        if constexpr (LAYERS == 2) {
            zero_acc<NTL>(out);
            layer_from_regs<NT, NTL, ACT>(h1, a.bias[0], half, out, a.Wp[1] + (size_t)lane * NTL, a.wstride);
        } else {
            f32x16 h2[NT];
            zero_acc<NT>(h2);
            layer_from_regs<NT, NT, ACT>(h1, a.bias[0], half, h2, a.Wp[1] + (size_t)lane * NT, a.wstride);
            zero_acc<NTL>(out);
            layer_from_regs<NT, NTL, ACT>(h2, a.bias[1], half, out, a.Wp[2] + (size_t)lane * NTL, a.wstride);
        }
    }
    __builtin_amdgcn_fence(__ATOMIC_ACQ_REL, "wavefront");
    GNN_STAMP(5);
    int next2_tile = 0x3fffffff;
    if (third_round) {
        if (lane == 0) next2_tile = atomicAdd(a0.tile_ctr, 1) + 2 * W_launch;
    }
    const int ip_next = tile_rowptr_clamp(a, next_tile, lane, ip_next_raw);
    int src_next = 0;
    float w_next = 0.0f;
    if (FULL || Ds == 64) tile_first_ids(a, ip_next, lane, src_next, w_next);
    if constexpr (SPLIT && PC == 2) gnn_flag_raise_range(a.flag_out, mx);
    GnnFlagPeek peek = {0, 0, 0};
    if (SPLIT && NTL == 2 && lane == 0) peek = gnn_flag_peek(a.flag_out);
    bool finished = false;
    if constexpr (SPLIT && NTL == 2) {
        if (fast64) {
#pragma unroll
            for (int jt = 0; jt < NTL; ++jt) {
                if (a.bn_scale) tile_epilogue<ACT, true, true, true, true>(out[jt], ep, ep + 32 * NTL, ep + 64 * NTL, jt, half, 1 << 30, a.usc[LAYERS - 1]);
                else tile_epilogue<ACT, false, true, true, true>(out[jt], ep, nullptr, nullptr, jt, half, 1 << 30, a.usc[LAYERS - 1]);
            }
            GNN_STAMP(6);
            if (nvalid == 32) finish_fast64_aligned(a, X, out, i0, lane, KP, c_aggs, peek);
            else finish_fast64_partial(a, X, out, i0, lane, KP, c_aggs, nvalid);
            finished = true;
        }
    }
    if (!(FULL && SPLIT && NTL == 2) && !finished) {
#pragma unroll
        for (int jt = 0; jt < NTL; ++jt) {
            const float us = SPLIT ? a.usc[LAYERS - 1] : 1.0f;
            if (a.bn_scale) tile_epilogue<ACT, true, SPLIT, true, SPLIT>(out[jt], ep, ep + 32 * NTL, ep + 64 * NTL, jt, half, 1 << 30, us);
            else tile_epilogue<ACT, false, SPLIT, true, SPLIT>(out[jt], ep, nullptr, nullptr, jt, half, 1 << 30, us);
            float *x = X + (lane & 31) * KP + c_aggs;
#pragma unroll
            for (int r = 0; r < 16; ++r) {
                const int f = 32 * jt + (r & 3) + 8 * (r >> 2) + 4 * half;
                if (f < Ds) x[f] = out[jt][r];
            }
        }
        __builtin_amdgcn_fence(__ATOMIC_ACQ_REL, "wavefront");
        GNN_STAMP(6);
        if constexpr (FULL) {
            if (nvalid == 32) check_store_fast64(a, X, i0, lane, KP, c_aggs);
            else check_store_fast64_partial(a, X, i0, lane, KP, c_aggs, nvalid);
        } else {
            if (fast64) check_store_fast64(a, X, i0, lane, KP, c_aggs);
            else check_store_generic(a, X, i0, lane, nvalid, KP, c_aggs);
        }
    }
    GNN_STAMP(7);
#undef GNN_STAMP
    __builtin_amdgcn_fence(__ATOMIC_ACQ_REL, "wavefront");
    tile = next_tile;
    next_tile = __builtin_amdgcn_readfirstlane(next2_tile) + a0.tile_base;
    ip_cur = ip_next; src_cur = src_next; w_cur = w_next;
  }
}

template <int LAYERS, int NT, int NTL, int ACT, bool SPLIT, bool FULL, bool GIVEN = false, int PC = 3>
inline void launch_one_pc(const GnnFusedArgs &a, unsigned grid, size_t lds_bytes, hipStream_t st)
{
    static bool raised[64] = {false};
    int dev = 0;
    (void)hipGetDevice(&dev);
    if (dev < 0 || dev >= 64 || !raised[dev]) {
        (void)hipFuncSetAttribute(reinterpret_cast<const void *>(&k_fused<LAYERS, NT, NTL, ACT, SPLIT, FULL, GIVEN, PC>),
                                  hipFuncAttributeMaxDynamicSharedMemorySize, 160 * 1024);
        if (dev >= 0 && dev < 64) raised[dev] = true;
    }
    hipLaunchKernelGGL((k_fused<LAYERS, NT, NTL, ACT, SPLIT, FULL, GIVEN, PC>), grid, a.threads ? a.threads : GNN_FUSED_THREADS, lds_bytes, st, a);
}
template <int LAYERS, int NT, int NTL, int ACT, bool SPLIT, bool FULL, bool GIVEN = false>
inline void launch_one(const GnnFusedArgs &a, unsigned grid, size_t lds_bytes, hipStream_t st)
{
    if (SPLIT && a.pieces == 2) launch_one_pc<LAYERS, NT, NTL, ACT, SPLIT, FULL, GIVEN, 2>(a, grid, lds_bytes, st);
    else launch_one_pc<LAYERS, NT, NTL, ACT, SPLIT, FULL, GIVEN, 3>(a, grid, lds_bytes, st);
}

template <int LAYERS, int NT, int NTL, int ACT, bool SPLIT>
inline void launch(const GnnFusedArgs &a, unsigned grid, size_t lds_bytes, hipStream_t st)
{
    if constexpr (NTL == 2) {
        if (a.full_tiles && a.agg_in) { launch_one<LAYERS, NT, NTL, ACT, SPLIT, true, true>(a, grid, lds_bytes, st); return; }
        if (a.full_tiles) { launch_one<LAYERS, NT, NTL, ACT, SPLIT, true>(a, grid, lds_bytes, st); return; }
    }
    launch_one<LAYERS, NT, NTL, ACT, SPLIT, false>(a, grid, lds_bytes, st);
}

template <int LAYERS, int ACT, bool SPLIT>
inline bool launch_tiles(int nt, int ntl, const GnnFusedArgs &a, unsigned grid, size_t lds_bytes, hipStream_t st)
{
    if constexpr (LAYERS == 1) {
        if (ntl == 1) launch<1, 1, 1, ACT, SPLIT>(a, grid, lds_bytes, st);
        else if (ntl == 2) launch<1, 2, 2, ACT, SPLIT>(a, grid, lds_bytes, st);
        else if (ntl == 4) launch<1, 4, 4, ACT, SPLIT>(a, grid, lds_bytes, st);
        else return false;
    } else {
        if (nt == 1 && ntl == 1) launch<LAYERS, 1, 1, ACT, SPLIT>(a, grid, lds_bytes, st);
        else if (nt == 2 && ntl == 2) launch<LAYERS, 2, 2, ACT, SPLIT>(a, grid, lds_bytes, st);
        else if (nt == 4 && ntl == 2) launch<LAYERS, 4, 2, ACT, SPLIT>(a, grid, lds_bytes, st);
        else if (nt == 4 && ntl == 4) launch<LAYERS, 4, 4, ACT, SPLIT>(a, grid, lds_bytes, st);
        else return false;
    }
    return true;
}

template <class F>
inline bool dispatch_act(int act, F &&f)
{
    switch (act) {
    case GNN_ACT_LINEAR: return f(std::integral_constant<int, GNN_ACT_LINEAR>{});
    case GNN_ACT_RELU: return f(std::integral_constant<int, GNN_ACT_RELU>{});
    case GNN_ACT_SELU: return f(std::integral_constant<int, GNN_ACT_SELU>{});
    case GNN_ACT_ELU: return f(std::integral_constant<int, GNN_ACT_ELU>{});
    case GNN_ACT_TANH: return f(std::integral_constant<int, GNN_ACT_TANH>{});
    case GNN_ACT_SIGMOID: return f(std::integral_constant<int, GNN_ACT_SIGMOID>{});
    default: return false;
    }
}

template <int LAYERS, bool SPLIT>
inline bool launch_act(int act, int nt, int ntl, const GnnFusedArgs &a, unsigned grid, size_t lds_bytes, hipStream_t st)
{
    return dispatch_act(act, [&](auto A) { return launch_tiles<LAYERS, A.value, SPLIT>(nt, ntl, a, grid, lds_bytes, st); });
}

}
```

include/gnn_hip.h:

```cpp
#ifndef GNN_HIP_H
#define GNN_HIP_H

#include <stdint.h>

#ifdef __cplusplus
extern "C" {
#endif

typedef enum {
    GNN_OK = 0,
    GNN_ERR_ARG = -1,
    GNN_ERR_HIP = -2,
    GNN_ERR_STATE = -3,
    GNN_ERR_COMM = -4,
    GNN_ERR_UNSUPPORTED = -5
} gnn_status;

typedef enum {
    GNN_ACT_LINEAR = 0, GNN_ACT_RELU = 1, GNN_ACT_SELU = 2, GNN_ACT_ELU = 3,
    GNN_ACT_TANH = 4, GNN_ACT_SIGMOID = 5, GNN_ACT_SOFTMAX = 6
} gnn_activation;

typedef struct gnn_graph gnn_graph;
typedef struct gnn_mlp gnn_mlp;
typedef struct gnn_loop gnn_loop;
typedef struct gnn_comm gnn_comm;

const char *gnn_last_error(void);
int gnn_version(void);
int gnn_device_count(int *count);
int gnn_device_synchronize(int device);

int gnn_graph_create(int64_t n_nodes, int64_t row_begin, int64_t n_rows, int64_t n_arcs, const int32_t *indptr,
                     const int32_t *adj_src, const float *adj_w, const float *arc_w, const float *arc_labels,
                     int dim_arc_label, const float *nodes, int dim_node_label, const uint8_t *mask, int device,
                     gnn_graph **out);
int gnn_graph_create_from_arcs(int64_t n_nodes, int64_t n_arcs, const int32_t *arc_src, const int32_t *arc_dst,
                               const float *arc_labels, int dim_arc_label, int aggregation_mode, const float *nodes,
                               int dim_node_label, const uint8_t *mask, int device, gnn_graph **out,
                               int32_t *indptr_out, int32_t *adj_src_out, float *adj_w_out, int32_t *arc_id_out,
                               float *arc_w_out);
int gnn_graph_derive(const gnn_graph *base, int extra_node_label_dims, gnn_graph **out);
int gnn_graph_update_labels(gnn_graph *dst, const gnn_graph *base, const gnn_loop *from, int get_state, int get_output);
int gnn_graph_set_arc_order(gnn_graph *g, const int32_t *arc_id, const float *arc_labels_orig);
int gnn_graph_derive_edge(const gnn_graph *base, int extra_nodes, int extra_arcs, gnn_graph **out);
int gnn_graph_get_nodes(const gnn_graph *g, float *nodes_out );
int gnn_graph_dims(const gnn_graph *g, int64_t *n_nodes, int64_t *n_rows, int64_t *n_arcs, int *dim_node_label,
                   int *dim_arc_label, int64_t *n_masked);
int gnn_graph_destroy(gnn_graph *g);

int gnn_mlp_create(int n_layers, const int32_t *dims, const int32_t *acts, const float *const *W, const float *const *b,
                   const float *bn, float bn_eps, int device, gnn_mlp **out);
int gnn_mlp_set_weights(gnn_mlp *m, const float *const *W, const float *const *b, const float *bn);
int gnn_mlp_forward(gnn_mlp *m, int64_t n_rows, const float *x, float *y);
int gnn_mlp_get_weights(gnn_mlp *m, float *const *W, float *const *b, float *bn);
int gnn_mlp_reset_optimizer(gnn_mlp *m);
int gnn_mlp_destroy(gnn_mlp *m);

int gnn_loop_create(gnn_graph *g, gnn_mlp *net_state, gnn_mlp *net_output, int state_dim, int max_iter, float threshold,
                    gnn_comm *comm , gnn_loop **out);
int gnn_loop_set_state0(gnn_loop *l, const float *state0, uint64_t seed);
int gnn_loop_run(gnn_loop *l, int training, float *k_out);
int gnn_loop_run_many(gnn_loop **loops, int n, float *k_out);
int gnn_loop_get_state(const gnn_loop *l, float *state_out );
int gnn_loop_get_output(const gnn_loop *l, float *out , int64_t *n_masked);
int gnn_loop_readout(const gnn_loop *l, int n_graphs, const int32_t *ng_indptr, const int32_t *ng_node,
                     const float *ng_w, float *out_graph );
int gnn_loop_set_edge_readout(gnn_loop *l, const int32_t *entry_dst, const float *arc_labels, const uint8_t *arc_mask);
int gnn_loop_train_step(gnn_loop *l, const int32_t *src_indptr, const int32_t *src_dst, const float *src_w,
                        const float *targets, const float *sample_weights, int64_t n_targets, int loss_kind,
                        int n_graphs, const int32_t *ng_indptr, const int32_t *ng_node, const float *ng_w,
                        const float *dropout_state, const float *dropout_output, const uint8_t *masks_state,
                        const uint8_t *masks_output, uint64_t seed, const float *bn_state, const float *bn_output,
                        float *loss_out, float *k_out, float *grads_state, float *grads_output,
                        float *bn_batch_state, float *bn_batch_output);
int gnn_loop_train_forward(gnn_loop *l, const int32_t *src_indptr, const int32_t *src_dst, const float *src_w,
                           const float *dropout_state, const float *dropout_output, const uint8_t *masks_state,
                           const uint8_t *masks_output, uint64_t seed, const float *bn_state, const float *bn_output,
                           float *k_out, float *out_nodes);
int gnn_loop_train_backward(gnn_loop *l, const float *d_out_nodes, const float *d_state_extra, float *grads_state,
                            float *grads_output, float *bn_batch_state, float *bn_batch_output, float *d_nodes,
                            float *d_arc_labels);
int gnn_loop_update_moving_statistics(gnn_loop *l, float bn_momentum_state, float bn_momentum_output);
int gnn_loop_arm_optimizer(gnn_loop *l, int kind, const float *hyper, int mean, float bn_momentum_state, float bn_momentum_output);
int gnn_loop_optimizer_step(gnn_loop *l, int kind, const float *hyper, float state_grad_scale, float bn_momentum_state,
                            float bn_momentum_output);
int gnn_loss_grad(int loss_kind, int64_t n_rows, int n_out, const float *targets, const float *out,
                  const float *sample_weights, double *loss, float *d_out);
int gnn_loss_grad_ex(int loss_kind, int64_t n_rows, int n_out, const float *targets, const float *out,
                     const float *sample_weights, double label_smoothing, double huber_delta, double *loss, float *d_out);
int gnn_loop_set_loss_params(gnn_loop *l, double label_smoothing, double huber_delta);
int gnn_mlp_set_regularizers(gnn_mlp *m, const double *l1, const double *l2);
int gnn_loop_set_clipping(gnn_loop *l, double clipvalue, double clipnorm, double global_clipnorm);
int gnn_loop_grad_sqnorm(gnn_loop *l, float state_grad_scale, double *sqnorm, double *penalty);
int gnn_loop_optimizer_step_scaled(gnn_loop *l, int kind, const float *hyper, float state_grad_scale, double grad_scale,
                                   float bn_momentum_state, float bn_momentum_output);
int gnn_loop_set_impl(gnn_loop *l, int impl, int *used);
int gnn_loop_gate_info(const gnn_loop *l, int *last_run_repeated, int *repeats_total);
int gnn_loop_set_pieces(gnn_loop *l, int pieces, int *used);
int gnn_loop_range_info(const gnn_loop *l, int *last_run_repeated, int *repeats_total);
int gnn_split_f16_exponent(float max_abs);
void gnn_split_f16(const float *v, int n, int e, uint16_t *p0, uint16_t *p1);
int gnn_loop_set_persistent(gnn_loop *l, int enable, int *used);
int gnn_loop_set_tile_form(gnn_loop *l, int form, int *used);
int gnn_loop_set_profiling(gnn_loop *l, int enable);
int gnn_loop_drop_cached_aggregates(gnn_loop *l);
int gnn_loop_get_timing(const gnn_loop *l, float *total_ms, float *avg_iter_ms, int *n_iter_timed);
int gnn_loop_get_exchange_timing(const gnn_loop *l, float *avg_between_bodies_ms);
int gnn_counters_get(const gnn_loop *l, double *bytes_per_iteration, double *flops_per_iteration, int *iterations, float *total_ms,
                     float *avg_iteration_ms);
int gnn_lgnn_run(gnn_loop *const *loops, gnn_graph *const *graphs, int n_layers, int get_state, int get_output, float *k_out);
int gnn_loop_destroy(gnn_loop *l);

int gnn_shard_range(int64_t n_nodes, int rank, int world, int64_t *row_begin, int64_t *n_rows);
int gnn_comm_unique_id(uint8_t id[128]);
int gnn_comm_create(const uint8_t id[128], int rank, int world, int device, gnn_comm **out);
int gnn_comm_allreduce_max(gnn_comm *c, double *value);
int gnn_comm_destroy(gnn_comm *c);
int gnn_halo_plan(int64_t n_nodes, int world, const int32_t *indptr, const int32_t *adj_src, int32_t *slot ,
                  int64_t *counts , int64_t *block);
int gnn_graph_create_halo(int64_t n_nodes_global, int rank, int world, int64_t halo_block, int64_t n_send, const int32_t *send_rows,
                          int64_t n_arcs, const int32_t *indptr, const int32_t *adj_src_replica, const float *adj_w,
                          const float *arc_w, const float *arc_labels, int dim_arc_label, const float *nodes_replica,
                          int dim_node_label, const uint8_t *mask, int device, gnn_graph **out);
int gnn_graph_set_full_adjacency(gnn_graph *g, int64_t n_global, const int32_t *indptr, const int32_t *adj_src, const float *adj_w);
int gnn_loop_set_slice_exchange(gnn_loop *l, int on);
int gnn_comm_create_loopback(int world, int device, gnn_comm **out );
int gnn_loop_run_group(gnn_loop **loops, int n, float *k_out);
int gnn_loop_readout_group(gnn_loop **loops, int n, int n_graphs, const int32_t *ng_indptr, const int32_t *ng_node,
                           const float *ng_w, float *out_graph);
int gnn_graph_update_labels_group(gnn_graph **dsts, gnn_graph *const *bases, gnn_loop *const *froms, int n, int get_state,
                                  int get_output);

#ifdef __cplusplus
}
#endif
#endif
```

Before: 1.737 billion node-state-updates/s.

## Add precompiled per-tile gather program for load-balanced neighbor aggregation

Builds a host-side 'gather program' once per graph. Each 32-node tile's arcs are packed into fixed 16-entry batches across four lane groups, with row counts balanced by a binary-searched split. Each entry holds the source index, row id, end flag and weight in one record. The fused kernel gets a PROG variant, used by default, that streams these batches instead of walking the CSR rowptr, which is meant to even out per-lane gather work and remove the rowptr and index indirection. The cost is extra device memory and padding entries for uneven tiles, plus a one-time D2H copy and CPU build, and a restriction to source ids below 2^23.

```diff
diff --git a/gnn_tf_2.x_amd/GNN/_engine.py b/gnn_tf_2.x_amd/GNN/_engine.py
--- a/gnn_tf_2.x_amd/GNN/_engine.py
+++ b/gnn_tf_2.x_amd/GNN/_engine.py
@@ -17,7 +17,7 @@
            'gnn_loop_train_forward', 'gnn_loop_train_backward', 'gnn_loop_arm_optimizer', 'gnn_loop_optimizer_step', 'gnn_loop_update_moving_statistics', 'gnn_loss_grad',
            'gnn_loss_grad_ex', 'gnn_loop_set_loss_params',
            'gnn_mlp_set_regularizers', 'gnn_loop_set_clipping', 'gnn_loop_grad_sqnorm', 'gnn_loop_optimizer_step_scaled',
-           'gnn_counters_get', 'gnn_lgnn_run', 'gnn_loop_run_many', 'gnn_loop_set_impl', 'gnn_loop_gate_info', 'gnn_loop_set_pieces', 'gnn_loop_range_info', 'gnn_split_f16_exponent', 'gnn_split_f16', 'gnn_loop_set_persistent', 'gnn_loop_set_tile_form', 'gnn_loop_drop_cached_aggregates', 'gnn_loop_set_profiling', 'gnn_loop_get_timing', 'gnn_loop_get_exchange_timing', 'gnn_loop_destroy', 'gnn_shard_range',
+           'gnn_counters_get', 'gnn_lgnn_run', 'gnn_loop_run_many', 'gnn_loop_set_impl', 'gnn_loop_gate_info', 'gnn_loop_set_pieces', 'gnn_loop_range_info', 'gnn_split_f16_exponent', 'gnn_split_f16', 'gnn_loop_set_persistent', 'gnn_loop_set_tile_form', 'gnn_loop_set_gather_form', 'gnn_gather_program_build', 'gnn_graph_gather_program_info', 'gnn_loop_drop_cached_aggregates', 'gnn_loop_set_profiling', 'gnn_loop_get_timing', 'gnn_loop_get_exchange_timing', 'gnn_loop_destroy', 'gnn_shard_range',
            'gnn_comm_unique_id', 'gnn_comm_create', 'gnn_comm_allreduce_max', 'gnn_comm_destroy', 'gnn_halo_plan', 'gnn_graph_create_halo',
            'gnn_comm_create_loopback', 'gnn_graph_set_full_adjacency', 'gnn_loop_set_slice_exchange', 'gnn_loop_run_group', 'gnn_loop_readout_group', 'gnn_graph_update_labels_group']
 
@@ -103,6 +103,19 @@
     b, n = C.c_int64(0), C.c_int64(0)
     _check(lib().gnn_shard_range(C.c_int64(n_nodes), C.c_int(rank), C.c_int(world), C.byref(b), C.byref(n)))
     return b.value, n.value
+
+
+def gather_program(indptr, adj_src, adj_w):
+    indptr = np.ascontiguousarray(indptr, dtype=np.int32)
+    adj_src = np.ascontiguousarray(adj_src, dtype=np.int32)
+    adj_w = _f32(adj_w)
+    n_rows = indptr.size - 1
+    hdr = np.zeros((n_rows // 32, 2), np.int32)
+    nb = C.c_int64(0)
+    _check(lib().gnn_gather_program_build(C.c_int64(n_rows), _ip(indptr), _ip(adj_src), _fp(adj_w), _ip(hdr), None, C.byref(nb)))
+    ent = np.zeros((nb.value, 64, 2), np.int32)
+    _check(lib().gnn_gather_program_build(C.c_int64(n_rows), _ip(indptr), _ip(adj_src), _fp(adj_w), None, _ip(ent), C.byref(nb)))
+    return hdr, ent.view(np.uint32)
 
 
 def halo_plan(n_nodes: int, world: int, indptr, adj_src):
@@ -225,6 +238,11 @@
         d = Graph(None, None, None, None, None, None, None, None, _handle=h)
         d._base = self
         return d
+
+    def gather_program_info(self) -> dict:
+        t, b, n, ms = C.c_int64(0), C.c_int64(0), C.c_int64(0), C.c_float(0)
+        _check(lib().gnn_graph_gather_program_info(self._h, C.byref(t), C.byref(b), C.byref(n), C.byref(ms)))
+        return dict(tiles=t.value, batches=b.value, bytes=n.value, build_ms=ms.value)
 
     def set_arc_order(self, arc_id, arc_labels_orig) -> None:
         arc_id = np.ascontiguousarray(arc_id, dtype=np.int32)
@@ -598,6 +616,11 @@
         _check(lib().gnn_loop_set_tile_form(self._h, C.c_int(int(form)), C.byref(used)))
         return used.value
 
+    def set_gather_form(self, form: int) -> int:
+        used = C.c_int(0)
+        _check(lib().gnn_loop_set_gather_form(self._h, C.c_int(int(form)), C.byref(used)))
+        return used.value
+
     def counters(self) -> dict:
         b, f, it, tot, avg = C.c_double(), C.c_double(), C.c_int(), C.c_float(), C.c_float()
         _check(lib().gnn_counters_get(self._h, C.byref(b), C.byref(f), C.byref(it), C.byref(tot), C.byref(avg)))
diff --git a/gnn_tf_2.x_amd/csrc/gnn_build.hip b/gnn_tf_2.x_amd/csrc/gnn_build.hip
--- a/gnn_tf_2.x_amd/csrc/gnn_build.hip
+++ b/gnn_tf_2.x_amd/csrc/gnn_build.hip
@@ -2,9 +2,12 @@
 #include <string.h>
 
 #include <algorithm>
+#include <chrono>
+#include <new>
 #include <vector>
 
 #include "gnn_common.h"
+#include "gnn_fused.h"
 
 namespace {
 
@@ -180,3 +183,132 @@
     return GNN_OK;
 #undef HIPCHK_G
 }
+
+namespace {
+
+void gather_program_split(const int (&slots)[32], int (&start)[5], int &longest)
+{
+    int lo = 0, hi = 0;
+    for (int r = 0; r < 32; ++r) { lo = std::max(lo, slots[r]); hi += slots[r]; }
+    auto groups_needed = [&](int cap) {
+        int n = 1, fill = 0;
+        for (int r = 0; r < 32; ++r) {
+            if (fill + slots[r] > cap) { ++n; fill = 0; }
+            fill += slots[r];
+        }
+        return n;
+    };
+    while (lo < hi) {
+        const int mid = lo + (hi - lo) / 2;
+        if (groups_needed(mid) <= 4) hi = mid; else lo = mid + 1;
+    }
+    int g = 0, fill = 0;
+    start[0] = 0;
+    for (int r = 0; r < 32; ++r) {
+        if (fill + slots[r] > lo) { start[++g] = r; fill = 0; }
+        fill += slots[r];
+    }
+    while (g < 4) start[++g] = 32;
+    longest = lo;
+}
+
+}
+
+extern "C" int gnn_gather_program_build(int64_t n_rows, const int32_t *indptr, const int32_t *adj_src, const float *adj_w, int32_t *hdr,
+                                        int32_t *ent, int64_t *n_batches)
+{
+    ARGCHK(n_rows >= 0 && indptr && n_batches, "n_rows / indptr / n_batches are required");
+    const int64_t tiles = n_rows / 32;
+    ARGCHK(indptr[tiles * 32] == 0 || (adj_src && adj_w), "arc arrays are required");
+    int64_t batch = 0;
+    for (int64_t t = 0; t < tiles; ++t) {
+        const int32_t *ip = indptr + t * 32;
+        int slots[32], start[5], longest = 0;
+        for (int r = 0; r < 32; ++r) {
+            ARGCHK(ip[r + 1] >= ip[r], "indptr not monotone at row %lld", (long long)(t * 32 + r));
+            slots[r] = std::max(1, ip[r + 1] - ip[r]);
+        }
+        gather_program_split(slots, start, longest);
+        const int nb = (longest + 15) / 16;
+        ARGCHK(batch + nb < ((int64_t)1 << 31) / 64, "gather program too large");
+        if (hdr) { hdr[2 * t] = (int32_t)batch; hdr[2 * t + 1] = nb; }
+        if (ent) {
+            for (int g = 0; g < 4; ++g) {
+                int s = 0;
+                auto put = [&](uint32_t word, float w) {
+                    int32_t *e = ent + (((batch + s / 16) * 64 + 16 * g + s % 16) * 2);
+                    memcpy(e, &word, 4);
+                    memcpy(e + 1, &w, 4);
+                    ++s;
+                };
+                for (int r = start[g]; r < start[g + 1]; ++r) {
+                    if (ip[r + 1] == ip[r]) put(GNN_GP_NOROW | GNN_GP_ROW_END | (uint32_t)r, 0.0f);
+                    for (int32_t e = ip[r]; e < ip[r + 1]; ++e) {
+                        if (adj_src[e] < 0 || adj_src[e] >= (1 << 23))
+                            return gnn_fail(GNN_ERR_UNSUPPORTED, "adj_src[%d]=%d does not fit a gather-program source word", e, adj_src[e]);
+                        put((uint32_t)adj_src[e] << 8 | (e + 1 == ip[r + 1] ? GNN_GP_ROW_END : 0u) | (uint32_t)r, adj_w[e]);
+                    }
+                }
+                while (s < 16 * nb) put(GNN_GP_NOROW, 0.0f);
+            }
+        }
+        batch += nb;
+    }
+    *n_batches = batch;
+    return GNN_OK;
+}
+
+int gnn_gather_program_ensure(const gnn_graph *g)
+{
+    gnn_graph_shared *sh = g->sh;
+    if (sh->gp_tried) return GNN_OK;
+    sh->gp_tried = true;
+    const int64_t tiles = g->n_rows / 32;
+    if (tiles == 0) return GNN_OK;
+    int dev_before = -1;
+    if (hipGetDevice(&dev_before) != hipSuccess || hipSetDevice(g->device) != hipSuccess) { (void)hipGetLastError(); return GNN_OK; }
+    const auto t0 = std::chrono::steady_clock::now();
+    int32_t *d_hdr = nullptr, *d_ent = nullptr;
+    int64_t batches = 0;
+    bool ok = false;
+    try {
+        std::vector<int32_t> indptr((size_t)tiles * 32 + 1), hdr((size_t)tiles * 2), src, ent;
+        std::vector<float> w;
+        ok = hipMemcpy(indptr.data(), sh->indptr, sizeof(int32_t) * indptr.size(), hipMemcpyDeviceToHost) == hipSuccess;
+        const size_t E = ok ? (size_t)indptr.back() : 0;
+        src.resize(E); w.resize(E);
+        ok = ok && (E == 0 || (hipMemcpy(src.data(), sh->adj_src, sizeof(int32_t) * E, hipMemcpyDeviceToHost) == hipSuccess &&
+                               hipMemcpy(w.data(), sh->adj_w, sizeof(float) * E, hipMemcpyDeviceToHost) == hipSuccess));
+        for (size_t e = 0; ok && e < E; ++e) ok = src[e] >= 0 && src[e] < (1 << 23);
+        ok = ok && gnn_gather_program_build(tiles * 32, indptr.data(), src.data(), w.data(), hdr.data(), nullptr, &batches) == GNN_OK;
+        if (ok) {
+            ent.resize((size_t)batches * 128);
+            ok = gnn_gather_program_build(tiles * 32, indptr.data(), src.data(), w.data(), nullptr, ent.data(), &batches) == GNN_OK;
+        }
+        ok = ok && gnn_dev_malloc((void **)&d_hdr, sizeof(int32_t) * hdr.size()) == hipSuccess &&
+             gnn_dev_malloc((void **)&d_ent, sizeof(int32_t) * ent.size()) == hipSuccess &&
+             hipMemcpy(d_hdr, hdr.data(), sizeof(int32_t) * hdr.size(), hipMemcpyHostToDevice) == hipSuccess &&
+             hipMemcpy(d_ent, ent.data(), sizeof(int32_t) * ent.size(), hipMemcpyHostToDevice) == hipSuccess;
+    } catch (const std::bad_alloc &) { ok = false; }
+    if (ok) {
+        sh->gp_hdr = d_hdr; sh->gp_ent = d_ent; sh->gp_tiles = tiles; sh->gp_batches = batches;
+        sh->gp_build_ms = std::chrono::duration<float, std::milli>(std::chrono::steady_clock::now() - t0).count();
+    } else {
+        (void)hipFree(d_hdr); (void)hipFree(d_ent);
+        (void)hipGetLastError();
+    }
+    (void)hipSetDevice(dev_before);
+    return GNN_OK;
+}
+
+extern "C" int gnn_graph_gather_program_info(const gnn_graph *g, int64_t *tiles, int64_t *batches, int64_t *bytes, float *build_ms)
+{
+    ARGCHK(g, "graph is NULL");
+    const gnn_graph_shared *sh = g->sh;
+    const bool have = sh->gp_ent != nullptr;
+    if (tiles) *tiles = have ? sh->gp_tiles : 0;
+    if (batches) *batches = have ? sh->gp_batches : 0;
+    if (bytes) *bytes = have ? sh->gp_tiles * 8 + sh->gp_batches * 512 : 0;
+    if (build_ms) *build_ms = have ? sh->gp_build_ms : 0.0f;
+    return GNN_OK;
+}
diff --git a/gnn_tf_2.x_amd/csrc/gnn_common.h b/gnn_tf_2.x_amd/csrc/gnn_common.h
--- a/gnn_tf_2.x_amd/csrc/gnn_common.h
+++ b/gnn_tf_2.x_amd/csrc/gnn_common.h
@@ -138,6 +138,10 @@
     int32_t *full_indptr = nullptr, *full_src = nullptr;
     float *full_w = nullptr;
     int64_t full_rows = 0;
+    int32_t *gp_hdr = nullptr, *gp_ent = nullptr;
+    int64_t gp_tiles = 0, gp_batches = 0;
+    bool gp_tried = false;
+    float gp_build_ms = 0.0f;
 };
 
 struct gnn_graph {
@@ -247,6 +251,8 @@
     bool graph_ready_seen = false;
     int impl_req = 1, impl_used = 0;
     int tile_form = 0;
+    int gather_form = 0;
+    bool gather_program = false;
     int32_t *ng_ip = nullptr, *ng_node = nullptr;
     float *ng_w = nullptr, *ng_out = nullptr, *ng_part = nullptr;
     std::vector<int32_t> ng_key;
@@ -302,6 +308,8 @@
 
 bool gnn_fused_supported(const gnn_loop *l);
 bool gnn_fused_pair_selected(const gnn_loop *l);
+bool gnn_fused_program_selected(const gnn_loop *l);
+int gnn_gather_program_ensure(const gnn_graph *g);
 int gnn_fused_prepare(gnn_loop *l);
 int gnn_fused_pack(gnn_mlp *m, int nlc);
 int gnn_fused_iteration(gnn_loop *l, int k);
diff --git a/gnn_tf_2.x_amd/csrc/gnn_engine.hip b/gnn_tf_2.x_amd/csrc/gnn_engine.hip
--- a/gnn_tf_2.x_amd/csrc/gnn_engine.hip
+++ b/gnn_tf_2.x_amd/csrc/gnn_engine.hip
@@ -667,6 +667,7 @@
     (void)hipFree(sh->src_indptr); (void)hipFree(sh->src_dst); (void)hipFree(sh->src_w);
     (void)hipFree(sh->arc_id); (void)hipFree(sh->arc_labels_orig);
     (void)hipFree(sh->full_indptr); (void)hipFree(sh->full_src); (void)hipFree(sh->full_w);
+    (void)hipFree(sh->gp_hdr); (void)hipFree(sh->gp_ent);
     delete sh;
 }
 
@@ -1339,6 +1340,14 @@
     ARGCHK(l && form >= 0 && form <= 2, "form must be 0 (library's choice), 1 (one wave per tile) or 2 (wave pair per tile)");
     l->tile_form = form;
     if (used) *used = (l->impl_req >= 1 && gnn_fused_supported(l)) ? (gnn_fused_pair_selected(l) ? 2 : 1) : 0;
+    return GNN_OK;
+}
+
+extern "C" int gnn_loop_set_gather_form(gnn_loop *l, int form, int *used)
+{
+    ARGCHK(l && form >= 0 && form <= 2, "form must be 0 (library's choice), 1 (walk the CSR) or 2 (the graph's gather program)");
+    l->gather_form = form;
+    if (used) *used = (l->impl_req >= 1 && gnn_fused_supported(l)) ? (gnn_fused_program_selected(l) ? 2 : 1) : 0;
     return GNN_OK;
 }
 
diff --git a/gnn_tf_2.x_amd/csrc/gnn_fused.h b/gnn_tf_2.x_amd/csrc/gnn_fused.h
--- a/gnn_tf_2.x_amd/csrc/gnn_fused.h
+++ b/gnn_tf_2.x_amd/csrc/gnn_fused.h
@@ -7,6 +7,9 @@
 constexpr int GNN_FUSED_THREADS = 64 * GNN_FUSED_WAVES;
 #define GNN_F16_EX 4
 #define GNN_F16_LIMIT 65504.0f
+#define GNN_GP_ROW_MASK 31u
+#define GNN_GP_ROW_END 32u
+#define GNN_GP_NOROW 0xfffffe00u
 
 struct GnnFusedArgs {
     int64_t n_rows, row_begin;
@@ -38,6 +41,8 @@
     int full_tiles;
     int variant;
     const float *agg_in;
+    const int32_t *gp_hdr, *gp_ent;
+    int gp_tiles;
     int threads;
     int single_ticket;
     unsigned long long *stamps;
diff --git a/gnn_tf_2.x_amd/csrc/gnn_fused.hip b/gnn_tf_2.x_amd/csrc/gnn_fused.hip
--- a/gnn_tf_2.x_amd/csrc/gnn_fused.hip
+++ b/gnn_tf_2.x_amd/csrc/gnn_fused.hip
@@ -28,6 +28,9 @@
 constexpr int GNN_FUSED_VARIANT_DEFAULT = 1;
 constexpr int GNN_FUSED_SPREAD_DEFAULT = 8;
 constexpr int GNN_FUSED_SPREAD_SMALL_DEFAULT = 6;
+#ifndef GNN_GATHER_FORM_DEFAULT
+#define GNN_GATHER_FORM_DEFAULT 2
+#endif
 constexpr int S_SLACK = 2;
 
 int round_tiles(int width) { return width <= 32 ? 1 : (width <= 64 ? 2 : 4); }
@@ -121,6 +124,16 @@
     if (!pair_covers(p, l->Ds) || pair_lds_bytes(p) > 160 * 1024) return false;
     if (l->tile_form) return l->tile_form == 2;
     return (l->g->n_rows + 31) / 32 <= (int64_t)4 * device_cus(l->device);
+}
+
+bool gnn_fused_program_selected(const gnn_loop *l)
+{
+    FusedPlan p;
+    if (l->impl_req < 1 || l->slice_mode || l->Ds != 64 || !make_plan(l->st, l->NLc, p) || p.NTL != 2) return false;
+    if ((l->gather_form ? l->gather_form : GNN_GATHER_FORM_DEFAULT) != 2) return false;
+    if (l->impl_req == 2 && gnn_fused_pair_selected(l)) return false;
+    if (gnn_gather_program_ensure(l->g) != GNN_OK) return false;
+    return l->g->sh->gp_ent != nullptr;
 }
 
 extern "C" int gnn_split_f16_exponent(float max_abs)
@@ -261,6 +274,7 @@
 int gnn_fused_prepare(gnn_loop *l)
 {
     const gnn_graph *g = l->g;
+    l->gather_program = gnn_fused_program_selected(l);
     const int IW = 2 * l->NLc + g->AL;
     if (!l->inv) {
         const size_t inv_floats = std::max<size_t>(1, (size_t)((g->n_rows + 31) / 32 * 32) * IW);
@@ -408,6 +422,7 @@
     else if (l->Ds == 64 && p.NTL == 2 && n_tiles64 >= 1) {
         GnnFusedArgs af = a;
         af.full_tiles = 1; af.tile_base = 0;
+        if (l->gather_program) { af.gp_hdr = g->sh->gp_hdr; af.gp_ent = g->sh->gp_ent; af.gp_tiles = (int)g->sh->gp_tiles; }
         ok = go(af, (unsigned)std::min<size_t>((size_t)n_cu, (size_t)n_tiles64));
     } else
         ok = go(a, grid);
diff --git a/gnn_tf_2.x_amd/csrc/gnn_fused_kernel.h b/gnn_tf_2.x_amd/csrc/gnn_fused_kernel.h
--- a/gnn_tf_2.x_amd/csrc/gnn_fused_kernel.h
+++ b/gnn_tf_2.x_amd/csrc/gnn_fused_kernel.h
@@ -764,25 +764,55 @@
       x[J] = __builtin_bit_cast(v4f, __builtin_amdgcn_raw_buffer_load_b128(rsrc, (row_bcast_i<J>(my_src) << 8) + voff0, 0, 0))), ...);
 }
 
+template <bool AL16>
+struct TileOwn64 {
+    v4f own[8];
+    float lab[4];
+    __device__ __forceinline__ void request(const GnnFusedArgs &a, int64_t i0, int lane)
+    {
+        const float *src = a.state_cur + (a.row_begin + i0) * 64 + lane * 4;
+#pragma unroll
+        for (int u = 0; u < 8; ++u) own[u] = gload4(src + u * 256);
+        const int IW = a.IW, nlab = 32 * IW;
+        const float *lsrc = a.inv + i0 * IW;
+#pragma unroll
+        for (int u = 0; u < 4; ++u) lab[u] = (lane + 64 * u < nlab) ? gload1(lsrc + lane + 64 * u) : 0.0f;
+    }
+    __device__ __forceinline__ void write(const GnnFusedArgs &a, float *X, int64_t i0, int lane, int KP, int c_aggs) const
+    {
+        constexpr int Ds = 64;
+        const int IW = a.IW, nlab = 32 * IW;
+#pragma unroll
+        for (int u = 0; u < 8; ++u) {
+            float *x = X + (4 * u + (lane >> 4)) * KP + (lane & 15) * 4;
+            if constexpr (AL16) *reinterpret_cast<v4f *>(x) = own[u];
+            else { x[0] = own[u].x; x[1] = own[u].y; x[2] = own[u].z; x[3] = own[u].w; }
+        }
+        const float inv_iw = 1.0f / (float)(IW > 0 ? IW : 1);
+#pragma unroll
+        for (int u = 0; u < 4; ++u) {
+            const int t = lane + 64 * u;
+            if (t < nlab) {
+                const int i = (int)(((float)t + 0.5f) * inv_iw), c = t - i * IW;
+                X[i * KP + label_col(c, Ds, a.NLc, c_aggs)] = lab[u];
+            }
+        }
+        if (nlab > 256)
+            for (int t = 256 + lane; t < nlab; t += 64) {
+                const int i = t / IW, c = t - i * IW;
+                X[i * KP + label_col(c, Ds, a.NLc, c_aggs)] = gload1(a.inv + i0 * IW + t);
+            }
+    }
+};
+
 template <bool AL16, bool PADDED = false>
 __device__ __forceinline__ void load_tile_fast64(const GnnFusedArgs &a, float *X, const int *ipt, int64_t i0, int lane,
                                                  int KP, int c_aggs, int my_src, float my_w)
 {
-    constexpr int GB = 16, Ds = 64;
+    constexpr int GB = 16;
     const int gl = lane & 15, grp = lane >> 4;
-    v4f own[8];
-    {
-        const float *src = a.state_cur + (a.row_begin + i0) * Ds + lane * 4;
-#pragma unroll
-        for (int u = 0; u < 8; ++u) own[u] = gload4(src + u * 256);
-    }
-    float lab[4];
-    const int IW = a.IW, nlab = 32 * IW;
-    {
-        const float *src = a.inv + i0 * IW;
-#pragma unroll
-        for (int u = 0; u < 4; ++u) lab[u] = (lane + 64 * u < nlab) ? gload1(src + lane + 64 * u) : 0.0f;
-    }
+    TileOwn64<AL16> own;
+    own.request(a, i0, lane);
     if constexpr (!PADDED) zero_pad_columns(a, X, lane, KP);
     __builtin_amdgcn_fence(__ATOMIC_ACQ_REL, "wavefront");
 
@@ -837,26 +867,65 @@
         else { xr[0] = acc01.x; xr[1] = acc01.y; xr[2] = acc23.x; xr[3] = acc23.y; }
         acc01 = v2f{0.f, 0.f}; acc23 = v2f{0.f, 0.f};
     }
-#pragma unroll
-    for (int u = 0; u < 8; ++u) {
-        float *x = X + (4 * u + (lane >> 4)) * KP + (lane & 15) * 4;
-        if constexpr (AL16) *reinterpret_cast<v4f *>(x) = own[u];
-        else { x[0] = own[u].x; x[1] = own[u].y; x[2] = own[u].z; x[3] = own[u].w; }
-    }
-    const float inv_iw = 1.0f / (float)(IW > 0 ? IW : 1);
-#pragma unroll
-    for (int u = 0; u < 4; ++u) {
-        const int t = lane + 64 * u;
-        if (t < nlab) {
-            const int i = (int)(((float)t + 0.5f) * inv_iw), c = t - i * IW;
-            X[i * KP + label_col(c, Ds, a.NLc, c_aggs)] = lab[u];
-        }
-    }
-    if (nlab > 256)
-        for (int t = 256 + lane; t < nlab; t += 64) {
-            const int i = t / IW, c = t - i * IW;
-            X[i * KP + label_col(c, Ds, a.NLc, c_aggs)] = gload1(a.inv + i0 * IW + t);
-        }
+    own.write(a, X, i0, lane, KP, c_aggs);
+}
+
+template <bool AL16, int J>
+__device__ __forceinline__ void prog_consume(int words, float w, v4f x, v2f &acc01, v2f &acc23, float *xo, int KP)
+{
+    gather_fma(acc01, acc23, w, x);
+    const unsigned t = (unsigned)row_bcast_i<J>(words);
+    if (t & GNN_GP_ROW_END) {
+        float *xr = xo + __umul24(t & GNN_GP_ROW_MASK, (unsigned)KP);
+        if constexpr (AL16) *reinterpret_cast<v4f *>(xr) = v4f{acc01.x, acc01.y, acc23.x, acc23.y};
+        else { xr[0] = acc01.x; xr[1] = acc01.y; xr[2] = acc23.x; xr[3] = acc23.y; }
+        acc01 = v2f{0.f, 0.f}; acc23 = v2f{0.f, 0.f};
+    }
+}
+template <bool AL16, int GB, int... J>
+__device__ __forceinline__ void prog_batch(int words, float my_w, __amdgpu_buffer_rsrc_t rsrc, int voff0, float (&w)[GB], v4f (&x)[GB],
+                                           std::integer_sequence<int, J...>)
+{
+    ((w[J] = row_bcast_f<J>(my_w),
+      x[J] = __builtin_bit_cast(v4f, __builtin_amdgcn_raw_buffer_load_b128(rsrc, (row_bcast_i<J>(words) & ~0xff) | voff0, 0, 0))), ...);
+}
+template <bool AL16, int GB, int... J>
+__device__ __forceinline__ void prog_consume_all(int words, const float (&w)[GB], const v4f (&x)[GB], v2f &acc01, v2f &acc23, float *xo, int KP,
+                                                 std::integer_sequence<int, J...>)
+{
+    (prog_consume<AL16, J>(words, w[J], x[J], acc01, acc23, xo, KP), ...);
+}
+typedef int v2i __attribute__((ext_vector_type(2)));
+__device__ __forceinline__ v2i prog_header_request(const GnnFusedArgs &a, int tile)
+{
+    v2i h = {0, 0};
+    if (tile < a.gp_tiles) h = *reinterpret_cast<const GNN_GLOBAL v2i *>(gptr(a.gp_hdr) + 2 * (int64_t)tile);
+    return h;
+}
+__device__ __forceinline__ v2i prog_entry(const GnnFusedArgs &a, int b, int lane)
+{
+    return *reinterpret_cast<const GNN_GLOBAL v2i *>(gptr(a.gp_ent) + ((int64_t)b * 64 + lane) * 2);
+}
+template <bool AL16>
+__device__ __forceinline__ void load_tile_prog64(const GnnFusedArgs &a, float *X, int64_t i0, int lane, int KP, int c_aggs, int first, int nb, v2i ent)
+{
+    constexpr int GB = 16;
+    const int gl = lane & 15;
+    TileOwn64<AL16> own;
+    own.request(a, i0, lane);
+    v2f acc01 = {0.f, 0.f}, acc23 = {0.f, 0.f};
+    const __amdgpu_buffer_rsrc_t rsrc = __builtin_amdgcn_make_buffer_rsrc(const_cast<float *>(a.state_cur), 0, (int)a.state_bytes, 0x00020000);
+    const int voff0 = gl * 16;
+    float *xo = X + c_aggs + gl * 4;
+    for (int b = 0; b < nb; ++b) {
+        float w[GB];
+        v4f x[GB];
+        const int words = ent.x;
+        prog_batch<AL16, GB>(words, __int_as_float(ent.y), rsrc, voff0, w, x, std::make_integer_sequence<int, GB>{});
+        if (b + 1 < nb) ent = prog_entry(a, first + b + 1, lane);
+        prog_consume_all<AL16, GB>(words, w, x, acc01, acc23, xo, KP, std::make_integer_sequence<int, GB>{});
+    }
+    own.write(a, X, i0, lane, KP, c_aggs);
 }
 
 template <bool AL16>
@@ -1104,7 +1173,7 @@
         for (int r = 0; r < 16; ++r) acc[jt][r] = 0.0f;
 }
 
-template <int LAYERS, int NT, int NTL, int ACT, bool SPLIT, bool FULL = false, bool GIVEN = false, int PC = 3>
+template <int LAYERS, int NT, int NTL, int ACT, bool SPLIT, bool FULL = false, bool GIVEN = false, int PC = 3, bool PROG = false>
 __global__ void __launch_bounds__(GNN_FUSED_THREADS, 2) k_fused(const GnnFusedArgs a0)
 {
     const GnnFusedArgs &a = a0;
@@ -1124,7 +1193,10 @@
     const int w_launch = wave * (int)gridDim.x + (int)blockIdx.x;
     const bool third_round = (int64_t)2 * W_launch * 32 < a.n_rows;
     int tile = w_launch + a.tile_base, next_tile = w_launch + W_launch + a.tile_base;
-    const int ip_first_raw = tile_rowptr_request(a, tile, lane);
+    int ip_first_raw = 0;
+    v2i hdr_first_raw = {0, 0};
+    if constexpr (PROG) hdr_first_raw = prog_header_request(a, tile);
+    else ip_first_raw = tile_rowptr_request(a, tile, lane);
     float *ep = lds + (size_t)GNN_FUSED_WAVES * 32 * KP + 32 + GNN_FUSED_WAVES * 36;
     for (int t = threadIdx.x; t < 3 * 32 * NTL; t += blockDim.x) {
         const int which = t / (32 * NTL), f = t - which * 32 * NTL;
@@ -1141,10 +1213,17 @@
         else rounds = (int)((((unsigned)blockIdx.x * GNN_FUSED_WAVES + (unsigned)wave) * 0x9E3779B1u) >> 16) % (unsigned)(a.stagger + 1);
         for (int i = 0; i < rounds; ++i) __builtin_amdgcn_s_sleep(127);
     }
-    int ip_cur = tile_rowptr_clamp(a, tile, lane, ip_first_raw);
-    int src_cur = 0;
+    int ip_cur = 0, src_cur = 0;
     float w_cur = 0.0f;
-    if (FULL || Ds == 64) tile_first_ids(a, ip_cur, lane, src_cur, w_cur);
+    int hdr_first = 0, hdr_nb = 0;
+    v2i ent_cur = {0, 0};
+    if constexpr (PROG) {
+        hdr_first = __builtin_amdgcn_readfirstlane(hdr_first_raw.x); hdr_nb = __builtin_amdgcn_readfirstlane(hdr_first_raw.y);
+        if (hdr_nb > 0) ent_cur = prog_entry(a, hdr_first, lane);
+    } else {
+        ip_cur = tile_rowptr_clamp(a, tile, lane, ip_first_raw);
+        if (FULL || Ds == 64) tile_first_ids(a, ip_cur, lane, src_cur, w_cur);
+    }
     if constexpr (FULL) zero_pad_columns(a, X, lane, KP);
   for (;;) {
     const int64_t i0 = (int64_t)tile * 32;
@@ -1170,11 +1249,25 @@
     GNN_STAMP(0);
 
     int *ipt = reinterpret_cast<int *>(lds + (size_t)GNN_FUSED_WAVES * 32 * KP + 32) + wave * 36;
-    if (lane <= 32) ipt[lane] = ip_cur;
-    const int ip_next_raw = tile_rowptr_request(a, next_tile, lane);
+    int ip_next_raw = 0;
+    v2i hdr_next_raw = {0, 0};
+    if constexpr (PROG) hdr_next_raw = prog_header_request(a, next_tile);
+    else {
+        if (lane <= 32) ipt[lane] = ip_cur;
+        ip_next_raw = tile_rowptr_request(a, next_tile, lane);
+    }
     const bool fast64 = FULL || ((Ds == 64) && (nvalid == 32) && !a.agg_in);
     if (a.variant & 1) __builtin_amdgcn_s_setprio(3);
     if constexpr (FULL && GIVEN) load_tile_given64<SPLIT>(a, X, i0, lane, KP, c_aggs);
+    else if constexpr (PROG) {
+        if (hdr_nb > 0) load_tile_prog64<SPLIT>(a, X, i0, lane, KP, c_aggs, hdr_first, hdr_nb, ent_cur);
+        else {
+            const int ip = tile_rowptr_clamp(a, tile, lane, tile_rowptr_request(a, tile, lane));
+            if (lane <= 32) ipt[lane] = ip;
+            tile_first_ids(a, ip, lane, src_cur, w_cur);
+            load_tile_fast64<SPLIT, true>(a, X, ipt, i0, lane, KP, c_aggs, src_cur, w_cur);
+        }
+    }
     else if constexpr (FULL) load_tile_fast64<SPLIT, true>(a, X, ipt, i0, lane, KP, c_aggs, src_cur, w_cur);
     else {
         if (fast64) load_tile_fast64<SPLIT>(a, X, ipt, i0, lane, KP, c_aggs, src_cur, w_cur);
@@ -1239,10 +1332,17 @@
     if (third_round) {
         if (lane == 0) next2_tile = atomicAdd(a0.tile_ctr, 1) + 2 * W_launch;
     }
-    const int ip_next = tile_rowptr_clamp(a, next_tile, lane, ip_next_raw);
-    int src_next = 0;
+    int ip_next = 0, src_next = 0;
     float w_next = 0.0f;
-    if (FULL || Ds == 64) tile_first_ids(a, ip_next, lane, src_next, w_next);
+    int hdr_first_next = 0, hdr_nb_next = 0;
+    v2i ent_next = {0, 0};
+    if constexpr (PROG) {
+        hdr_first_next = __builtin_amdgcn_readfirstlane(hdr_next_raw.x); hdr_nb_next = __builtin_amdgcn_readfirstlane(hdr_next_raw.y);
+        if (hdr_nb_next > 0) ent_next = prog_entry(a, hdr_first_next, lane);
+    } else {
+        ip_next = tile_rowptr_clamp(a, next_tile, lane, ip_next_raw);
+        if (FULL || Ds == 64) tile_first_ids(a, ip_next, lane, src_next, w_next);
+    }
     if constexpr (SPLIT && PC == 2) gnn_flag_raise_range(a.flag_out, mx);
     GnnFlagPeek peek = {0, 0, 0};
     if (SPLIT && NTL == 2 && lane == 0) peek = gnn_flag_peek(a.flag_out);
@@ -1289,21 +1389,25 @@
     tile = next_tile;
     next_tile = __builtin_amdgcn_readfirstlane(next2_tile) + a0.tile_base;
     ip_cur = ip_next; src_cur = src_next; w_cur = w_next;
+    hdr_first = hdr_first_next; hdr_nb = hdr_nb_next; ent_cur = ent_next;
   }
 }
 
-template <int LAYERS, int NT, int NTL, int ACT, bool SPLIT, bool FULL, bool GIVEN = false, int PC = 3>
+template <int LAYERS, int NT, int NTL, int ACT, bool SPLIT, bool FULL, bool GIVEN = false, int PC = 3, bool PROG = false>
 inline void launch_one_pc(const GnnFusedArgs &a, unsigned grid, size_t lds_bytes, hipStream_t st)
 {
+    if constexpr (FULL && !GIVEN && !PROG) {
+        if (a.gp_tiles > 0) { launch_one_pc<LAYERS, NT, NTL, ACT, SPLIT, FULL, GIVEN, PC, true>(a, grid, lds_bytes, st); return; }
+    }
     static bool raised[64] = {false};
     int dev = 0;
     (void)hipGetDevice(&dev);
     if (dev < 0 || dev >= 64 || !raised[dev]) {
-        (void)hipFuncSetAttribute(reinterpret_cast<const void *>(&k_fused<LAYERS, NT, NTL, ACT, SPLIT, FULL, GIVEN, PC>),
+        (void)hipFuncSetAttribute(reinterpret_cast<const void *>(&k_fused<LAYERS, NT, NTL, ACT, SPLIT, FULL, GIVEN, PC, PROG>),
                                   hipFuncAttributeMaxDynamicSharedMemorySize, 160 * 1024);
         if (dev >= 0 && dev < 64) raised[dev] = true;
     }
-    hipLaunchKernelGGL((k_fused<LAYERS, NT, NTL, ACT, SPLIT, FULL, GIVEN, PC>), grid, a.threads ? a.threads : GNN_FUSED_THREADS, lds_bytes, st, a);
+    hipLaunchKernelGGL((k_fused<LAYERS, NT, NTL, ACT, SPLIT, FULL, GIVEN, PC, PROG>), grid, a.threads ? a.threads : GNN_FUSED_THREADS, lds_bytes, st, a);
 }
 template <int LAYERS, int NT, int NTL, int ACT, bool SPLIT, bool FULL, bool GIVEN = false>
 inline void launch_one(const GnnFusedArgs &a, unsigned grid, size_t lds_bytes, hipStream_t st)
diff --git a/include/gnn_hip.h b/include/gnn_hip.h
--- a/include/gnn_hip.h
+++ b/include/gnn_hip.h
@@ -103,6 +103,10 @@
 void gnn_split_f16(const float *v, int n, int e, uint16_t *p0, uint16_t *p1);
 int gnn_loop_set_persistent(gnn_loop *l, int enable, int *used);
 int gnn_loop_set_tile_form(gnn_loop *l, int form, int *used);
+int gnn_loop_set_gather_form(gnn_loop *l, int form, int *used);
+int gnn_gather_program_build(int64_t n_rows, const int32_t *indptr, const int32_t *adj_src, const float *adj_w, int32_t *hdr, int32_t *ent,
+                             int64_t *n_batches);
+int gnn_graph_gather_program_info(const gnn_graph *g, int64_t *tiles, int64_t *batches, int64_t *bytes, float *build_ms);
 int gnn_loop_set_profiling(gnn_loop *l, int enable);
 int gnn_loop_drop_cached_aggregates(gnn_loop *l);
 int gnn_loop_get_timing(const gnn_loop *l, float *total_ms, float *avg_iter_ms, int *n_iter_timed);
```

New measurement: 1.766 billion node-state-updates/s (median of 6 runs). 1.7% higher.
